# adrelino/mv-lm-icp

Measured on NVIDIA H100. Metric: ICP iterations/sec (corr+LM), higher is better.
Workload: dtype f64

## Files before the change

mv_lm_icp_b200/csrc/g2o.cuh:

```cuda
#pragma once
#include <cuda_runtime.h>
#include "../../include/mvicp.h"
#include "knn.cuh"
#include "lm_eval.cuh"
#include "lm_step.cuh"
#include "se3_math.cuh"
#include "types.cuh"

namespace mv {

enum { G2O_BUILD = 0, G2O_TRIAL = 1 };

struct G2oState {
  int32_t M, E, n, max_iter, max_calls, no_impr_limit, max_trials, ortho_after;
  int32_t phase, done, ended, last_call_end, call, iter, q, no_impr;
  int32_t n_iters, n_trials, n_accepted, n_evals, n_trace, trace_cap;
  double tau, lambda, nu, chi, last_chi, chi_initial, scale;
};

__host__ __device__ __forceinline__ void g2o_prec0(const double* n, double eps, double* Om) {
  double y[3] = {-n[1] * n[0], 1.0 - n[1] * n[1], -n[1] * n[2]};
  const double yy = y[0] * y[0] + y[1] * y[1] + y[2] * y[2];
  if (yy > 0.0) { const double s = sqrt(yy); y[0] /= s; y[1] /= s; y[2] /= s; }
  double x[3]; cross(n, y, x);
  const double* R[3] = {x, y, n};
  const double d[3] = {eps, eps, 1.0};
  int k = 0;
  for (int a = 0; a < 3; ++a)
    for (int b = a; b < 3; ++b) Om[k++] = (R[0][a] * d[0]) * R[0][b] + (R[1][a] * d[1]) * R[1][b] + (R[2][a] * d[2]) * R[2][b];
}

template <bool F32, bool NF32, int COST>
__global__ void __launch_bounds__(EVAL_THREADS)
g2o_eval_kernel(const FrameDev* __restrict__ frames, const EdgeDev* __restrict__ edges, const Tile* __restrict__ tiles, int tile_len,
                const int32_t* __restrict__ corr, const Rt* __restrict__ pose_eval, const G2oState* __restrict__ S, double eps,
                double* __restrict__ partial) {
  if (S->done) return;
  const bool build = S->phase == G2O_BUILD;
  const Tile t = tiles[blockIdx.x];
  const EdgeDev e = edges[t.edge];
  __shared__ double sF1[9], st1[3], sF0T[9], smt[3], sM01[9];
  __shared__ double sred[EVAL_THREADS / 32][2][GACC];
  if (threadIdx.x == 0) {
    const Rt a = pose_eval[e.src], k = pose_eval[e.dst];
    for (int i = 0; i < 9; ++i) sF1[i] = a.R[i];
    for (int i = 0; i < 3; ++i) for (int j = 0; j < 3; ++j) sF0T[3 * i + j] = k.R[3 * j + i];
    double ft[3]; matTvec(k.R, k.t, ft);
    for (int i = 0; i < 3; ++i) { st1[i] = a.t[i]; smt[i] = -ft[i]; }
    matTmul(k.R, a.R, sM01);
  }
  __syncthreads();
  const int role = threadIdx.x & 1;
  double C[9];
#pragma unroll
  for (int i = 0; i < 9; ++i) C[i] = role ? ((i % 4 == 0) ? 1.0 : 0.0) : sM01[i];
  const double tsg = role ? -1.0 : 1.0, rsg = role ? 2.0 : -2.0;
  const FrameDev fs = frames[e.src];
  const FrameDev fd = frames[e.dst];
  double acc[GACC];
#pragma unroll
  for (int i = 0; i < GACC; ++i) acc[i] = 0.0;
  const int end = min(t.start + tile_len, e.n_src);
  for (int k0 = t.start; k0 < end; k0 += EVAL_THREADS / 2) {
    const int k = k0 + (threadIdx.x >> 1);
    const int c = k < end ? __ldg(corr + e.off + k) : -1;
    const bool ok = c >= 0;
    if (!__any_sync(0xffffffffu, ok)) continue;
    double p[3] = {0, 0, 0}, q[3] = {0, 0, 0}, n[3] = {0, 0, 0}; int dummy;
    if (ok) {
      Rec<F32>::load(fs.pts_o, k, p[0], p[1], p[2], dummy);
      Rec<F32>::load(fd.pts_o, c, q[0], q[1], q[2], dummy);
      if (COST == COST_P2PLANE) Rec<NF32>::load(fd.nor_o, c, n[0], n[1], n[2], dummy);
    }
    const double live = ok ? 1.0 : 0.0;
    double y[3], u[3], r[3];
    matvec(sF1, p, y);
#pragma unroll
    for (int i = 0; i < 3; ++i) y[i] += st1[i];
    matvec(sF0T, y, u);
#pragma unroll
    for (int i = 0; i < 3; ++i) { u[i] += smt[i]; r[i] = u[i] - q[i]; }
    double Om[6] = {1, 0, 0, 1, 0, 1};
    if (COST == COST_P2PLANE) g2o_prec0(n, eps, Om);
    const double O3[9] = {Om[0], Om[1], Om[2], Om[1], Om[3], Om[4], Om[2], Om[4], Om[5]};
    double Or[3]; matvec(O3, r, Or);
    acc[45] += live * (r[0] * Or[0] + r[1] * Or[1] + r[2] * Or[2]);
    if (!build) continue;
    const double v[3] = {role ? u[0] : p[0], role ? u[1] : p[1], role ? u[2] : p[2]};
    const double vx[3][3] = {{0.0, v[2], -v[1]}, {-v[2], 0.0, v[0]}, {v[1], -v[0], 0.0}};
    double J[3][6], W[3][6];
#pragma unroll
    for (int i = 0; i < 3; ++i)
#pragma unroll
      for (int j = 0; j < 3; ++j) {
        J[i][j] = tsg * C[3 * i + j];
        J[i][3 + j] = rsg * (C[3 * i] * vx[j][0] + C[3 * i + 1] * vx[j][1] + C[3 * i + 2] * vx[j][2]);
      }
#pragma unroll
    for (int i = 0; i < 3; ++i)
#pragma unroll
      for (int j = 0; j < 6; ++j) W[i][j] = O3[3 * i] * J[0][j] + O3[3 * i + 1] * J[1][j] + O3[3 * i + 2] * J[2][j];
    int idx = 0;
#pragma unroll
    for (int a = 0; a < 6; ++a)
#pragma unroll
      for (int b = a; b < 6; ++b) acc[idx++] += live * (J[0][a] * W[0][b] + J[1][a] * W[1][b] + J[2][a] * W[2][b]);
#pragma unroll
    for (int a = 0; a < 3; ++a) {
      double X[3];
#pragma unroll
      for (int i = 0; i < 3; ++i) { const double o = __shfl_xor_sync(0xffffffffu, J[i][3 + a], 1); X[i] = role ? o : J[i][a]; }
#pragma unroll
      for (int b = 0; b < 6; ++b) {
        double Y[3];
#pragma unroll
        for (int i = 0; i < 3; ++i) { const double o = __shfl_xor_sync(0xffffffffu, W[i][b], 1); Y[i] = role ? W[i][b] : o; }
        acc[21 + 6 * a + b] += live * (X[0] * Y[0] + X[1] * Y[1] + X[2] * Y[2]);
      }
    }
#pragma unroll
    for (int a = 0; a < 6; ++a) acc[39 + a] += live * (J[0][a] * Or[0] + J[1][a] * Or[1] + J[2][a] * Or[2]);
  }
  const int lane = threadIdx.x & 31, wid = threadIdx.x >> 5;
#pragma unroll
  for (int i = 0; i < GACC; ++i) {
    if (!build && i != 45) continue;
    double v = acc[i];
#pragma unroll
    for (int o = 16; o > 1; o >>= 1) v += __shfl_xor_sync(0xffffffffu, v, o);
    if (lane < 2) sred[wid][lane][i] = v;
  }
  __syncthreads();
  if (threadIdx.x < 2 * GACC) {
    const int rl = threadIdx.x / GACC, i = threadIdx.x - GACC * rl;
    if (!build && i != 45) return;
    double v = 0.0;
    for (int w = 0; w < EVAL_THREADS / 32; ++w) v += sred[w][rl][i];
    int dst = -1;
    if (i < 21) {
      int a = 0, rem = i; while (rem >= 6 - a) { rem -= 6 - a; ++a; }
      dst = u12(6 * rl + a, 6 * rl + a + rem);
    } else if (i < 39) {
      const int a = (i - 21) / 6, b = (i - 21) - 6 * a;
      dst = u12(rl ? 3 + a : a, 6 + b);
    } else if (i < 45) dst = 78 + 6 * rl + (i - 39);
    else if (rl == 0) dst = 90;
    if (dst >= 0) partial[(size_t)blockIdx.x * GBLK + dst] = v;
  }
}

__global__ void __launch_bounds__(EDGE_THREADS)
g2o_edge_kernel(const int32_t* __restrict__ edge_tile_begin, const double* __restrict__ partial, const G2oState* __restrict__ S,
                double* __restrict__ out) {
  if (S->done) return;
  const bool build = S->phase == G2O_BUILD;
  const int e = blockIdx.x, tid = threadIdx.x;
  __shared__ double blk[GBLK];
  double* o = out + (size_t)EOUT_ * e;
  for (int j = tid; j < 91; j += EDGE_THREADS) {
    if (!build && j != 90) continue;
    double v = 0.0;
    for (int t = edge_tile_begin[e]; t < edge_tile_begin[e + 1]; ++t) v += partial[(size_t)t * GBLK + j];
    blk[j] = v;
  }
  __syncthreads();
  if (!build) { if (tid == 0) o[156] = blk[90]; return; }
  for (int r = tid; r < 157; r += EDGE_THREADS) {
    if (r < 144) { const int a = r / 12, b = r - 12 * a; o[r] = blk[u12(min(a, b), max(a, b))]; }
    else if (r < 156) o[r] = blk[78 + (r - 144)];
    else o[r] = blk[90];
  }
}

__global__ void g2o_count_kernel(const EdgeDev* __restrict__ edges, const Tile* __restrict__ tiles, int tile_len, const int32_t* __restrict__ corr,
                                 unsigned long long* __restrict__ count) {
  const Tile t = tiles[blockIdx.x];
  const EdgeDev e = edges[t.edge];
  const int end = min(t.start + tile_len, e.n_src);
  int m = 0;
  for (int k = t.start + threadIdx.x; k < end; k += blockDim.x) m += __ldg(corr + e.off + k) >= 0 ? 1 : 0;
  if (m) atomicAdd(count + t.edge, (unsigned long long)m);
}

struct G2oWork {
  G2oState* S;
  const double* eout;
  Rt* x;
  Rt* ev;
  int32_t* n_oplus;
  NormalLayout lay;
  double *H, *g;
  double* chi_calls;
  double* trace;
};

__global__ void g2o_init_kernel(G2oWork w, int M) {
  const int f = blockIdx.x * blockDim.x + threadIdx.x;
  if (f >= M) return;
  Rt a; pose16_to_Rt(w.lay.poses16 + 16 * f, &a);
  w.x[f] = a; w.ev[f] = a; w.n_oplus[f] = 0;
}

__device__ __forceinline__ void g2o_oplus(const Rt& x, const double* d, int* count, int ortho_after, Rt* out) {
  const double qq = d[3] * d[3] + d[4] * d[4] + d[5] * d[5];
  double R[9] = {1, 0, 0, 0, 1, 0, 0, 0, 1};
  if (!(1.0 - qq < 0.0)) {
    const double qw = sqrt(1.0 - qq), qx = d[3], qy = d[4], qz = d[5];
    const double tx = 2 * qx, ty = 2 * qy, tz = 2 * qz;
    const double twx = tx * qw, twy = ty * qw, twz = tz * qw, txx = tx * qx, txy = ty * qx, txz = tz * qx, tyy = ty * qy, tyz = tz * qy, tzz = tz * qz;
    R[0] = 1 - (tyy + tzz); R[1] = txy - twz; R[2] = txz + twy;
    R[3] = txy + twz; R[4] = 1 - (txx + tzz); R[5] = tyz - twx;
    R[6] = txz - twy; R[7] = tyz + twx; R[8] = 1 - (txx + tyy);
  }
  matmul(x.R, R, out->R);
  matvec(x.R, d, out->t);
  for (int i = 0; i < 3; ++i) out->t[i] += x.t[i];
  if (++*count > ortho_after) {
    *count = 0;
    double Em[9]; matTmul(out->R, out->R, Em);
    Em[0] -= 1; Em[4] -= 1; Em[8] -= 1;
    double FE[9]; matmul(out->R, Em, FE);
    for (int i = 0; i < 9; ++i) out->R[i] -= 0.5 * FE[i];
  }
}

__global__ void __launch_bounds__(STEP_THREADS) g2o_step_kernel(G2oWork w) {
  extern __shared__ double smem[];
  __shared__ double red[40];
  __shared__ G2oState s_state;
  __shared__ int s_solve, s_accept, s_tobuild;
  if (w.S->done) { if (threadIdx.x == 0) publish_step(w.lay, true); return; }
  const int tid = threadIdx.x, T = blockDim.x;
  copy_state(&s_state, w.S);
  G2oState* S = &s_state;
  const int n = S->n, M = S->M, E = S->E;
  const int phase = S->phase;
  const NormalLayout& lay = w.lay;
  double* colj = smem; double* dg = smem + 2 * (n + 1);
  double* L = lay.l_in_smem ? smem + 3 * (n + 1) : lay.Lg;

  const double chi_eval = edge_cost_sum(w.eout, E, red);

  auto end_iter = [&](double rho) {
    S->iter += 1; S->n_iters += 1;
    const bool term = S->q == S->max_trials || rho == 0.0;
    if (term || S->iter >= S->max_iter) {
      S->last_call_end = term ? MVICP_G2O_CALL_TERMINATE : MVICP_G2O_CALL_ITERATIONS;
      w.chi_calls[S->call + 1] = S->chi;
      const double impr = (S->last_chi - S->chi) / S->last_chi;
      S->last_chi = S->chi;
      if (!(impr > 0.0)) S->no_impr += 1;
      S->call += 1;
      if (S->no_impr > S->no_impr_limit) { S->done = 1; S->ended = MVICP_G2O_END_NO_IMPROVEMENT; return; }
      if (S->call >= S->max_calls) { S->done = 1; S->ended = MVICP_G2O_END_MAX_CALLS; return; }
      S->iter = 0;
    }
    S->phase = G2O_BUILD;
    s_tobuild = 1;
  };
  auto record = [&](double tchi, double rho, bool acc) {
    if (S->n_trace < S->trace_cap) {
      double* r = w.trace + 5 * (size_t)S->n_trace;
      r[0] = S->lambda; r[1] = S->chi; r[2] = tchi; r[3] = rho; r[4] = acc ? 1.0 : 0.0;
    }
    S->n_trace += 1;
  };

  if (tid == 0) { s_solve = 0; s_accept = 0; s_tobuild = 0; S->n_evals += 1; }
  if (phase == G2O_BUILD) {
    gather_blocks(lay, w.eout, n, w.H);
    gather_gradient(lay, w.eout, M, w.g);
    __syncthreads();
    double md = 0.0;
    for (int j = tid; j < n; j += T) md = fmax(md, fabs(w.H[(size_t)j * n + j]));
    md = block_max(md, red);
    if (tid == 0) {
      if (S->call == 0 && S->iter == 0) { S->chi_initial = S->last_chi = chi_eval; w.chi_calls[0] = chi_eval; }
      S->chi = chi_eval;
      if (S->iter == 0) { S->lambda = S->tau * md; S->nu = 2.0; }
      S->q = 0;
      s_solve = 1;
    }
  } else if (tid == 0) {
    const double tchi = chi_eval;
    const double rho = (S->chi - tchi) / S->scale;
    const bool acc = rho > 0.0 && isfinite(tchi);
    record(tchi, rho, acc);
    if (acc) {
      const double a = 1.0 - (2.0 * rho - 1.0) * (2.0 * rho - 1.0) * (2.0 * rho - 1.0);
      S->lambda *= fmax(1.0 / 3.0, fmin(2.0 / 3.0, a));
      S->nu = 2.0; S->chi = tchi; S->n_accepted += 1;
      s_accept = 1;
    } else { S->lambda *= S->nu; S->nu *= 2.0; }
    S->q += 1;
    if (rho < 0.0 && S->q < S->max_trials) s_solve = 1; else end_iter(rho);
  }
  __syncthreads();
  if (s_accept) for (int f = tid; f < M; f += T) w.x[f] = w.ev[f];
  __syncthreads();

  while (s_solve) {
    const double lambda = S->lambda;
    for (int i = tid >> 5; i < n; i += T >> 5) {
      const int rbi = lay.rowbase[i];
      for (int j = lay.rfirst[i] + (tid & 31); j <= i; j += 32) L[rbi + j] = w.H[(size_t)i * n + j] + (i == j ? lambda : 0.0);
    }
    { const int rbn = lay.rowbase[n]; for (int j = tid; j < n; j += T) L[rbn + j] = -w.g[j]; }
    __syncthreads();
    bool ok = chol_solve(L, lay.rowbase, n, colj, dg, lay.rhs, lay.rlast, lay.rfirst);
    double bad = 0.0;
    if (ok) for (int j = tid; j < n; j += T) if (!isfinite(lay.rhs[j])) bad = 1.0;
    bad = block_sum(bad, red);
    ok = ok && bad == 0.0;
    double sc = 0.0;
    if (ok) for (int j = tid; j < n; j += T) sc += lay.rhs[j] * (lambda * lay.rhs[j] - w.g[j]);
    sc = block_sum(sc, red);
    for (int f = tid; f < M; f += T) {
      const int cf = lay.col[f];
      if (cf < 0) continue;
      Rt nx;
      g2o_oplus(w.x[f], lay.rhs + cf, &w.n_oplus[f], S->ortho_after, &nx);
      if (ok) w.ev[f] = nx;
    }
    __syncthreads();
    if (tid == 0) {
      S->n_trials += 1;
      s_solve = 0;
      if (ok) { S->scale = sc + 1e-3; S->phase = G2O_TRIAL; }
      else {
        const double rho = -INFINITY;
        record(INFINITY, rho, false);
        S->lambda *= S->nu; S->nu *= 2.0; S->q += 1;
        if (S->q < S->max_trials) s_solve = 1; else end_iter(rho);
      }
    }
    __syncthreads();
  }
  if (s_tobuild && !S->done) for (int f = tid; f < M; f += T) w.ev[f] = w.x[f];
  if (S->done)
    for (int f = tid; f < M; f += T) if (lay.col[f] >= 0) Rt_to_pose16(&w.x[f], lay.poses16 + 16 * f);
  __syncthreads();
  copy_state(w.S, &s_state);
  if (tid == 0) publish_step(lay, S->done);
}

}
```

mv_lm_icp_b200/csrc/lm_step.cuh:

```cuda
#pragma once
#include <cuda_runtime.h>
#include "../../include/mvicp.h"
#include "se3_math.cuh"
#include "types.cuh"

namespace mv {

constexpr int STEP_THREADS = 512;
constexpr int EOUT = 160;

struct LmState {
  mvicp_lm_options opt;
  int32_t param, cost_kind, robust, M, E, F, n, G;
  int32_t phase, done, termination, iteration, n_success, n_invalid, n_evals, n_solves, reuse_diagonal, nonrigid;
  double radius, decrease_factor, x_cost, cand_cost, x_norm, initial_cost, model_cost_change, step_norm, gmax;
};

struct NormalLayout {
  const int32_t* col;
  const int32_t* hb_ptr; const int32_t* hb_row; const int32_t* hb_col; const int32_t* hc_edge; const int32_t* hc_sub; int32_t n_hblocks;
  const int32_t* gb_ptr; const int32_t* gc_edge; const int32_t* gc_side;
  const int32_t* rlast; const int32_t* rfirst;
  const int32_t* rowbase;
  double *Lg, *rhs;
  int32_t l_in_smem;
  double* poses16;
  volatile int32_t* host_flag;
  int32_t seq;
};

struct LmWork {
  LmState* S;
  const EdgeDev* edges;
  const double* eout;
  volatile int* peer_flags;
  int32_t world, xseq;
  double* x;
  double* cand;
  Rt* Rt_eval;
  double* K_eval;
  FrameGen* G_eval;
  NormalLayout lay;
  double *H, *g, *Hc, *gc, *scale, *diag, *step;
  long long* prof;
};

struct LmProblem {
  LmState* S;
  const int32_t* frame;
  const int32_t* edge;
  NormalLayout lay;
  double *H, *g, *Hc, *gc, *scale, *diag, *step;
};

__device__ __forceinline__ double block_sum(double v, double* red) {
  __syncthreads();
  const int lane = threadIdx.x & 31, wid = threadIdx.x >> 5;
#pragma unroll
  for (int o = 16; o > 0; o >>= 1) v += __shfl_down_sync(0xffffffffu, v, o);
  if (lane == 0) red[wid] = v;
  __syncthreads();
  if (threadIdx.x == 0) { double s = 0; for (int w = 0; w < STEP_THREADS / 32; ++w) s += red[w]; red[32] = s; }
  __syncthreads();
  return red[32];
}
__device__ __forceinline__ double block_max(double v, double* red) {
  __syncthreads();
  const int lane = threadIdx.x & 31, wid = threadIdx.x >> 5;
#pragma unroll
  for (int o = 16; o > 0; o >>= 1) v = fmax(v, __shfl_down_sync(0xffffffffu, v, o));
  if (lane == 0) red[wid] = v;
  __syncthreads();
  if (threadIdx.x == 0) { double s = 0; for (int w = 0; w < STEP_THREADS / 32; ++w) s = fmax(s, red[w]); red[32] = s; }
  __syncthreads();
  return red[32];
}

__device__ __forceinline__ void gather_blocks(const NormalLayout& l, const double* eout, int n, double* H) {
  for (int idx = threadIdx.x; idx < l.n_hblocks * 36; idx += blockDim.x) {
    const int b = idx / 36, r = idx - 36 * b, i = r / 6, j = r - 6 * i;
    double s = 0;
    for (int c = l.hb_ptr[b]; c < l.hb_ptr[b + 1]; ++c) {
      const int e = l.hc_edge[c], sub = l.hc_sub[c];
      s += eout[(size_t)EOUT * e + (6 * (sub >> 1) + i) * 12 + 6 * (sub & 1) + j];
    }
    H[(size_t)(l.hb_row[b] + i) * n + l.hb_col[b] + j] = s;
  }
}
__device__ __forceinline__ void gather_gradient(const NormalLayout& l, const double* eout, int M, double* g) {
  for (int idx = threadIdx.x; idx < M * 6; idx += blockDim.x) {
    const int f = idx / 6, i = idx - 6 * f;
    if (l.col[f] < 0) continue;
    double s = 0;
    for (int c = l.gb_ptr[f]; c < l.gb_ptr[f + 1]; ++c) s += eout[(size_t)EOUT * l.gc_edge[c] + 144 + 6 * l.gc_side[c] + i];
    g[l.col[f] + i] = s;
  }
}
__device__ __forceinline__ double edge_cost_sum(const double* eout, int E, double* red, const int32_t* edge = nullptr) {
  double s = 0.0;
  for (int e = threadIdx.x; e < E; e += blockDim.x) s += eout[(size_t)EOUT * (edge ? edge[e] : e) + 156];
  return block_sum(s, red);
}
template <typename State> __device__ __forceinline__ void copy_state(State* dst, const State* src) {
  for (int i = threadIdx.x; i < (int)(sizeof(State) / sizeof(int32_t)); i += blockDim.x)
    reinterpret_cast<int32_t*>(dst)[i] = reinterpret_cast<const int32_t*>(src)[i];
  __syncthreads();
}
__device__ __forceinline__ void publish_step(const NormalLayout& l, bool done) {
  __threadfence();
  l.host_flag[l.seq & 7] = (l.seq << 1) | (done ? 1 : 0);
  __threadfence_system();
}

__global__ void lm_init_kernel(LmWork w) {
  LmState* S = w.S;
  const int f = blockIdx.x * blockDim.x + threadIdx.x;
  if (f >= S->M) return;
  double x[7] = {0, 0, 0, 0, 0, 0, 0};
  param_of_pose(S->param, w.lay.poses16 + 16 * f, x);
  if (S->param != PARAM_AA) {
    const double n2 = x[0] * x[0] + x[1] * x[1] + x[2] * x[2] + x[3] * x[3];
    if (!(fabs(n2 - 1.0) <= 1e-9)) atomicExch(&S->nonrigid, 1);
  }
  Rt a; Rt_of_param(S->param, x, &a);
  double K[36]; tangent_map(S->param, x, &a, K);
  for (int i = 0; i < 7; ++i) { w.x[7 * f + i] = x[i]; w.cand[7 * f + i] = x[i]; }
  w.Rt_eval[f] = a;
  for (int i = 0; i < 36; ++i) w.K_eval[36 * f + i] = K[i];
  if (w.G_eval && S->param != PARAM_AA) frame_general(S->param, x, &w.G_eval[f]);
}

__device__ __forceinline__ void chol_factor_diag(double* L, const int32_t* rb, int j0, double* dinv, volatile int* s_ok, int lane) {
  double D[6][6], inv[6];
#pragma unroll
  for (int i = 0; i < 6; ++i)
#pragma unroll
    for (int k = 0; k <= i; ++k) D[i][k] = L[rb[j0 + i] + j0 + k];
  bool okb = true;
#pragma unroll
  for (int k = 0; k < 6; ++k) {
    double d = D[k][k];
#pragma unroll
    for (int m = 0; m < k; ++m) d -= D[k][m] * D[k][m];
    if (!(d > 0.0) || !isfinite(d)) okb = false;
    inv[k] = rsqrt(d); D[k][k] = d * inv[k];
#pragma unroll
    for (int i = k + 1; i < 6; ++i) {
      double v = D[i][k];
#pragma unroll
      for (int m = 0; m < k; ++m) v -= D[i][m] * D[k][m];
      D[i][k] = v * inv[k];
    }
  }
  __syncwarp();
  if (lane == 0) {
    if (!okb) *s_ok = 0;
#pragma unroll
    for (int i = 0; i < 6; ++i) {
#pragma unroll
      for (int k = 0; k <= i; ++k) L[rb[j0 + i] + j0 + k] = D[i][k];
      dinv[j0 + i] = inv[i];
    }
  }
}

__device__ bool chol_solve(double* L, const int32_t* __restrict__ rowbase, int n, double* scratch, double* dinv, double* y,
                           const int32_t* __restrict__ rlast, const int32_t* __restrict__ rfirst, long long* prof = nullptr) {
  const int T = blockDim.x, tid = threadIdx.x, lane = tid & 31, wid = tid >> 5, nw = T >> 5;
  int32_t* s_rfirst = reinterpret_cast<int32_t*>(scratch);
  int32_t* s_rlast = s_rfirst + n;
  int32_t* rb = s_rlast + n;
  volatile int* s_ok = reinterpret_cast<volatile int*>(rb + n + 1);
  for (int i = tid; i < n; i += T) { s_rfirst[i] = rfirst[i]; s_rlast[i] = rlast[i]; }
  for (int i = tid; i <= n; i += T) rb[i] = rowbase[i];
  if (tid == 0) *s_ok = 1;
  __syncthreads();
  const int NB = n / 6;
  if (wid == 0) chol_factor_diag(L, rb, 0, dinv, s_ok, lane);
  __syncthreads();
  long long t_panel = 0, t_ahead = 0, t_bar = 0;
  for (int J = 0; J < NB; ++J) {
    if (!*s_ok) return false;
    const long long c0 = prof ? clock64() : 0;
    const int j0 = 6 * J;
    const int rl = s_rlast[j0 + 5];
    const int nrows = rl - (j0 + 5) + 1;
    for (int q = tid; q < nrows; q += T) {
      const int r = (q == nrows - 1) ? n : j0 + 6 + q;
      if (r < n && s_rfirst[r] > j0 + 5) continue;
      double* row = L + rb[r] + j0;
      double v[6];
#pragma unroll
      for (int k = 0; k < 6; ++k) {
        double a = row[k];
#pragma unroll
        for (int m = 0; m < k; ++m) a -= v[m] * L[rb[j0 + k] + j0 + m];
        v[k] = a * dinv[j0 + k];
      }
#pragma unroll
      for (int k = 0; k < 6; ++k) row[k] = v[k];
    }
    const long long c1 = prof ? clock64() : 0;
    __syncthreads();
    const long long c2 = prof ? clock64() : 0;
    const bool next = J + 1 < NB;
    if (wid == 0 && next) {
      const int b0 = j0 + 6;
      if (lane < 21 && s_rfirst[b0] <= j0 + 5) {
        int i = 0, rem = lane; while (rem > i) { rem -= i + 1; ++i; }
        const int k = rem;
        double* row = L + rb[b0 + i]; const double* lc = L + rb[b0 + k] + j0;
        double a = row[b0 + k];
#pragma unroll
        for (int m = 0; m < 6; ++m) a -= row[j0 + m] * lc[m];
        row[b0 + k] = a;
      }
      __syncwarp();
      chol_factor_diag(L, rb, b0, dinv, s_ok, lane);
    } else {
      const int w0 = next ? 1 : 0, wn = next ? nw - 1 : nw;
      const int qfirst = next ? 6 : 0;
      for (int q = qfirst + (wid - w0); q < nrows; q += wn) {
        const int r = (q == nrows - 1) ? n : j0 + 6 + q;
        if (r < n && s_rfirst[r] > j0 + 5) continue;
        double* row = L + rb[r];
        double lr[6];
#pragma unroll
        for (int k = 0; k < 6; ++k) lr[k] = row[j0 + k];
        const int cend = min(r, rl);
        for (int c = j0 + 6 + lane; c <= cend; c += 32) {
          if (s_rfirst[c] > j0 + 5) continue;
          const double* lc = L + rb[c] + j0;
          double a = row[c];
#pragma unroll
          for (int k = 0; k < 6; ++k) a -= lr[k] * lc[k];
          row[c] = a;
        }
      }
    }
    const long long c3 = prof ? clock64() : 0;
    __syncthreads();
    if (prof) { const long long c4 = clock64(); t_panel += c1 - c0; t_ahead += c3 - c2; t_bar += (c2 - c1) + (c4 - c3); }
  }
  if (prof && tid == 0) { prof[8] = t_panel; prof[9] = t_ahead; prof[10] = t_bar; }
  if (!*s_ok) return false;
  for (int i = tid; i < n; i += T) y[i] = L[rb[n] + i];
  __syncthreads();
  if (wid == 0) {
    for (int J = NB - 1; J >= 0; --J) {
      const int j0 = 6 * J;
      double x[6];
#pragma unroll
      for (int k = 5; k >= 0; --k) {
        double a = y[j0 + k];
#pragma unroll
        for (int m = k + 1; m < 6; ++m) a -= L[rb[j0 + m] + j0 + k] * x[m];
        x[k] = a * dinv[j0 + k];
      }
      __syncwarp();
#pragma unroll
      for (int k = 0; k < 6; ++k) if (lane == k) y[j0 + k] = x[k];
      for (int i = s_rfirst[j0] + lane; i < j0; i += 32) {
        double a = y[i];
#pragma unroll
        for (int k = 0; k < 6; ++k) a -= L[rb[j0 + k] + i] * x[k];
        y[i] = a;
      }
      __syncwarp();
    }
  }
  __syncthreads();
  return true;
}

template <bool COMP>
__device__ __forceinline__ void lm_step_body(const LmWork& w, const LmProblem& p) {
  extern __shared__ double smem[];
  __shared__ double red[40];
  __shared__ int s_flag;
  if (p.S->done) { if (!COMP && threadIdx.x == 0) publish_step(w.lay, true); return; }
  const int tid = threadIdx.x, T = blockDim.x;
  __shared__ LmState s_state;
  copy_state(&s_state, p.S);
  LmState* S = &s_state;
  const int n = S->n, M = S->M, E = S->E, param = S->param;
  const NormalLayout& lay = p.lay;
  auto gf = [&](int f) { return COMP ? p.frame[f] : f; };
  long long* prof = w.prof ? w.prof + 16 * (w.lay.seq & 3) : nullptr;
#define MV_STAMP(i) do { if (prof && tid == 0) prof[i] = clock64(); } while (0)
  MV_STAMP(0);
  if (w.peer_flags) {
    if (tid < w.world) {
      const long long t0 = clock64();
      while (w.peer_flags[tid] - w.xseq < 0) {
        if (clock64() - t0 > 4000000000LL) { S->nonrigid = 2; break; }
      }
    }
    __syncthreads();
  }
  double* colj = smem; double* dg = smem + 2 * (S->n + 1);
  double* L = lay.l_in_smem ? smem + 3 * (S->n + 1) : lay.Lg;

  gather_blocks(lay, w.eout, n, p.Hc);
  gather_gradient(lay, w.eout, M, p.gc);
  __syncthreads();
  const double eval_cost = edge_cost_sum(w.eout, E, red, COMP ? p.edge : nullptr);

  MV_STAMP(1);
  bool take = false;
  if (tid == 0) {
    s_flag = 0;
    S->n_evals += 1;
    if (!isfinite(eval_cost)) {
      if (S->phase == 0) { S->done = 1; S->termination = MVICP_TERM_EVAL_FAILURE; }
      else {
        S->n_invalid += 1;
        if (S->n_invalid >= S->opt.max_num_consecutive_invalid_steps) { S->done = 1; S->termination = MVICP_TERM_INVALID_STEPS; }
        S->radius = S->radius / S->decrease_factor; S->decrease_factor *= 2.0; S->reuse_diagonal = 1;
      }
    } else if (S->phase == 0) {
      S->x_cost = eval_cost; S->initial_cost = eval_cost; s_flag = 1;
    } else {
      S->cand_cost = eval_cost;
      if (S->step_norm <= S->opt.parameter_tolerance * (S->x_norm + S->opt.parameter_tolerance)) {
        S->done = 1; S->termination = MVICP_TERM_PARAMETER_TOLERANCE;
      } else if (fabs(S->x_cost - eval_cost) <= S->opt.function_tolerance * S->x_cost) {
        S->done = 1; S->termination = MVICP_TERM_FUNCTION_TOLERANCE;
      } else {
        const double rho = (S->x_cost - eval_cost) / S->model_cost_change;
        if (rho > S->opt.min_relative_decrease) {
          s_flag = 1; S->n_success += 1; S->x_cost = eval_cost;
          const double q = 2.0 * rho - 1.0;
          S->radius = fmin(S->opt.max_trust_region_radius, S->radius / fmax(1.0 / 3.0, 1.0 - q * q * q));
          S->decrease_factor = 2.0; S->reuse_diagonal = 0;
        } else {
          S->radius = S->radius / S->decrease_factor; S->decrease_factor *= 2.0; S->reuse_diagonal = 1;
          if (S->radius < S->opt.min_trust_region_radius) { S->done = 1; S->termination = MVICP_TERM_MIN_RADIUS; }
        }
      }
    }
  }
  __syncthreads();
  take = s_flag != 0;
  if (take) {
    for (int idx = tid; idx < lay.n_hblocks * 36; idx += T) {
      const int b = idx / 36, r = idx - 36 * b, i = r / 6, j = r - 6 * i;
      const size_t at = (size_t)(lay.hb_row[b] + i) * n + lay.hb_col[b] + j;
      p.H[at] = p.Hc[at];
    }
    for (int idx = tid; idx < n; idx += T) p.g[idx] = p.gc[idx];
    for (int idx = tid; idx < M * 7; idx += T) { const int at = COMP ? 7 * gf(idx / 7) + idx % 7 : idx; w.x[at] = w.cand[at]; }
    __syncthreads();
    if (S->phase == 0)
      for (int j = tid; j < n; j += T) p.scale[j] = S->opt.jacobi_scaling ? 1.0 / (1.0 + sqrt(p.H[(size_t)j * n + j])) : 1.0;
    double xs = 0.0, gm = 0.0;
    for (int f = tid; f < M; f += T) {
      if (lay.col[f] < 0) continue;
      const int G = S->G;
      double xf[7], ng[6], xp[7];
      for (int i = 0; i < G; ++i) { xf[i] = w.x[7 * gf(f) + i]; xs += xf[i] * xf[i]; }
      for (int i = 0; i < 6; ++i) ng[i] = -p.g[lay.col[f] + i];
      param_plus(param, xf, ng, xp);
      for (int i = 0; i < G; ++i) gm = fmax(gm, fabs(xf[i] - xp[i]));
    }
    xs = block_sum(xs, red);
    gm = block_max(gm, red);
    if (tid == 0) {
      S->x_norm = sqrt(xs); S->gmax = gm;
      if (gm <= S->opt.gradient_tolerance) { S->done = 1; S->termination = MVICP_TERM_GRADIENT_TOLERANCE; }
      if (S->phase == 0) { S->phase = 1; S->iteration = 0; S->reuse_diagonal = 0; }
    }
    __syncthreads();
  }

  MV_STAMP(2);
  while (!S->done) {
    __syncthreads();
    if (S->iteration >= S->opt.max_num_iterations) {
      __syncthreads();
      if (tid == 0) { S->done = 1; S->termination = MVICP_TERM_MAX_ITERATIONS; }
      __syncthreads();
      break;
    }
    const int reuse = S->reuse_diagonal;
    const double radius = S->radius;
    __syncthreads();
    if (!reuse)
      for (int j = tid; j < n; j += T) {
        const double d = p.scale[j] * p.scale[j] * p.H[(size_t)j * n + j];
        p.diag[j] = fmin(fmax(d, S->opt.min_lm_diagonal), S->opt.max_lm_diagonal);
      }
    __syncthreads();
    for (int i = tid >> 5; i < n; i += T >> 5) {
      const double si = p.scale[i];
      const int rbi = lay.rowbase[i];
      for (int j = lay.rfirst[i] + (tid & 31); j <= i; j += 32) {
        double v = si * p.H[(size_t)i * n + j] * p.scale[j];
        if (i == j) { const double ldg = sqrt(p.diag[i] / radius); v += ldg * ldg; }
        L[rbi + j] = v;
      }
    }
    { const int rbn = lay.rowbase[n]; for (int j = tid; j < n; j += T) L[rbn + j] = p.scale[j] * p.g[j]; }
    __syncthreads();
    MV_STAMP(3);
    bool ok = chol_solve(L, lay.rowbase, n, colj, dg, lay.rhs, lay.rlast, lay.rfirst, prof);
    MV_STAMP(4);
    double bad = 0.0;
    if (ok) for (int j = tid; j < n; j += T) if (!isfinite(lay.rhs[j])) bad = 1.0;
    bad = block_sum(bad, red);
    ok = ok && (bad == 0.0);
    double mcc = 0.0;
    if (ok) {
      for (int j = tid; j < n; j += T) p.step[j] = -lay.rhs[j];
      __syncthreads();
      double acc = 0.0;
      for (int i = tid; i < n; i += T) {
        const double y = lay.rhs[i];
        acc += 0.5 * (y * p.scale[i] * p.g[i] + (p.diag[i] / radius) * y * y);
      }
      mcc = block_sum(acc, red);
    }
    const bool valid = ok && (mcc > 0.0);
    __syncthreads();
    if (tid == 0) {
      S->iteration += 1; S->n_solves += 1; S->reuse_diagonal = 1; S->model_cost_change = mcc;
      if (!valid) {
        S->n_invalid += 1;
        if (S->n_invalid >= S->opt.max_num_consecutive_invalid_steps) { S->done = 1; S->termination = MVICP_TERM_INVALID_STEPS; }
        S->radius = S->radius / S->decrease_factor; S->decrease_factor *= 2.0;
      } else S->n_invalid = 0;
    }
    __syncthreads();
    if (!valid) continue;
    double sn = 0.0;
    for (int f = tid; f < M; f += T) {
      const int G = S->G, g_f = gf(f);
      double xf[7], d[6], xp[7] = {0, 0, 0, 0, 0, 0, 0};
      for (int i = 0; i < 7; ++i) xf[i] = w.x[7 * g_f + i];
      if (lay.col[f] >= 0) {
        for (int i = 0; i < 6; ++i) d[i] = p.step[lay.col[f] + i] * p.scale[lay.col[f] + i];
        param_plus(param, xf, d, xp);
        for (int i = 0; i < G; ++i) sn += (xf[i] - xp[i]) * (xf[i] - xp[i]);
      } else for (int i = 0; i < 7; ++i) xp[i] = xf[i];
      for (int i = 0; i < 7; ++i) w.cand[7 * g_f + i] = xp[i];
      Rt a; Rt_of_param(param, xp, &a);
      w.Rt_eval[g_f] = a;
      double K[36]; tangent_map(param, xp, &a, K);
      for (int i = 0; i < 36; ++i) w.K_eval[36 * g_f + i] = K[i];
      if (w.G_eval && param != PARAM_AA) frame_general(param, xp, &w.G_eval[g_f]);
    }
    sn = block_sum(sn, red);
    MV_STAMP(5);
    if (tid == 0) S->step_norm = sqrt(sn);
    __syncthreads();
    break;
  }
  __syncthreads();
  if (S->done) {
    for (int f = tid; f < M; f += T) {
      double xf[7]; for (int i = 0; i < 7; ++i) xf[i] = w.x[7 * gf(f) + i];
      pose_of_param(param, xf, w.lay.poses16 + 16 * gf(f));
    }
  }
  __syncthreads();
  copy_state(p.S, &s_state);
  MV_STAMP(6);
  if (!COMP && tid == 0) publish_step(w.lay, S->done);
  MV_STAMP(7);
#undef MV_STAMP
}

__global__ void __launch_bounds__(STEP_THREADS) lm_step_kernel(LmWork w) {
  const LmProblem p{w.S, nullptr, nullptr, w.lay, w.H, w.g, w.Hc, w.gc, w.scale, w.diag, w.step};
  lm_step_body<false>(w, p);
}

__global__ void __launch_bounds__(STEP_THREADS) lm_step_components_kernel(LmWork w, const LmProblem* __restrict__ probs, unsigned int* ticket) {
  __shared__ LmProblem s_prob;
  copy_state(&s_prob, probs + blockIdx.x);
  lm_step_body<true>(w, s_prob);
  __shared__ int s_last;
  __syncthreads();
  if (threadIdx.x == 0) { __threadfence(); s_last = atomicAdd(ticket, 1u) == gridDim.x - 1; }
  __syncthreads();
  if (!s_last) return;
  __threadfence();
  int open = 0;
  for (int k = threadIdx.x; k < (int)gridDim.x; k += blockDim.x) open |= *(volatile const int*)&probs[k].S->done == 0;
  open = __syncthreads_count(open);
  if (threadIdx.x == 0) { *ticket = 0u; publish_step(w.lay, open == 0); }
}

}
```

mv_lm_icp_b200/csrc/mvicp.cu:

```cuda
#include <cuda_runtime.h>
#include <nccl.h>
#ifdef __linux__
#include <sched.h>
#endif
#include <algorithm>
#include <atomic>
#include <cmath>
#include <cstdarg>
#include <cstdio>
#include <cstdlib>
#include <cstring>
#include <limits>
#include <numeric>
#include <string>
#include <thread>
#include <vector>

#include "../../include/mvicp.h"
#include "closed.cuh"
#include "compact.cuh"
#include "device_io.cuh"
#include "far.cuh"
#include "g2o.cuh"
#include "knn.cuh"
#include "lm_eval.cuh"
#include "lm_step.cuh"
#include "normals.cuh"
#include "se3_math.cuh"
#include "select.cuh"
#include "types.cuh"

using namespace mv;

static thread_local std::string g_err;
static int fail(int code, const char* fmt, ...) {
  char buf[512];
  va_list ap; va_start(ap, fmt); vsnprintf(buf, sizeof buf, fmt, ap); va_end(ap);
  g_err = buf;
  return code;
}
#define CU(call)                                                                                              \
  do {                                                                                                        \
    cudaError_t e_ = (call);                                                                                  \
    if (e_ != cudaSuccess) return fail(MVICP_ERR_CUDA, "%s:%d %s: %s", __FILE__, __LINE__, #call, cudaGetErrorString(e_)); \
  } while (0)
#define NC(call)                                                                                              \
  do {                                                                                                        \
    ncclResult_t r_ = (call);                                                                                 \
    if (r_ != ncclSuccess) return fail(MVICP_ERR_NCCL, "%s:%d %s: %s", __FILE__, __LINE__, #call, ncclGetErrorString(r_)); \
  } while (0)
#define RET(call) do { int r__ = (call); if (r__ != MVICP_OK) return r__; } while (0)

struct DevBuf {
  void* p = nullptr; size_t cap = 0;
  DevBuf() = default;
  DevBuf(const DevBuf&) = delete;
  DevBuf& operator=(const DevBuf&) = delete;
  ~DevBuf() { release(); }
  int reserve(size_t bytes) {
    if (bytes <= cap) return MVICP_OK;
    if (p) cudaFree(p);
    p = nullptr; cap = 0;
    CU(cudaMalloc(&p, bytes ? bytes : 16));
    cap = bytes ? bytes : 16;
    return MVICP_OK;
  }
  void release() { if (p) cudaFree(p); p = nullptr; cap = 0; }
  template <typename T> T* as() const { return reinterpret_cast<T*>(p); }
};

struct mvicp_ctx {
  int device = 0, flags = 0;
  cudaStream_t stream = nullptr; bool own_stream = false;
  int rank = 0, world = 1; ncclComm_t comm = nullptr;
  void* xbuf = nullptr; void* peer_x[MAX_PEERS] = {}; bool p2p_ok = false; int32_t xseq = 0;
  static constexpr int X_ECAP = 4096;
  int M = 0; bool f32 = true; bool nor_f32 = true; bool have_normals = true;
  std::vector<void*> nor_dbl;
  float normals_ms = 0.f;
  std::vector<int64_t> n_pts;
  std::vector<FrameDev> h_frames;
  std::vector<void*> frame_allocs;
  DevBuf d_obb;
  int seeded_rounds = 0;
  DevBuf d_single;
  DevBuf d_prof;
  DevBuf d_tile_count, d_tile_off, d_edge_off, d_recs;
  bool obb_ready = false;
  int last_lm_iters = 1 << 20;
  DevBuf d_frames, d_poses;
  std::vector<uint8_t> fixed;
  std::vector<double> h_poses;
  int E = 0;
  std::vector<EdgeDev> h_edges;
  std::vector<int32_t> edge_owner;
  DevBuf d_edges, d_xf, d_corr, d_d2, d_count, d_sel, d_hist, d_weight, d_median, d_selcand, d_selcand_n;
  DevBuf d_sel_cnt;
  DevBuf d_sel_win;
  DevBuf d_certs, d_cert_cnt;
  DevBuf d_todo, d_todo_n;
  bool cert_valid = false;
  int64_t cert_rounds = 0;
  bool sel_valid = false;
  int64_t sel_guess_rounds = 0;
  DevBuf d_knn_tiles, d_eval_tiles, d_edge_tile_begin, d_partial;
  int n_knn_tiles = 0, n_eval_tiles = 0, eval_tile_len = EVAL_TILE;
  int64_t total_slots = 0;
  bool have_corr = false;
  bool nonrigid = false;
  std::vector<float> h_weight; std::vector<unsigned long long> h_count;
  DevBuf d_state, d_x, d_cand, d_Rt, d_K, d_col, d_H, d_g, d_Hc, d_gc, d_scale, d_diag, d_L, d_rhs, d_step,
      d_eout, d_hb_ptr, d_hb_row, d_hb_col, d_hc_edge, d_hc_sub, d_gb_ptr, d_gc_edge, d_gc_side, d_posegather, d_rlast, d_rfirst, d_rowbase, d_gen;
  int64_t l_size = 0;
  int n_free = 0;
  NormalLayout lay{};
  std::vector<int32_t> h_col;
  void* h_state = nullptr;
  volatile int32_t* h_flag = nullptr; volatile int32_t* d_flag = nullptr;
  std::vector<uint8_t> lm_key; uint32_t graph_gen = 0;
  DevBuf d_cmp_i32, d_cmp_f64, d_cmp_prob, d_cmp_state, d_cmp_ticket;
  std::vector<uint8_t> cmp_key;
  std::vector<int32_t> cmp_of_frame;
  std::vector<int32_t> cmp_prob;
  std::vector<int32_t> cmp_M, cmp_E, cmp_n;
  int n_cmp = 0, n_prob = 0; size_t cmp_dyn = 0, cmp_edge_map = 0;
  DevBuf d_g2o_state, d_g2o_x, d_g2o_ev, d_g2o_nop, d_g2o_chi, d_g2o_trace, d_g2o_tiles, d_g2o_tile_begin, d_g2o_cnt;
  int64_t g2o_trials = 0;
  mvicp_stats stats{};
  cudaEvent_t ev[8]{};
  std::vector<cudaEvent_t> eval_ev;
  int eval_ev_used = 0;
  bool ev_knn = false, ev_lm = false;
  float lm_eval_acc = 0.f;
  DevBuf d_cpq, d_cpr;
  DevBuf d_set_win, d_set_bad;
  DevBuf d_knn_nor;
};

static inline int owner_of(const mvicp_ctx* c, int frame) { return (int)(((int64_t)frame * c->world) / std::max(1, c->M)); }
static void assign_edge_owners(mvicp_ctx* c) {
  const int E = c->E;
  c->edge_owner.assign(E, -1);
  int64_t total = 0;
  for (int e = 0; e < E; ++e) if (!c->fixed[c->h_edges[e].src]) total += c->n_pts[c->h_edges[e].src];
  int64_t before = 0;
  for (int e = 0; e < E; ++e) {
    const int s = c->h_edges[e].src;
    if (c->fixed[s]) continue;
    const int64_t n = c->n_pts[s];
    c->edge_owner[e] = total > 0 ? (int)std::min<int64_t>(c->world - 1, ((2 * before + n) * c->world) / (2 * total)) : 0;
    before += n;
  }
}

#include "tree_build.h"
#include "tree_gpu.cuh"

extern "C" { static int refresh_after_fixed_change(mvicp_ctx* c); }

static bool poses_nonrigid(const double* poses16, int M) {
  for (int f = 0; f < M; ++f) {
    Rt a; pose16_to_Rt(poses16 + 16 * f, &a);
    double q[4]; quat_of_matrix(a.R, q);
    const double n2 = q[0] * q[0] + q[1] * q[1] + q[2] * q[2] + q[3] * q[3];
    if (!(std::fabs(n2 - 1.0) <= 1e-9)) return true;
  }
  return false;
}

static unsigned host_workers() {
  unsigned n = std::max(1u, std::thread::hardware_concurrency());
#ifdef __linux__
  cpu_set_t set; CPU_ZERO(&set);
  if (sched_getaffinity(0, sizeof set, &set) == 0) { const int k = CPU_COUNT(&set); if (k > 0) n = std::min<unsigned>(n, (unsigned)k); }
  if (FILE* f = std::fopen("/sys/fs/cgroup/cpu.max", "r")) {
    char q[32]; long long period = 0;
    if (std::fscanf(f, "%31s %lld", q, &period) == 2 && std::strcmp(q, "max") != 0 && period > 0) {
      const long long quota = std::atoll(q);
      if (quota > 0) n = std::min<unsigned>(n, (unsigned)std::max<long long>(1, quota / period));
    }
    std::fclose(f);
  }
#endif
  return std::max(1u, n);
}

static int finish_set_frames(mvicp_ctx* c, int M) {
  if (c->f32 && c->nor_f32)
    for (int f = 0; f < M; ++f) {
      FrameDev& fr = c->h_frames[f];
      if (!fr.nor_o) continue;
      void* d_pn = nullptr;
      CU(cudaMalloc(&d_pn, sizeof(float4) * 2 * (size_t)fr.n)); c->frame_allocs.push_back(d_pn);
      pack_pn_kernel<<<(fr.n + 255) / 256, 256, 0, c->stream>>>((const float4*)fr.pts_o, (const float4*)fr.nor_o, fr.n, (float4*)d_pn);
      c->stats.kernel_launches += 1;
      fr.pn_o = (const float4*)d_pn;
    }
  RET(c->d_frames.reserve(sizeof(FrameDev) * M));
  CU(cudaMemcpy(c->d_frames.p, c->h_frames.data(), sizeof(FrameDev) * M, cudaMemcpyHostToDevice));
  RET(c->d_poses.reserve(sizeof(double) * 16 * M));
  c->h_poses.assign((size_t)16 * M, 0.0);
  for (int f = 0; f < M; ++f) for (int i = 0; i < 4; ++i) c->h_poses[16 * f + 5 * i] = 1.0;
  CU(cudaMemcpy(c->d_poses.p, c->h_poses.data(), sizeof(double) * 16 * M, cudaMemcpyHostToDevice));
  c->fixed.assign(M, 0); c->fixed[0] = 1;
  c->E = 0; c->h_edges.clear(); c->have_corr = false;
  c->last_lm_iters = 1 << 20;
  return MVICP_OK;
}

#ifdef __CUDACC__
template <bool F32>
static int build_frames_on_device(mvicp_ctx* c, int M, const std::vector<double*>& d_xyz, const std::vector<double*>& d_nor,
                                  const int64_t* n_pts, const std::vector<float>& absmax) {
  const size_t rec = F32 ? sizeof(float4) : sizeof(double4a);
  const bool want_obb = !(c->flags & MVICP_FLAG_NO_OBB);
  KdScratch S;
  std::vector<ObbDev> ho(M);
  cudaError_t err = cudaSuccess;
  for (int f = 0; f < M && err == cudaSuccess; ++f) {
    const int n = (int)n_pts[f];
    const int64_t n_leaf = std::max<int64_t>(1, ((int64_t)n + LEAF - 1) / LEAF);
    int L = 1; while (L < n_leaf) L <<= 1;
    int depth = 0; while ((1 << depth) < L) ++depth;
    const int n_pad = (int)(n_leaf * LEAF);
    void *d_o = nullptr, *d_n = nullptr, *d_s = nullptr, *d_b = nullptr, *d_sf = nullptr, *d_pos = nullptr, *d_fc = nullptr, *d_ob = nullptr, *d_adj = nullptr;
    auto grab = [&](void** p, size_t bytes) { if (err == cudaSuccess) { err = cudaMalloc(p, bytes); if (err == cudaSuccess) c->frame_allocs.push_back(*p); } };
    grab(&d_o, rec * (size_t)n); grab(&d_s, rec * (size_t)n_pad); grab(&d_b, sizeof(Box) * 2 * (size_t)L); grab(&d_fc, sizeof(float) * 2 * (size_t)L);
    grab(&d_pos, sizeof(int32_t) * (size_t)n); grab(&d_adj, sizeof(int32_t) * ADJ_SLOTS * (size_t)L);
    if (F32) d_sf = d_s; else grab(&d_sf, sizeof(float4) * (size_t)n_pad);
    if (d_nor[f]) grab(&d_n, rec * (size_t)n);
    if (want_obb) grab(&d_ob, sizeof(ObbNode) * 2 * (size_t)L);
    if (err != cudaSuccess) break;
    const KdGeom g{n, L, depth};
    err = kd_build_device<F32>(c->stream, S, d_xyz[f], g, d_s, (float4*)d_sf, (int32_t*)d_pos, (Box*)d_b, (float*)d_fc, (int32_t*)d_adj, (ObbNode*)d_ob,
                               &c->stats.kernel_launches);
    kd_pack_orig_kernel<F32><<<(n + 255) / 256, 256, 0, c->stream>>>(d_xyz[f], n, d_o);
    if (d_nor[f]) kd_pack_orig_kernel<F32><<<(n + 255) / 256, 256, 0, c->stream>>>(d_nor[f], n, d_n);
    c->stats.kernel_launches += d_nor[f] ? 2 : 1;
    c->h_frames[f] = FrameDev{d_o, d_n, nullptr, d_s, (const float4*)d_sf, (const Box*)d_b, (const float*)d_fc, (const int32_t*)d_pos,
                              (c->flags & MVICP_FLAG_NO_ADJ) ? nullptr : (const int32_t*)d_adj, (int32_t)n, L, depth, absmax[f]};
    ho[f] = ObbDev{(const ObbNode*)d_ob};
  }
  if (err == cudaSuccess) err = cudaStreamSynchronize(c->stream);
  S.release();
  if (err != cudaSuccess) return fail(MVICP_ERR_CUDA, "device tree build: %s", cudaGetErrorString(err));
  if (want_obb) {
    RET(c->d_obb.reserve(sizeof(ObbDev) * M));
    CU(cudaMemcpy(c->d_obb.p, ho.data(), sizeof(ObbDev) * M, cudaMemcpyHostToDevice));
    c->obb_ready = true;
  }
  return MVICP_OK;
}

static int set_frames_device(mvicp_ctx* c, int M, const double* const* pts, const double* const* nor, const int64_t* n_pts,
                             cudaMemcpyKind kind) {
  std::vector<double*> d_xyz(M, nullptr), d_nor(M, nullptr);
  int* d_flags = nullptr;
  auto cleanup = [&]() { for (double* p : d_xyz) cudaFree(p); for (double* p : d_nor) cudaFree(p); cudaFree(d_flags); };
  std::vector<int> h_flags(4 * (size_t)M);
  for (int f = 0; f < M; ++f) { h_flags[4 * f] = 1; h_flags[4 * f + 1] = 0; h_flags[4 * f + 2] = 1; h_flags[4 * f + 3] = 0; }
  cudaError_t err = cudaMalloc(&d_flags, sizeof(int) * 4 * (size_t)M);
  if (err == cudaSuccess) err = cudaMemcpy(d_flags, h_flags.data(), sizeof(int) * 4 * (size_t)M, cudaMemcpyHostToDevice);
  for (int f = 0; f < M && err == cudaSuccess; ++f) {
    const size_t bytes = sizeof(double) * 3 * (size_t)n_pts[f];
    err = cudaMalloc(&d_xyz[f], bytes);
    if (err == cudaSuccess) err = cudaMemcpyAsync(d_xyz[f], pts[f], bytes, kind, c->stream);
    if (err == cudaSuccess) kd_scan_kernel<<<2 * NUM_SMS, 256, 0, c->stream>>>(d_xyz[f], 3ll * n_pts[f], d_flags + 4 * f);
    if (err == cudaSuccess && nor && nor[f]) {
      err = cudaMalloc(&d_nor[f], bytes);
      if (err == cudaSuccess) err = cudaMemcpyAsync(d_nor[f], nor[f], bytes, kind, c->stream);
      if (err == cudaSuccess) kd_scan_kernel<<<2 * NUM_SMS, 256, 0, c->stream>>>(d_nor[f], 3ll * n_pts[f], d_flags + 4 * f + 2);
    }
    c->stats.kernel_launches += (nor && nor[f]) ? 2 : 1;
  }
  if (err == cudaSuccess) err = cudaMemcpyAsync(h_flags.data(), d_flags, sizeof(int) * 4 * (size_t)M, cudaMemcpyDeviceToHost, c->stream);
  if (err == cudaSuccess) err = cudaStreamSynchronize(c->stream);
  if (err != cudaSuccess) { cleanup(); return fail(MVICP_ERR_CUDA, "mvicp_set_frames (upload): %s", cudaGetErrorString(err)); }
  bool f32 = true; std::vector<float> absmax(M);
  for (int f = 0; f < M; ++f) {
    f32 = f32 && h_flags[4 * f] != 0 && h_flags[4 * f + 2] != 0;
    std::memcpy(&absmax[f], &h_flags[4 * f + 1], 4);
    if (!std::isfinite(absmax[f])) { cleanup(); return fail(MVICP_ERR_INVALID, "frame %d has a non-finite coordinate", f); }
  }
  c->f32 = f32; c->nor_f32 = f32;
  c->h_frames.assign(M, FrameDev{});
  const int rc = f32 ? build_frames_on_device<true>(c, M, d_xyz, d_nor, n_pts, absmax) : build_frames_on_device<false>(c, M, d_xyz, d_nor, n_pts, absmax);
  cleanup();
  return rc;
}
#endif

static bool all_fp32(const double* v, int64_t n) {
  for (int64_t i = 0; i < n; ++i) if ((double)(float)v[i] != v[i]) return false;
  return true;
}

static void pack_records(bool f32, const double* xyz, const int32_t* order, const int32_t* wfield, int64_t n, void* out) {
  for (int64_t i = 0; i < n; ++i) {
    const int64_t j = order ? order[i] : i;
    const int32_t w = wfield ? wfield[i] : 0;
    if (f32) {
      float4 r; r.x = (float)xyz[3 * j]; r.y = (float)xyz[3 * j + 1]; r.z = (float)xyz[3 * j + 2];
      std::memcpy(&r.w, &w, 4);
      reinterpret_cast<float4*>(out)[i] = r;
    } else {
      double4a r; r.x = xyz[3 * j]; r.y = xyz[3 * j + 1]; r.z = xyz[3 * j + 2];
      const long long wl = w; std::memcpy(&r.w, &wl, 8);
      reinterpret_cast<double4a*>(out)[i] = r;
    }
  }
}

static void pad_records(bool f32, void* recs, int64_t n, int64_t n_pad) {
  const int32_t w = INT32_MAX;
  for (int64_t i = n; i < n_pad; ++i) {
    if (f32) { float4 r; r.x = r.y = r.z = INFINITY; std::memcpy(&r.w, &w, 4); reinterpret_cast<float4*>(recs)[i] = r; }
    else { double4a r; r.x = r.y = r.z = INFINITY; const long long wl = w; std::memcpy(&r.w, &wl, 8); reinterpret_cast<double4a*>(recs)[i] = r; }
  }
}

static int check_device_ptr(const mvicp_ctx* c, const void* p, const char* fn, const char* what) {
  if (!p) return fail(MVICP_ERR_INVALID, "%s: %s is null", fn, what);
  cudaPointerAttributes a; std::memset(&a, 0, sizeof a);
  if (cudaPointerGetAttributes(&a, p) != cudaSuccess) { cudaGetLastError(); return fail(MVICP_ERR_INVALID, "%s: %s is not device memory", fn, what); }
  if ((a.type != cudaMemoryTypeDevice && a.type != cudaMemoryTypeManaged) || a.device != c->device)
    return fail(MVICP_ERR_INVALID, "%s: %s is not device memory of device %d", fn, what, c->device);
  return MVICP_OK;
}

extern "C" {

int mvicp_abi_version(void) { return 1; }
const char* mvicp_last_error(void) { return g_err.c_str(); }

void mvicp_default_lm_options(mvicp_lm_options* o) {
  o->max_num_iterations = 50; o->max_num_consecutive_invalid_steps = 5; o->jacobi_scaling = 1; o->reserved = 0;
  o->initial_trust_region_radius = 1e4; o->max_trust_region_radius = 1e16; o->min_trust_region_radius = 1e-32;
  o->min_relative_decrease = 1e-3; o->min_lm_diagonal = 1e-6; o->max_lm_diagonal = 1e32;
  o->function_tolerance = 1e-6; o->gradient_tolerance = 1e-10; o->parameter_tolerance = 1e-8;
}

int mvicp_create(const mvicp_config* cfg, mvicp_ctx** out) {
  if (!out) return fail(MVICP_ERR_INVALID, "mvicp_create: out is null");
  int ndev = 0;
  cudaError_t e = cudaGetDeviceCount(&ndev);
  if (e != cudaSuccess || ndev == 0)
    return fail(MVICP_ERR_CUDA, "mvicp_create: no CUDA device (%s); this engine has no CPU path", cudaGetErrorString(e));
  mvicp_ctx* c = new mvicp_ctx();
  c->device = cfg ? cfg->device : 0;
  c->flags = cfg ? cfg->flags : 0;
  if (c->device < 0 || c->device >= ndev) { const int d = c->device; delete c; return fail(MVICP_ERR_INVALID, "device %d out of range", d); }
  auto init = [&]() -> int {
    CU(cudaSetDevice(c->device));
    if (cfg && cfg->stream) c->stream = (cudaStream_t)cfg->stream;
    else { CU(cudaStreamCreateWithFlags(&c->stream, cudaStreamNonBlocking)); c->own_stream = true; }
    for (auto& ev : c->ev) CU(cudaEventCreate(&ev));
    CU(cudaMallocHost(&c->h_state, sizeof(LmState)));
    CU(cudaHostAlloc((void**)&c->h_flag, sizeof(int32_t) * 8, cudaHostAllocMapped));
    CU(cudaHostGetDevicePointer((void**)&c->d_flag, (void*)c->h_flag, 0));
    RET(c->d_single.reserve(16));
    return MVICP_OK;
  };
  const int rc = init();
  if (rc != MVICP_OK) { const std::string keep = g_err; mvicp_destroy(c); g_err = keep; return rc; }
  *out = c;
  return MVICP_OK;
}

void mvicp_destroy(mvicp_ctx* c) {
  if (!c) return;
  cudaSetDevice(c->device);
  if (c->stream) cudaStreamSynchronize(c->stream);
  for (int p = 0; p < MAX_PEERS; ++p) if (c->peer_x[p] && c->peer_x[p] != c->xbuf) cudaIpcCloseMemHandle(c->peer_x[p]);
  if (c->xbuf) cudaFree(c->xbuf);
  if (c->comm) ncclCommDestroy(c->comm);
  for (void* p : c->frame_allocs) cudaFree(p);
  for (auto& ev : c->ev) if (ev) cudaEventDestroy(ev);
  for (auto& ev : c->eval_ev) cudaEventDestroy(ev);
  if (c->h_state) cudaFreeHost(c->h_state);
  if (c->h_flag) cudaFreeHost((void*)c->h_flag);

  if (c->own_stream && c->stream) cudaStreamDestroy(c->stream);
  delete c;
}

}
static int set_frames_impl(mvicp_ctx* c, int32_t M, const double* const* pts, const double* const* nor, const int64_t* n_pts, bool dev_src) {
  if (!c || M <= 0 || !pts || !n_pts) return fail(MVICP_ERR_INVALID, "mvicp_set_frames: bad arguments");
  CU(cudaSetDevice(c->device));
  CU(cudaStreamSynchronize(c->stream));
  for (void* p : c->frame_allocs) cudaFree(p);
  c->frame_allocs.clear();
  c->M = M; c->n_pts.assign(n_pts, n_pts + M);
  c->have_normals = true;
  bool f32 = true;
  for (int f = 0; f < M; ++f) {
    if (n_pts[f] <= 0) return fail(MVICP_ERR_EMPTY, "frame %d has no points (nanoflann would throw, nanoflann.hpp:904)", f);
    if (n_pts[f] > (int64_t)INT32_MAX / 2) return fail(MVICP_ERR_INVALID, "frame %d too large", f);
    if (!pts[f]) return fail(MVICP_ERR_INVALID, "frame %d: null points", f);
    if (!nor || !nor[f]) c->have_normals = false;
  }
  c->nor_dbl.clear();
  c->obb_ready = false;
#ifdef __CUDACC__
  if (!(c->flags & MVICP_FLAG_HOST_BUILD)) {
    RET(set_frames_device(c, M, pts, nor, n_pts, dev_src ? cudaMemcpyDeviceToDevice : cudaMemcpyHostToDevice));
    return finish_set_frames(c, M);
  }
#endif
  std::vector<std::vector<double>> staged;
  std::vector<const double*> hp, hn;
  if (dev_src) {
    staged.resize(2 * (size_t)M); hp.assign(M, nullptr); hn.assign(M, nullptr);
    for (int f = 0; f < M; ++f) {
      const size_t cnt = 3 * (size_t)n_pts[f];
      staged[2 * f].resize(cnt);
      CU(cudaMemcpyAsync(staged[2 * f].data(), pts[f], sizeof(double) * cnt, cudaMemcpyDeviceToHost, c->stream));
      hp[f] = staged[2 * f].data();
      if (nor && nor[f]) {
        staged[2 * f + 1].resize(cnt);
        CU(cudaMemcpyAsync(staged[2 * f + 1].data(), nor[f], sizeof(double) * cnt, cudaMemcpyDeviceToHost, c->stream));
        hn[f] = staged[2 * f + 1].data();
      }
    }
    CU(cudaStreamSynchronize(c->stream));
    pts = hp.data();
    if (nor) nor = hn.data();
  }
  for (int f = 0; f < M; ++f) f32 = f32 && all_fp32(pts[f], 3 * n_pts[f]) && (!nor || !nor[f] || all_fp32(nor[f], 3 * n_pts[f]));
  c->f32 = f32; c->nor_f32 = f32;
  const size_t rec = f32 ? sizeof(float4) : sizeof(double4a);
  std::vector<HostFrameBuild> builds(M);
  {
    const unsigned hw = host_workers();
    std::vector<std::thread> pool;
    std::atomic<int> next{0};
    for (unsigned t = 0; t < std::min<unsigned>(hw, (unsigned)M); ++t)
      pool.emplace_back([&]() { for (int f; (f = next.fetch_add(1)) < M;) build_frame(pts[f], n_pts[f], builds[f]); });
    for (auto& th : pool) th.join();
  }
  c->h_frames.assign(M, FrameDev{});
  std::vector<char> stage;
  for (int f = 0; f < M; ++f) {
    const int64_t n = n_pts[f];
    void *d_o = nullptr, *d_n = nullptr, *d_s = nullptr, *d_b = nullptr, *d_sf = nullptr, *d_pos = nullptr, *d_fc = nullptr, *d_adj = nullptr;
    CU(cudaMalloc(&d_o, rec * n)); c->frame_allocs.push_back(d_o);
    const int64_t n_pad = ((n + LEAF - 1) / LEAF) * LEAF;
    CU(cudaMalloc(&d_s, rec * n_pad)); c->frame_allocs.push_back(d_s);
    CU(cudaMalloc(&d_b, sizeof(Box) * builds[f].boxes.size())); c->frame_allocs.push_back(d_b);
    stage.resize(rec * n);
    pack_records(f32, pts[f], nullptr, nullptr, n, stage.data());
    CU(cudaMemcpy(d_o, stage.data(), rec * n, cudaMemcpyHostToDevice));
    stage.resize(rec * n_pad);
    pack_records(f32, pts[f], builds[f].order.data(), builds[f].order.data(), n, stage.data());
    pad_records(f32, stage.data(), n, n_pad);
    CU(cudaMemcpy(d_s, stage.data(), rec * n_pad, cudaMemcpyHostToDevice));
    if (nor && nor[f]) {
      CU(cudaMalloc(&d_n, rec * n)); c->frame_allocs.push_back(d_n);
      pack_records(f32, nor[f], nullptr, nullptr, n, stage.data());
      CU(cudaMemcpy(d_n, stage.data(), rec * n, cudaMemcpyHostToDevice));
    }
    CU(cudaMemcpy(d_b, builds[f].boxes.data(), sizeof(Box) * builds[f].boxes.size(), cudaMemcpyHostToDevice));
    if (f32) d_sf = d_s;
    else {
      CU(cudaMalloc(&d_sf, sizeof(float4) * n_pad)); c->frame_allocs.push_back(d_sf);
      stage.resize(sizeof(float4) * n_pad);
      pack_records(true, pts[f], builds[f].order.data(), builds[f].order.data(), n, stage.data());
      pad_records(true, stage.data(), n, n_pad);
      CU(cudaMemcpy(d_sf, stage.data(), sizeof(float4) * n_pad, cudaMemcpyHostToDevice));
    }
    CU(cudaMalloc(&d_fc, sizeof(float) * builds[f].faces.size())); c->frame_allocs.push_back(d_fc);
    CU(cudaMemcpy(d_fc, builds[f].faces.data(), sizeof(float) * builds[f].faces.size(), cudaMemcpyHostToDevice));
    CU(cudaMalloc(&d_pos, sizeof(int32_t) * n)); c->frame_allocs.push_back(d_pos);
    CU(cudaMemcpy(d_pos, builds[f].pos_of.data(), sizeof(int32_t) * n, cudaMemcpyHostToDevice));
    CU(cudaMalloc(&d_adj, sizeof(int32_t) * builds[f].adj.size())); c->frame_allocs.push_back(d_adj);
    CU(cudaMemcpy(d_adj, builds[f].adj.data(), sizeof(int32_t) * builds[f].adj.size(), cudaMemcpyHostToDevice));
    c->h_frames[f] = FrameDev{d_o, d_n, nullptr, d_s, (const float4*)d_sf, (const Box*)d_b, (const float*)d_fc, (const int32_t*)d_pos,
                              (c->flags & MVICP_FLAG_NO_ADJ) ? nullptr : (const int32_t*)d_adj, (int32_t)n, builds[f].n_leaf_pad, builds[f].depth, builds[f].absmax};
  }
  c->last_lm_iters = 1 << 20;
  if (!(c->flags & MVICP_FLAG_NO_OBB)) {
    std::vector<ObbDev> ho(M);
    std::vector<std::vector<ObbHost>> obbs(M);
    {
      const unsigned hw = host_workers();
      std::vector<std::thread> pool; std::atomic<int> next{0};
      for (unsigned t = 0; t < std::min<unsigned>(hw, (unsigned)M); ++t)
        pool.emplace_back([&]() { for (int f; (f = next.fetch_add(1)) < M;) build_obb(pts[f], n_pts[f], builds[f], obbs[f]); });
      for (auto& th : pool) th.join();
    }
    static_assert(sizeof(ObbHost) == sizeof(ObbNode) && sizeof(ObbNode) == 64, "oriented node = 64 bytes");
    for (int f = 0; f < M; ++f) {
      void* d = nullptr;
      CU(cudaMalloc(&d, sizeof(ObbNode) * obbs[f].size())); c->frame_allocs.push_back(d);
      CU(cudaMemcpy(d, obbs[f].data(), sizeof(ObbNode) * obbs[f].size(), cudaMemcpyHostToDevice));
      ho[f] = ObbDev{(const ObbNode*)d};
    }
    RET(c->d_obb.reserve(sizeof(ObbDev) * M));
    CU(cudaMemcpy(c->d_obb.p, ho.data(), sizeof(ObbDev) * M, cudaMemcpyHostToDevice));
    c->obb_ready = true;
  }
  return finish_set_frames(c, M);
}
extern "C" {

int mvicp_set_frames(mvicp_ctx* c, int32_t M, const double* const* pts, const double* const* nor, const int64_t* n_pts) {
  return set_frames_impl(c, M, pts, nor, n_pts, false);
}

int mvicp_set_frames_device(mvicp_ctx* c, int32_t M, const double* const* pts, const double* const* nor, const int64_t* n_pts) {
  if (!c || M <= 0 || !pts || !n_pts) return fail(MVICP_ERR_INVALID, "mvicp_set_frames_device: bad arguments");
  CU(cudaSetDevice(c->device));
  for (int f = 0; f < M; ++f) {
    if (n_pts[f] <= 0 || !pts[f]) continue;
    RET(check_device_ptr(c, pts[f], "mvicp_set_frames_device", "pts_xyz[f]"));
    if (nor && nor[f]) RET(check_device_ptr(c, nor[f], "mvicp_set_frames_device", "nor_xyz[f]"));
  }
  return set_frames_impl(c, M, pts, nor, n_pts, true);
}

int mvicp_set_poses(mvicp_ctx* c, const double* poses16, const uint8_t* fixed) {
  if (!c || !c->M || !poses16) return fail(MVICP_ERR_INVALID, "mvicp_set_poses: bad arguments / no frames");
  CU(cudaSetDevice(c->device));
  if (std::memcmp(c->h_poses.data(), poses16, sizeof(double) * 16 * c->M) != 0) c->last_lm_iters = 1 << 20;
  std::memcpy(c->h_poses.data(), poses16, sizeof(double) * 16 * c->M);
  CU(cudaMemcpyAsync(c->d_poses.p, c->h_poses.data(), sizeof(double) * 16 * c->M, cudaMemcpyHostToDevice, c->stream));
  CU(cudaStreamSynchronize(c->stream));
  if (fixed && !std::equal(fixed, fixed + c->M, c->fixed.begin())) { c->fixed.assign(fixed, fixed + c->M); RET(refresh_after_fixed_change(c)); }
  c->nonrigid = poses_nonrigid(poses16, c->M);
  return MVICP_OK;
}

int mvicp_get_poses(mvicp_ctx* c, double* poses16) {
  if (!c || !c->M || !poses16) return fail(MVICP_ERR_INVALID, "mvicp_get_poses: bad arguments / no frames");
  CU(cudaSetDevice(c->device));
  CU(cudaMemcpyAsync(c->h_poses.data(), c->d_poses.p, sizeof(double) * 16 * c->M, cudaMemcpyDeviceToHost, c->stream));
  CU(cudaStreamSynchronize(c->stream));
  std::memcpy(poses16, c->h_poses.data(), sizeof(double) * 16 * c->M);
  return MVICP_OK;
}

static int layout_work(mvicp_ctx* c) {
  const int E = c->E;
  if (!E) return MVICP_OK;
  int64_t off = 0, owned_slots = 0;
  assign_edge_owners(c);
  for (int e = 0; e < E; ++e) {
    EdgeDev& ed = c->h_edges[e];
    ed.off = off; ed.n_src = (int32_t)c->n_pts[ed.src];
    ed.owned = c->edge_owner[e] == c->rank ? 1 : 0;
    off += ed.n_src;
    if (ed.owned) owned_slots += ed.n_src;
  }
  c->total_slots = off;
  int64_t active_slots = 0;
  for (int e = 0; e < E; ++e) if (c->edge_owner[e] >= 0) active_slots += c->h_edges[e].n_src;
  int tl = 8192;
  while (tl > 1024 && active_slots / tl < 8 * NUM_SMS) tl >>= 1;
  c->eval_tile_len = tl;
  (void)owned_slots;
  std::vector<Tile> kt, et; std::vector<int32_t> etb(E + 1, 0);
  for (int e = 0; e < E; ++e) {
    const EdgeDev& ed = c->h_edges[e];
    etb[e] = (int32_t)et.size();
    if (!ed.owned) continue;
    for (int s = 0; s < ed.n_src; s += KNN_TILE) kt.push_back(Tile{e, s});
    for (int s = 0; s < ed.n_src; s += tl) et.push_back(Tile{e, s});
  }
  etb[E] = (int32_t)et.size();
  c->n_knn_tiles = (int)kt.size(); c->n_eval_tiles = (int)et.size();
  RET(c->d_edges.reserve(sizeof(EdgeDev) * E));
  RET(c->d_knn_tiles.reserve(sizeof(Tile) * std::max<size_t>(1, kt.size())));
  RET(c->d_eval_tiles.reserve(sizeof(Tile) * std::max<size_t>(1, et.size())));
  RET(c->d_edge_tile_begin.reserve(sizeof(int32_t) * (E + 1)));
  RET(c->d_partial.reserve(sizeof(double) * NBLK * std::max<size_t>(1, et.size())));
  CU(cudaMemcpy(c->d_edges.p, c->h_edges.data(), sizeof(EdgeDev) * E, cudaMemcpyHostToDevice));
  if (!kt.empty()) CU(cudaMemcpy(c->d_knn_tiles.p, kt.data(), sizeof(Tile) * kt.size(), cudaMemcpyHostToDevice));
  if (!et.empty()) CU(cudaMemcpy(c->d_eval_tiles.p, et.data(), sizeof(Tile) * et.size(), cudaMemcpyHostToDevice));
  CU(cudaMemcpy(c->d_edge_tile_begin.p, etb.data(), sizeof(int32_t) * (E + 1), cudaMemcpyHostToDevice));
  ++c->graph_gen;
  return MVICP_OK;
}

static int rebuild_work(mvicp_ctx* c) {
  const int E = c->E;
  if (!E) return MVICP_OK;
  RET(layout_work(c));
  const int64_t off = c->total_slots;
  RET(c->d_xf.reserve(sizeof(EdgeXf) * E));
  RET(c->d_corr.reserve(sizeof(int32_t) * off));
  RET(c->d_d2.reserve(sizeof(double) * off));
  RET(c->d_count.reserve(sizeof(unsigned long long) * E));
  RET(c->d_sel.reserve(sizeof(SelState) * E));
  RET(c->d_hist.reserve(sizeof(unsigned int) * SEL_BINS * (size_t)E));
  RET(c->d_weight.reserve(sizeof(float) * E));
  RET(c->d_median.reserve(sizeof(double) * E));
  RET(c->d_selcand.reserve(sizeof(unsigned long long) * SEL_CAP * (size_t)E));
  RET(c->d_selcand_n.reserve(sizeof(unsigned int) * E));
  RET(c->d_sel_cnt.reserve(sizeof(unsigned int) * (2 * (size_t)E + 1)));
  CU(cudaMemset(c->d_sel_cnt.p, 0, sizeof(unsigned int) * (2 * (size_t)E + 1)));
  RET(c->d_sel_win.reserve(sizeof(unsigned long long) * 3 * (size_t)E));
  RET(c->d_certs.reserve(sizeof(float4) * off));
  RET(c->d_todo.reserve(sizeof(int2) * off));
  RET(c->d_todo_n.reserve(sizeof(unsigned int)));
  CU(cudaMemset(c->d_todo_n.p, 0, sizeof(unsigned int)));
  RET(c->d_cert_cnt.reserve(sizeof(unsigned long long) * E));
  CU(cudaMemset(c->d_cert_cnt.p, 0, sizeof(unsigned long long) * E));
  c->cert_valid = false;
  c->sel_valid = false;
  CU(cudaMemset(c->d_hist.p, 0, sizeof(unsigned int) * SEL_BINS * (size_t)E));
  CU(cudaMemset(c->d_weight.p, 0, sizeof(float) * E));
  CU(cudaMemset(c->d_selcand_n.p, 0, sizeof(unsigned int) * E));
  CU(cudaMemset(c->d_count.p, 0, sizeof(unsigned long long) * E));
  CU(cudaMemset(c->d_corr.p, 0xff, sizeof(int32_t) * off));
  c->h_weight.assign(E, 0.f); c->h_count.assign(E, 0ull);
  c->have_corr = false;
  return MVICP_OK;
}

static int refresh_after_fixed_change(mvicp_ctx* c) {
  if (!c->E) return MVICP_OK;
  CU(cudaStreamSynchronize(c->stream));
  return c->world > 1 ? rebuild_work(c) : layout_work(c);
}

int mvicp_set_graph(mvicp_ctx* c, int32_t E, const int32_t* src, const int32_t* dst) {
  if (!c || !c->M || E < 0 || (E && (!src || !dst))) return fail(MVICP_ERR_INVALID, "mvicp_set_graph: bad arguments / no frames");
  CU(cudaSetDevice(c->device));
  CU(cudaStreamSynchronize(c->stream));
  for (int e = 0; e < E; ++e)
    if (src[e] < 0 || src[e] >= c->M || dst[e] < 0 || dst[e] >= c->M || src[e] == dst[e])
      return fail(MVICP_ERR_INVALID, "edge %d: (%d -> %d) invalid", e, src[e], dst[e]);
  c->E = E; c->h_edges.assign(E, EdgeDev{});
  for (int e = 0; e < E; ++e) { c->h_edges[e].src = src[e]; c->h_edges[e].dst = dst[e]; }
  return rebuild_work(c);
}

int mvicp_pose_graph_knn(mvicp_ctx* c, int32_t knn) {
  if (!c || !c->M || knn < 0) return fail(MVICP_ERR_INVALID, "mvicp_pose_graph_knn: bad arguments / no frames");
  std::vector<int32_t> src, dst;
  for (int i = 0; i < c->M; ++i) {
    std::vector<std::pair<float, int>> nb;
    for (int j = 0; j < c->M; ++j) {
      if (i == j) continue;
      const double* a = &c->h_poses[16 * i + 12]; const double* b = &c->h_poses[16 * j + 12];
      const double d0 = a[0] - b[0], d1 = a[1] - b[1], d2 = a[2] - b[2];
      nb.push_back({(float)std::sqrt(d0 * d0 + d1 * d1 + d2 * d2), j});
    }
    std::stable_sort(nb.begin(), nb.end(), [](const std::pair<float, int>& x, const std::pair<float, int>& y) { return x.first < y.first; });
    for (int q = 0; q < knn && q < (int)nb.size(); ++q) { src.push_back(i); dst.push_back(nb[q].second); }
  }
  return mvicp_set_graph(c, (int32_t)src.size(), src.data(), dst.data());
}

int mvicp_get_graph(mvicp_ctx* c, int32_t* E, int32_t* src, int32_t* dst) {
  if (!c || !E) return fail(MVICP_ERR_INVALID, "mvicp_get_graph: bad arguments");
  *E = c->E;
  for (int e = 0; e < c->E; ++e) { if (src) src[e] = c->h_edges[e].src; if (dst) dst[e] = c->h_edges[e].dst; }
  return MVICP_OK;
}

}
static double cutoff_d2max(float thresh) {
  const double t = (double)thresh;
  if (!(t > 0.0)) return -1.0;
  if (std::isinf(t)) return std::numeric_limits<double>::max();
  double x = t * t;
  while (x > 0.0 && !(std::sqrt(x) < t)) x = std::nextafter(x, 0.0);
  while (std::sqrt(std::nextafter(x, std::numeric_limits<double>::infinity())) < t) x = std::nextafter(x, std::numeric_limits<double>::infinity());
  return std::sqrt(x) < t ? x : -1.0;
}
template <bool F32> static int launch_correspond(mvicp_ctx* c, float thresh) {
  const int E = c->E;
  const double d2max = cutoff_d2max(thresh);
  const bool seed = c->have_corr && !(c->flags & MVICP_FLAG_NO_SEED);
  bool guess = false, far = false;
  int cert = 0;
  const bool ww = !(c->flags & MVICP_FLAG_STEP_LOOP);
  if (c->n_knn_tiles) {
    if (!seed || c->last_lm_iters == (1 << 20)) c->seeded_rounds = 0;
    far = c->obb_ready && (!seed || c->seeded_rounds < 1);
    if (seed) ++c->seeded_rounds;
    const bool steady = seed && !far && ww, converged = steady && c->last_lm_iters <= 1;
    guess = converged && c->sel_valid && !(c->flags & MVICP_FLAG_NO_SELECT_GUESS);
    if (steady && !(c->flags & MVICP_FLAG_NO_CERT)) cert = (guess && c->cert_valid) ? 2 : (c->last_lm_iters <= 3 ? 1 : 0);
  }
  edge_xf_kernel<<<(E + 127) / 128, 128, 0, c->stream>>>(c->d_poses.as<double>(), c->d_edges.as<EdgeDev>(), E, c->d_xf.as<EdgeXf>());
  CU(cudaEventRecord(c->ev[0], c->stream));
  if (c->n_knn_tiles) {
    unsigned int* cnt = c->d_sel_cnt.as<unsigned int>();
    const SelGuess sg = {c->d_sel_win.as<unsigned long long>(), cnt, cnt + E, c->d_selcand.as<unsigned long long>(), c->d_selcand_n.as<unsigned int>()};
#define MV_KNN_ARGS c->d_frames.as<FrameDev>(), c->d_edges.as<EdgeDev>(), c->d_xf.as<EdgeXf>(), c->d_knn_tiles.as<Tile>(), \
                    c->d_corr.as<int32_t>(), c->d_d2.as<double>(), seed ? c->d_corr.as<int32_t>() : nullptr, d2max
#define MV_KNN_TAIL sg, E, c->d_certs.as<float4>()
    if (far) knn_far_kernel<F32><<<c->n_knn_tiles, KNN_TILE, 0, c->stream>>>(MV_KNN_ARGS, c->d_obb.as<ObbDev>());
    else if (cert == 2) {
      const CertTodo todo = {c->d_todo.as<int2>(), c->d_todo_n.as<unsigned int>()};
      knn_cert_kernel<F32><<<c->n_knn_tiles, KNN_TILE, 0, c->stream>>>(MV_KNN_ARGS, MV_KNN_TAIL, c->d_cert_cnt.as<unsigned long long>(), todo);
      knn_todo_kernel<F32><<<NUM_SMS * 5, KNN_TILE, 0, c->stream>>>(c->d_frames.as<FrameDev>(), c->d_edges.as<EdgeDev>(), c->d_xf.as<EdgeXf>(),
          c->d_corr.as<int32_t>(), c->d_d2.as<double>(), c->d_corr.as<int32_t>(), d2max, MV_KNN_TAIL, todo);
      c->stats.kernel_launches += 1;
    }
    else if (guess && cert == 1) knn_kernel<F32, true, true, 1><<<c->n_knn_tiles, KNN_TILE, 0, c->stream>>>(MV_KNN_ARGS, MV_KNN_TAIL);
    else if (guess) knn_kernel<F32, true, true, 0><<<c->n_knn_tiles, KNN_TILE, 0, c->stream>>>(MV_KNN_ARGS, MV_KNN_TAIL);
    else if (cert == 1) knn_kernel<F32, true, false, 1><<<c->n_knn_tiles, KNN_TILE, 0, c->stream>>>(MV_KNN_ARGS, MV_KNN_TAIL);
    else if (ww) knn_kernel<F32, true, false, 0><<<c->n_knn_tiles, KNN_TILE, 0, c->stream>>>(MV_KNN_ARGS, MV_KNN_TAIL);
    else knn_kernel<F32, false, false, 0><<<c->n_knn_tiles, KNN_TILE, 0, c->stream>>>(MV_KNN_ARGS, MV_KNN_TAIL);
    c->cert_valid = cert != 0;
    if (cert == 2) ++c->cert_rounds;
#undef MV_KNN_TAIL
#undef MV_KNN_ARGS
  }
  CU(cudaEventRecord(c->ev[1], c->stream));
  c->stats.kernel_launches += 1 + (c->n_knn_tiles ? 1 : 0);
  if (guess) {
    unsigned int* cnt = c->d_sel_cnt.as<unsigned int>();
    select_guess_finish_kernel<<<E, SEL_THREADS, 0, c->stream>>>(c->d_edges.as<EdgeDev>(), c->d_corr.as<int32_t>(), c->d_d2.as<double>(),
        c->d_sel.as<SelState>(), cnt, cnt + E, c->d_selcand.as<unsigned long long>(), c->d_selcand_n.as<unsigned int>(),
        c->d_weight.as<float>(), c->d_median.as<double>(), c->d_count.as<unsigned long long>(), c->d_sel_win.as<unsigned long long>(), cnt + 2 * (size_t)E,
        c->d_todo_n.as<unsigned int>());
    c->stats.kernel_launches += 1;
    ++c->sel_guess_rounds;
  } else {
  select_init_kernel<<<(E + 127) / 128, 128, 0, c->stream>>>(c->d_sel.as<SelState>(), E);
  c->stats.kernel_launches += 1;
  const int shifts[2] = {53, 42};
  for (int p = 0; p < 2; ++p) {
    if (c->n_eval_tiles)
      select_hist_kernel<<<c->n_eval_tiles, SEL_THREADS, 0, c->stream>>>(
          c->d_edges.as<EdgeDev>(), c->d_eval_tiles.as<Tile>(), c->eval_tile_len, c->d_corr.as<int32_t>(), c->d_d2.as<double>(),
          c->d_sel.as<SelState>(), shifts[p], 11, c->d_hist.as<unsigned int>());
    select_pick_kernel<<<E, SEL_THREADS, 0, c->stream>>>(c->d_sel.as<SelState>(), c->d_hist.as<unsigned int>(), shifts[p], p == 0, 0,
                                                         c->d_weight.as<float>(), c->d_median.as<double>(),
                                                         c->d_count.as<unsigned long long>());
    c->stats.kernel_launches += 1 + (c->n_eval_tiles ? 1 : 0);
  }
  if (c->n_eval_tiles)
    select_collect_kernel<<<c->n_eval_tiles, SEL_THREADS, 0, c->stream>>>(
        c->d_edges.as<EdgeDev>(), c->d_eval_tiles.as<Tile>(), c->eval_tile_len, c->d_corr.as<int32_t>(), c->d_d2.as<double>(),
        c->d_sel.as<SelState>(), c->d_selcand.as<unsigned long long>(), c->d_selcand_n.as<unsigned int>());
  select_finish_kernel<<<E, SEL_THREADS, 0, c->stream>>>(c->d_edges.as<EdgeDev>(), c->d_corr.as<int32_t>(), c->d_d2.as<double>(),
                                                         c->d_sel.as<SelState>(), c->d_selcand.as<unsigned long long>(),
                                                         c->d_selcand_n.as<unsigned int>(), c->d_weight.as<float>(), c->d_median.as<double>(),
                                                         c->d_sel_win.as<unsigned long long>());
  c->stats.kernel_launches += 1 + (c->n_eval_tiles ? 1 : 0);
  }
  c->sel_valid = true;
  CU(cudaEventRecord(c->ev[2], c->stream));
  CU(cudaGetLastError());
  return MVICP_OK;
}

extern "C" {
int mvicp_correspond(mvicp_ctx* c, float thresh) {
  if (!c || !c->M || !c->E) return fail(MVICP_ERR_STATE, "mvicp_correspond: frames and graph must be set first");
  CU(cudaSetDevice(c->device));
  RET(c->f32 ? launch_correspond<true>(c, thresh) : launch_correspond<false>(c, thresh));
  c->have_corr = true; c->ev_knn = true;
  int64_t q = 0; for (const EdgeDev& e : c->h_edges) if (e.owned) q += e.n_src;
  c->stats.queries = q;
  return MVICP_OK;
}

static int fetch_edge_meta(mvicp_ctx* c) {
  CU(cudaMemcpyAsync(c->h_weight.data(), c->d_weight.p, sizeof(float) * c->E, cudaMemcpyDeviceToHost, c->stream));
  CU(cudaMemcpyAsync(c->h_count.data(), c->d_count.p, sizeof(unsigned long long) * c->E, cudaMemcpyDeviceToHost, c->stream));
  CU(cudaStreamSynchronize(c->stream));
  return MVICP_OK;
}

int mvicp_get_edge(mvicp_ctx* c, int32_t e, int32_t* first, int32_t* second, double* dist, int64_t* count, float* weight) {
  if (!c || e < 0 || e >= c->E) return fail(MVICP_ERR_INVALID, "mvicp_get_edge: bad edge");
  CU(cudaSetDevice(c->device));
  const EdgeDev& ed = c->h_edges[e];
  if (!ed.owned && !c->fixed[ed.src]) return fail(MVICP_ERR_NOT_OWNER, "edge %d is processed by rank %d", e, c->edge_owner[e]);
  RET(fetch_edge_meta(c));
  if (weight) *weight = c->h_weight[e];
  if (count) *count = (int64_t)c->h_count[e];
  if (first || second || dist) {
    std::vector<int32_t> corr(ed.n_src); std::vector<double> d2(ed.n_src);
    CU(cudaMemcpy(corr.data(), c->d_corr.as<int32_t>() + ed.off, sizeof(int32_t) * ed.n_src, cudaMemcpyDeviceToHost));
    CU(cudaMemcpy(d2.data(), c->d_d2.as<double>() + ed.off, sizeof(double) * ed.n_src, cudaMemcpyDeviceToHost));
    int64_t n = 0;
    for (int k = 0; k < ed.n_src; ++k)
      if (corr[k] >= 0) {
        if (first) first[n] = k;
        if (second) second[n] = corr[k];
        if (dist) dist[n] = std::sqrt(d2[k]);
        ++n;
      }
    if (count) *count = n;
  }
  return MVICP_OK;
}

static int compact_count_scan(mvicp_ctx* c) {
  const int E = c->E, nt = c->n_knn_tiles;
  RET(c->d_tile_count.reserve(sizeof(unsigned int) * std::max(1, nt)));
  RET(c->d_tile_off.reserve(sizeof(unsigned long long) * std::max(1, nt)));
  RET(c->d_edge_off.reserve(sizeof(unsigned long long) * (E + 1)));
  if (nt) compact_count_kernel<<<nt, KNN_TILE, 0, c->stream>>>(c->d_edges.as<EdgeDev>(), c->d_knn_tiles.as<Tile>(), c->d_corr.as<int32_t>(), c->d_tile_count.as<unsigned int>());
  compact_scan_kernel<<<1, 1024, 0, c->stream>>>(c->d_tile_count.as<unsigned int>(), nt, c->d_knn_tiles.as<Tile>(), E,
                                                 c->d_tile_off.as<unsigned long long>(), c->d_edge_off.as<unsigned long long>());
  c->stats.kernel_launches += nt ? 2 : 1;
  return MVICP_OK;
}

int mvicp_get_all_edges(mvicp_ctx* c, void* out_records, int64_t capacity, int64_t* offsets, float* weights) {
  if (!c || !c->E || !offsets) return fail(MVICP_ERR_INVALID, "mvicp_get_all_edges: bad arguments / no graph");
  if (!c->have_corr) return fail(MVICP_ERR_STATE, "mvicp_get_all_edges: call mvicp_correspond first");
  CU(cudaSetDevice(c->device));
  const int E = c->E, nt = c->n_knn_tiles;
  RET(compact_count_scan(c));
  std::vector<unsigned long long> eo(E + 1);
  CU(cudaMemcpyAsync(eo.data(), c->d_edge_off.p, sizeof(unsigned long long) * (E + 1), cudaMemcpyDeviceToHost, c->stream));
  if (weights) CU(cudaMemcpyAsync(weights, c->d_weight.p, sizeof(float) * E, cudaMemcpyDeviceToHost, c->stream));
  CU(cudaStreamSynchronize(c->stream));
  for (int e = 0; e <= E; ++e) offsets[e] = (int64_t)eo[e];
  if (out_records) {
    const int64_t total = (int64_t)eo[E];
    if (total > capacity) return fail(MVICP_ERR_INVALID, "mvicp_get_all_edges: %lld records, capacity %lld", (long long)total, (long long)capacity);
    if (total) {
      RET(c->d_recs.reserve(sizeof(CorrRec) * (size_t)total));
      compact_scatter_kernel<<<nt, KNN_TILE, 0, c->stream>>>(c->d_edges.as<EdgeDev>(), c->d_knn_tiles.as<Tile>(), c->d_corr.as<int32_t>(), c->d_d2.as<double>(),
                                                             c->d_tile_off.as<unsigned long long>(), c->d_recs.as<CorrRec>());
      c->stats.kernel_launches += 1;
      CU(cudaMemcpyAsync(out_records, c->d_recs.p, sizeof(CorrRec) * (size_t)total, cudaMemcpyDeviceToHost, c->stream));
      CU(cudaStreamSynchronize(c->stream));
    }
  }
  CU(cudaGetLastError());
  return MVICP_OK;
}

int mvicp_get_all_edges_device(mvicp_ctx* c, void* out_records, int64_t capacity, int64_t* offsets, float* weights) {
  if (!c || !c->E || !offsets) return fail(MVICP_ERR_INVALID, "mvicp_get_all_edges_device: bad arguments / no graph");
  if (!c->have_corr) return fail(MVICP_ERR_STATE, "mvicp_get_all_edges_device: call mvicp_correspond first");
  CU(cudaSetDevice(c->device));
  RET(check_device_ptr(c, offsets, "mvicp_get_all_edges_device", "offsets"));
  if (out_records) RET(check_device_ptr(c, out_records, "mvicp_get_all_edges_device", "out_records"));
  if (weights) RET(check_device_ptr(c, weights, "mvicp_get_all_edges_device", "weights"));
  const int E = c->E, nt = c->n_knn_tiles;
  if (out_records) {
    int64_t bound = 0;
    for (const EdgeDev& ed : c->h_edges) if (ed.owned) bound += ed.n_src;
    if (capacity < bound)
      return fail(MVICP_ERR_INVALID, "mvicp_get_all_edges_device: up to %lld records, capacity %lld", (long long)bound, (long long)capacity);
  }
  RET(compact_count_scan(c));
  static_assert(sizeof(unsigned long long) == sizeof(int64_t), "offsets are copied as they are");
  CU(cudaMemcpyAsync(offsets, c->d_edge_off.p, sizeof(int64_t) * (E + 1), cudaMemcpyDeviceToDevice, c->stream));
  if (weights) CU(cudaMemcpyAsync(weights, c->d_weight.p, sizeof(float) * E, cudaMemcpyDeviceToDevice, c->stream));
  if (out_records && nt) {
    compact_scatter_kernel<<<nt, KNN_TILE, 0, c->stream>>>(c->d_edges.as<EdgeDev>(), c->d_knn_tiles.as<Tile>(), c->d_corr.as<int32_t>(), c->d_d2.as<double>(),
                                                           c->d_tile_off.as<unsigned long long>(), reinterpret_cast<CorrRec*>(out_records));
    c->stats.kernel_launches += 1;
  }
  CU(cudaGetLastError());
  return MVICP_OK;
}

int mvicp_host_alloc(size_t bytes, void** out) {
  if (!out) return fail(MVICP_ERR_INVALID, "mvicp_host_alloc: bad arguments");
  *out = nullptr;
  if (!bytes) return MVICP_OK;
  CU(cudaHostAlloc(out, bytes, cudaHostAllocPortable));
  return MVICP_OK;
}
int mvicp_host_free(void* p) {
  if (p) CU(cudaFreeHost(p));
  return MVICP_OK;
}

int mvicp_get_nn(mvicp_ctx* c, int32_t e, int32_t* nn_idx, double* nn_d2) {
  if (!c || e < 0 || e >= c->E) return fail(MVICP_ERR_INVALID, "mvicp_get_nn: bad edge");
  CU(cudaSetDevice(c->device));
  const EdgeDev& ed = c->h_edges[e];
  if (!ed.owned) return fail(MVICP_ERR_NOT_OWNER, "edge %d is not processed by this rank", e);
  CU(cudaStreamSynchronize(c->stream));
  if (nn_idx) {
    CU(cudaMemcpy(nn_idx, c->d_corr.as<int32_t>() + ed.off, sizeof(int32_t) * ed.n_src, cudaMemcpyDeviceToHost));
    for (int k = 0; k < ed.n_src; ++k) if (nn_idx[k] < 0) nn_idx[k] = ~nn_idx[k];
  }
  if (nn_d2) CU(cudaMemcpy(nn_d2, c->d_d2.as<double>() + ed.off, sizeof(double) * ed.n_src, cudaMemcpyDeviceToHost));
  return MVICP_OK;
}

int mvicp_set_edge(mvicp_ctx* c, int32_t e, const int32_t* first, const int32_t* second, int64_t count, float weight) {
  if (!c || e < 0 || e >= c->E || count < 0 || (count && (!first || !second))) return fail(MVICP_ERR_INVALID, "mvicp_set_edge: bad arguments");
  CU(cudaSetDevice(c->device));
  const EdgeDev& ed = c->h_edges[e];
  std::vector<int32_t> corr(ed.n_src, ~0);
  const int n_dst = (int)c->n_pts[ed.dst];
  for (int64_t i = 0; i < count; ++i) {
    if (first[i] < 0 || first[i] >= ed.n_src || second[i] < 0 || second[i] >= n_dst) return fail(MVICP_ERR_INVALID, "mvicp_set_edge: index out of range at %lld", (long long)i);
    corr[first[i]] = second[i];
  }
  CU(cudaStreamSynchronize(c->stream));
  CU(cudaMemcpy(c->d_corr.as<int32_t>() + ed.off, corr.data(), sizeof(int32_t) * ed.n_src, cudaMemcpyHostToDevice));
  CU(cudaMemcpy(c->d_weight.as<float>() + e, &weight, sizeof(float), cudaMemcpyHostToDevice));
  const unsigned long long cnt = (unsigned long long)count;
  CU(cudaMemcpy(c->d_count.as<unsigned long long>() + e, &cnt, sizeof cnt, cudaMemcpyHostToDevice));
  c->cert_valid = false;
  return MVICP_OK;
}

int mvicp_set_edge_device(mvicp_ctx* c, int32_t e, const int32_t* first, const int32_t* second, int64_t count, float weight) {
  if (!c || e < 0 || e >= c->E || count < 0 || (count && (!first || !second))) return fail(MVICP_ERR_INVALID, "mvicp_set_edge_device: bad arguments");
  CU(cudaSetDevice(c->device));
  if (count) {
    RET(check_device_ptr(c, first, "mvicp_set_edge_device", "first"));
    RET(check_device_ptr(c, second, "mvicp_set_edge_device", "second"));
  }
  const EdgeDev& ed = c->h_edges[e];
  const int n_dst = (int)c->n_pts[ed.dst];
  RET(c->d_set_win.reserve(sizeof(unsigned long long) * (size_t)std::max(1, ed.n_src)));
  RET(c->d_set_bad.reserve(sizeof(unsigned long long)));
  unsigned long long* win = c->d_set_win.as<unsigned long long>();
  unsigned long long* bad = c->d_set_bad.as<unsigned long long>();
  CU(cudaMemsetAsync(win, 0, sizeof(unsigned long long) * (size_t)ed.n_src, c->stream));
  CU(cudaMemsetAsync(bad, 0xff, sizeof(unsigned long long), c->stream));
  if (count) {
    const int grid = (int)std::min<int64_t>((count + 255) / 256, 8 * NUM_SMS);
    set_edge_scan_kernel<<<grid, 256, 0, c->stream>>>(first, second, (long long)count, ed.n_src, n_dst, win, bad);
    c->stats.kernel_launches += 1;
  }
  const int grid = (int)std::max<int64_t>(1, std::min<int64_t>((ed.n_src + 255) / 256, 8 * NUM_SMS));
  set_edge_write_kernel<<<grid, 256, 0, c->stream>>>(second, win, ed.n_src, bad, c->d_corr.as<int32_t>() + ed.off, c->d_weight.as<float>() + e,
                                                     c->d_count.as<unsigned long long>() + e, weight, (unsigned long long)count);
  c->stats.kernel_launches += 1;
  unsigned long long h_bad = 0;
  CU(cudaMemcpyAsync(&h_bad, bad, sizeof h_bad, cudaMemcpyDeviceToHost, c->stream));
  CU(cudaStreamSynchronize(c->stream));
  CU(cudaGetLastError());
  if (h_bad != ~0ull) return fail(MVICP_ERR_INVALID, "mvicp_set_edge_device: index out of range at %lld", (long long)h_bad);
  c->cert_valid = false;
  return MVICP_OK;
}

int mvicp_closest_point(mvicp_ctx* c, int32_t frame, const double q[3], int64_t* idx, double* d2) {
  if (!c || frame < 0 || frame >= c->M || !q) return fail(MVICP_ERR_INVALID, "mvicp_closest_point: bad arguments");
  CU(cudaSetDevice(c->device));
  long long* d_i = c->d_single.as<long long>(); double* d_d = c->d_single.as<double>() + 1;
  if (c->f32) knn_single_kernel<true><<<1, 1, 0, c->stream>>>(c->d_frames.as<FrameDev>(), frame, q[0], q[1], q[2], d_i, d_d);
  else knn_single_kernel<false><<<1, 1, 0, c->stream>>>(c->d_frames.as<FrameDev>(), frame, q[0], q[1], q[2], d_i, d_d);
  c->stats.kernel_launches += 1;
  long long hi = 0; double hd = 0;
  CU(cudaMemcpyAsync(&hi, d_i, 8, cudaMemcpyDeviceToHost, c->stream));
  CU(cudaMemcpyAsync(&hd, d_d, 8, cudaMemcpyDeviceToHost, c->stream));
  CU(cudaStreamSynchronize(c->stream));
  if (idx) *idx = hi;
  if (d2) *d2 = hd;
  return MVICP_OK;
}

}
static int launch_closest_points(mvicp_ctx* c, int frame, const double* q, int64_t n, long long* idx, double* d2) {
  const int grid = (int)std::min<int64_t>((n + 127) / 128, 64 * NUM_SMS);
  if (c->f32) closest_points_kernel<true><<<grid, 128, 0, c->stream>>>(c->d_frames.as<FrameDev>(), frame, q, (long long)n, idx, d2);
  else closest_points_kernel<false><<<grid, 128, 0, c->stream>>>(c->d_frames.as<FrameDev>(), frame, q, (long long)n, idx, d2);
  c->stats.kernel_launches += 1;
  CU(cudaGetLastError());
  return MVICP_OK;
}
extern "C" {

int mvicp_closest_points(mvicp_ctx* c, int32_t frame, const double* q, int64_t n, int64_t* idx, double* d2) {
  if (!c || frame < 0 || frame >= c->M || n < 0 || (n && !q)) return fail(MVICP_ERR_INVALID, "mvicp_closest_points: bad arguments");
  if (!n) return MVICP_OK;
  CU(cudaSetDevice(c->device));
  RET(c->d_cpq.reserve(sizeof(double) * 3 * (size_t)n));
  RET(c->d_cpr.reserve(16 * (size_t)n));
  long long* d_i = c->d_cpr.as<long long>(); double* d_d = c->d_cpr.as<double>() + n;
  CU(cudaMemcpyAsync(c->d_cpq.p, q, sizeof(double) * 3 * (size_t)n, cudaMemcpyHostToDevice, c->stream));
  RET(launch_closest_points(c, frame, c->d_cpq.as<double>(), n, d_i, d_d));
  if (idx) CU(cudaMemcpyAsync(idx, d_i, sizeof(int64_t) * (size_t)n, cudaMemcpyDeviceToHost, c->stream));
  if (d2) CU(cudaMemcpyAsync(d2, d_d, sizeof(double) * (size_t)n, cudaMemcpyDeviceToHost, c->stream));
  CU(cudaStreamSynchronize(c->stream));
  return MVICP_OK;
}

int mvicp_closest_points_device(mvicp_ctx* c, int32_t frame, const double* q, int64_t n, int64_t* idx, double* d2) {
  if (!c || frame < 0 || frame >= c->M || n < 0 || (n && !q)) return fail(MVICP_ERR_INVALID, "mvicp_closest_points_device: bad arguments");
  if (!n) return MVICP_OK;
  CU(cudaSetDevice(c->device));
  RET(check_device_ptr(c, q, "mvicp_closest_points_device", "q_xyz"));
  if (idx) RET(check_device_ptr(c, idx, "mvicp_closest_points_device", "idx"));
  if (d2) RET(check_device_ptr(c, d2, "mvicp_closest_points_device", "d2"));
  return launch_closest_points(c, frame, q, n, reinterpret_cast<long long*>(idx), d2);
}

struct LayoutPlan {
  std::vector<int32_t> col, hb_ptr{0}, hb_row, hb_col, hc_edge, hc_sub, gb_ptr{0}, gc_edge, gc_side, rlast, rfirst, rowbase;
  int64_t l_size = 0;
};
static int plan_normal_layout(const mvicp_ctx* c, const std::vector<int32_t>& frames, const std::vector<int32_t>& edges, int n,
                              const std::vector<uint8_t>& active, LayoutPlan& p) {
  const int M = (int)frames.size();
  std::vector<int32_t> loc(c->M, -1);
  for (int i = 0; i < M; ++i) loc[frames[i]] = i;
  std::vector<std::vector<std::pair<int, int>>> blk((size_t)M * M), gl(M);
  for (const int e : edges) {
    if (!active[e]) continue;
    const int s = loc[c->h_edges[e].src], k = loc[c->h_edges[e].dst];
    const bool fs = c->h_col[frames[s]] >= 0, fk = c->h_col[frames[k]] >= 0;
    if (fs) { blk[(size_t)s * M + s].push_back({e, 0}); gl[s].push_back({e, 0}); }
    if (fs && fk) { blk[(size_t)s * M + k].push_back({e, 1}); blk[(size_t)k * M + s].push_back({e, 2}); }
    if (fk) { blk[(size_t)k * M + k].push_back({e, 3}); gl[k].push_back({e, 1}); }
  }
  p.col.resize(M);
  for (int i = 0; i < M; ++i) p.col[i] = c->h_col[frames[i]];
  for (int r = 0; r < M; ++r)
    for (int q = 0; q < M; ++q) {
      const auto& l = blk[(size_t)r * M + q];
      if (l.empty()) continue;
      p.hb_row.push_back(p.col[r]); p.hb_col.push_back(p.col[q]);
      for (auto& pr : l) { p.hc_edge.push_back(pr.first); p.hc_sub.push_back(pr.second); }
      p.hb_ptr.push_back((int32_t)p.hc_edge.size());
    }
  for (int f = 0; f < M; ++f) { for (auto& pr : gl[f]) { p.gc_edge.push_back(pr.first); p.gc_side.push_back(pr.second); } p.gb_ptr.push_back((int32_t)p.gc_edge.size()); }
  const int n_hblocks = (int)p.hb_row.size();
  std::vector<int32_t>& rfirst = p.rfirst; std::vector<int32_t>& rlast = p.rlast;
  rfirst.resize(n); rlast.resize(n);
  for (int r = 0; r < n; ++r) rfirst[r] = (r / 6) * 6;
  for (int b = 0; b < n_hblocks; ++b)
    if (p.hb_col[b] < p.hb_row[b]) for (int i = 0; i < 6; ++i) rfirst[p.hb_row[b] + i] = std::min(rfirst[p.hb_row[b] + i], p.hb_col[b]);
  for (int j = 0; j < n; ++j) { rlast[j] = j; }
  for (int r = 0; r < n; ++r) for (int j = rfirst[r]; j <= r; ++j) rlast[j] = std::max(rlast[j], r);
  for (int j = 1; j < n; ++j) rlast[j] = std::max(rlast[j], rlast[j - 1]);
  p.rowbase.resize(n + 1); int64_t at = 0;
  for (int r = 0; r < n; ++r) { p.rowbase[r] = (int32_t)(at - rfirst[r]); at += r - rfirst[r] + 1; }
  p.rowbase[n] = (int32_t)at; at += n;
  if (at > INT32_MAX) return fail(MVICP_ERR_INVALID, "normal matrix too large");
  p.l_size = at;
  return MVICP_OK;
}

static int build_normal_layout(mvicp_ctx* c, int n, const std::vector<uint8_t>& active) {
  const int E = c->E;
  std::vector<int32_t> frames(c->M), edges(E);
  std::iota(frames.begin(), frames.end(), 0); std::iota(edges.begin(), edges.end(), 0);
  LayoutPlan pl;
  RET(plan_normal_layout(c, frames, edges, n, active, pl));
  const int n_hblocks = (int)pl.hb_row.size();
  auto up = [&](DevBuf& b, const std::vector<int32_t>& v) -> int {
    RET(b.reserve(sizeof(int32_t) * std::max<size_t>(1, v.size())));
    if (!v.empty()) CU(cudaMemcpyAsync(b.p, v.data(), sizeof(int32_t) * v.size(), cudaMemcpyHostToDevice, c->stream));
    return MVICP_OK;
  };
  RET(up(c->d_hb_ptr, pl.hb_ptr)); RET(up(c->d_hb_row, pl.hb_row)); RET(up(c->d_hb_col, pl.hb_col)); RET(up(c->d_hc_edge, pl.hc_edge));
  RET(up(c->d_hc_sub, pl.hc_sub)); RET(up(c->d_gb_ptr, pl.gb_ptr)); RET(up(c->d_gc_edge, pl.gc_edge)); RET(up(c->d_gc_side, pl.gc_side));
  RET(up(c->d_col, pl.col));
  RET(up(c->d_rlast, pl.rlast)); RET(up(c->d_rfirst, pl.rfirst));
  const int64_t at = pl.l_size;
  c->l_size = at;
  RET(c->d_L.reserve(sizeof(double) * (size_t)at));
  RET(up(c->d_rowbase, pl.rowbase));
  RET(c->d_H.reserve(sizeof(double) * n * n)); RET(c->d_g.reserve(sizeof(double) * n)); RET(c->d_rhs.reserve(sizeof(double) * n));
  RET(c->d_eout.reserve(sizeof(double) * EOUT * E));
  CU(cudaMemsetAsync(c->d_H.p, 0, sizeof(double) * (size_t)n * n, c->stream));
  CU(cudaStreamSynchronize(c->stream));
  NormalLayout& l = c->lay;
  l.col = c->d_col.as<int32_t>();
  l.hb_ptr = c->d_hb_ptr.as<int32_t>(); l.hb_row = c->d_hb_row.as<int32_t>(); l.hb_col = c->d_hb_col.as<int32_t>();
  l.hc_edge = c->d_hc_edge.as<int32_t>(); l.hc_sub = c->d_hc_sub.as<int32_t>(); l.n_hblocks = n_hblocks;
  l.gb_ptr = c->d_gb_ptr.as<int32_t>(); l.gc_edge = c->d_gc_edge.as<int32_t>(); l.gc_side = c->d_gc_side.as<int32_t>();
  l.rlast = c->d_rlast.as<int32_t>(); l.rfirst = c->d_rfirst.as<int32_t>(); l.rowbase = c->d_rowbase.as<int32_t>();
  l.Lg = c->d_L.as<double>(); l.rhs = c->d_rhs.as<double>(); l.host_flag = c->d_flag;
  return MVICP_OK;
}
}
template <bool F32> static void launch_eval(mvicp_ctx* c, int cost, int robust, DoneGate gate) {
  const int nt = c->n_eval_tiles;
  if (!nt) return;
#define MV_EVAL(NF, COSTK)                                                                                       \
  lm_eval_kernel<F32, NF, COSTK><<<nt, EVAL_THREADS, 0, c->stream>>>(                                            \
      c->d_frames.as<FrameDev>(), c->d_edges.as<EdgeDev>(), c->d_eval_tiles.as<Tile>(), c->eval_tile_len,       \
      c->d_corr.as<int32_t>(), c->d_Rt.as<Rt>(), c->d_weight.as<float>(), robust, c->d_partial.as<double>(), gate)
#define MV_EVALC(NF) { if (cost == COST_P2P) MV_EVAL(NF, COST_P2P); else if (cost == COST_P2PLANE) MV_EVAL(NF, COST_P2PLANE); else MV_EVAL(NF, COST_MIXED); }
  if (F32 && c->nor_f32) MV_EVALC(F32) else MV_EVALC(false)
#undef MV_EVALC
#undef MV_EVAL
}

template <bool F32> static void launch_eval_general(mvicp_ctx* c, int param, int cost, int robust, DoneGate gate) {
  const int rot0 = param == PARAM_QUAT ? 0 : 3;
  const int nt = c->n_eval_tiles;
  if (!nt) return;
#define MV_EVALG(COSTK)                                                                                          \
  if (F32 && c->nor_f32) lm_eval_general_kernel<F32, F32, COSTK><<<nt, EVAL_THREADS, 0, c->stream>>>(        \
      c->d_frames.as<FrameDev>(), c->d_edges.as<EdgeDev>(), c->d_eval_tiles.as<Tile>(), c->eval_tile_len,       \
      c->d_corr.as<int32_t>(), c->d_gen.as<FrameGen>(), c->d_weight.as<float>(), robust, rot0, c->d_partial.as<double>(), gate); \
  else lm_eval_general_kernel<F32, false, COSTK><<<nt, EVAL_THREADS, 0, c->stream>>>(                        \
      c->d_frames.as<FrameDev>(), c->d_edges.as<EdgeDev>(), c->d_eval_tiles.as<Tile>(), c->eval_tile_len,       \
      c->d_corr.as<int32_t>(), c->d_gen.as<FrameGen>(), c->d_weight.as<float>(), robust, rot0, c->d_partial.as<double>(), gate)
  if (cost == COST_P2P) { MV_EVALG(COST_P2P); } else if (cost == COST_P2PLANE) { MV_EVALG(COST_P2PLANE); } else { MV_EVALG(COST_MIXED); }
#undef MV_EVALG
}

template <typename Kernel, typename Eval, typename Step>
static int run_steps(mvicp_ctx* c, Kernel kernel, int n, int64_t max_evals, const char* what, NormalLayout& lay, Eval&& eval, Step&& step) {
  const size_t l_bytes = sizeof(double) * (size_t)c->l_size;
  const size_t vec_bytes = sizeof(double) * 3 * (size_t)(n + 1);
  lay.l_in_smem = (l_bytes + vec_bytes) <= 220 * 1024 ? 1 : 0;
  const size_t dyn = vec_bytes + (lay.l_in_smem ? l_bytes : 0);
  CU(cudaFuncSetAttribute(kernel, cudaFuncAttributeMaxDynamicSharedMemorySize, 220 * 1024));
  for (int i = 0; i < 8; ++i) c->h_flag[i] = 0;
  c->eval_ev_used = 0;
  int64_t issued = 0, seen = 0;
  auto issue = [&]() -> int {
    if ((int)c->eval_ev.size() < c->eval_ev_used + 2) { cudaEvent_t a, b; CU(cudaEventCreate(&a)); CU(cudaEventCreate(&b)); c->eval_ev.push_back(a); c->eval_ev.push_back(b); }
    CU(cudaEventRecord(c->eval_ev[c->eval_ev_used], c->stream));
    eval();
    CU(cudaEventRecord(c->eval_ev[c->eval_ev_used + 1], c->stream));
    c->eval_ev_used += 2;
    lay.seq = (int32_t)(issued + 1);
    RET(step(dyn));
    ++issued;
    return MVICP_OK;
  };
  RET(issue());
  while (true) {
    if (issued - seen < 2 && issued <= max_evals) RET(issue());
    const int32_t want = (int32_t)(seen + 1);
    int32_t v;
    long spins = 0;
    while (((v = c->h_flag[want & 7]) >> 1) != want) {
      if ((++spins & 0xfffff) == 0 && cudaStreamQuery(c->stream) != cudaErrorNotReady) {
        v = c->h_flag[want & 7];
        if ((v >> 1) != want) { CU(cudaGetLastError()); return fail(MVICP_ERR_CUDA, "%s step %d never reported", what, want); }
        break;
      }
    }
    ++seen;
    if ((v & 1) != 0 || seen > max_evals) break;
  }
  return MVICP_OK;
}

static int read_back_solve(mvicp_ctx* c, void* state, const void* d_state, size_t bytes) {
  CU(cudaEventRecord(c->ev[4], c->stream));
  CU(cudaMemcpyAsync(state, d_state, bytes, cudaMemcpyDeviceToHost, c->stream));
  CU(cudaMemcpyAsync(c->h_poses.data(), c->d_poses.p, sizeof(double) * 16 * c->M, cudaMemcpyDeviceToHost, c->stream));
  CU(cudaStreamSynchronize(c->stream));
  CU(cudaGetLastError());
  c->ev_lm = true;
  return MVICP_OK;
}

static int refresh_if_fixed_changed(mvicp_ctx* c) {
  bool stale = false;
  for (int e = 0; e < c->E; ++e) if ((c->edge_owner[e] < 0) != (c->fixed[c->h_edges[e].src] != 0)) stale = true;
  if (!stale) return MVICP_OK;
  if (c->world > 1) return fail(MVICP_ERR_STATE, "sharded run: frame 0 was free when the edges were distributed; fix it (mvicp_set_poses) before mvicp_correspond");
  return refresh_after_fixed_change(c);
}

template <typename Solve>
static int run_pairwise(const mvicp_config* cfg, const double* src, const double* dst, const double* nor, int64_t n, double* pose16_out,
                        Solve&& solve) {
  mvicp_ctx* c = nullptr;
  RET(mvicp_create(cfg, &c));
  const double* pts[2] = {dst, src}; const double* nrs[2] = {nor, nor};
  const int64_t np[2] = {n, n};
  int rc = mvicp_set_frames(c, 2, pts, nor ? nrs : nullptr, np);
  const int32_t es = 1, ed = 0;
  if (rc == MVICP_OK) rc = mvicp_set_graph(c, 1, &es, &ed);
  if (rc == MVICP_OK) {
    std::vector<int32_t> id(n); std::iota(id.begin(), id.end(), 0);
    rc = mvicp_set_edge(c, 0, id.data(), id.data(), n, 1.0f);
  }
  if (rc == MVICP_OK) rc = solve(c);
  std::vector<double> poses(32);
  if (rc == MVICP_OK) rc = mvicp_get_poses(c, poses.data());
  if (rc == MVICP_OK) std::memcpy(pose16_out, poses.data() + 16, sizeof(double) * 16);
  const std::string keep = g_err;
  mvicp_destroy(c);
  g_err = keep;
  return rc;
}

static void summary_of_state(const LmState& st, mvicp_lm_summary* s) {
  s->termination = st.termination; s->num_iterations = st.iteration; s->num_successful_steps = st.n_success;
  s->num_evaluations = st.n_evals; s->num_linear_solves = st.n_solves; s->reserved = 0;
  s->initial_cost = st.initial_cost; s->final_cost = st.x_cost;
}
static void summary_no_unknowns(mvicp_lm_summary* s) { std::memset(s, 0, sizeof *s); s->termination = MVICP_TERM_GRADIENT_TOLERANCE; }

extern "C" {
int mvicp_optimize(mvicp_ctx* c, int32_t param, int32_t cost, int32_t robust, const mvicp_lm_options* opt_in, mvicp_lm_summary* summary) {
  if (!c || !c->M || !c->E) return fail(MVICP_ERR_STATE, "mvicp_optimize: frames and graph must be set first");
  if (param < 0 || param > 2 || cost < 0 || cost > 2) return fail(MVICP_ERR_INVALID, "mvicp_optimize: bad param/cost");
  if (cost != COST_P2P && !c->have_normals) return fail(MVICP_ERR_INVALID, "point-to-plane needs normals for every frame");
  CU(cudaSetDevice(c->device));
  const int M = c->M, E = c->E;
  c->fixed[0] = 1;
  c->h_col.assign(M, -1); int n = 0;
  for (int f = 0; f < M; ++f) if (!c->fixed[f]) { c->h_col[f] = n; n += 6; }
  c->n_free = n / 6;
  mvicp_lm_options opt; if (opt_in) opt = *opt_in; else mvicp_default_lm_options(&opt);
  if (n == 0) {
    if (summary) summary_no_unknowns(summary);
    return MVICP_OK;
  }
  RET(refresh_if_fixed_changed(c));
  std::vector<uint8_t> key(c->fixed); key.push_back((uint8_t)(c->graph_gen & 0xff)); key.push_back((uint8_t)((c->graph_gen >> 8) & 0xff));
  if (key != c->lm_key) {
    RET(c->d_state.reserve(sizeof(LmState)));
    RET(c->d_x.reserve(sizeof(double) * 7 * M)); RET(c->d_cand.reserve(sizeof(double) * 7 * M));
    RET(c->d_Rt.reserve(sizeof(Rt) * M)); RET(c->d_K.reserve(sizeof(double) * 36 * M));
    RET(c->d_Hc.reserve(sizeof(double) * n * n)); RET(c->d_gc.reserve(sizeof(double) * n)); RET(c->d_scale.reserve(sizeof(double) * n));
    RET(c->d_diag.reserve(sizeof(double) * n)); RET(c->d_step.reserve(sizeof(double) * n));
    CU(cudaMemsetAsync(c->d_Hc.p, 0, sizeof(double) * (size_t)n * n, c->stream));
    std::vector<uint8_t> active(E);
    for (int e = 0; e < E; ++e) active[e] = !c->fixed[c->h_edges[e].src];
    RET(build_normal_layout(c, n, active));
    c->lm_key = key;
  }
  LmState st; std::memset(&st, 0, sizeof st);
  st.opt = opt; st.param = param; st.cost_kind = cost; st.robust = robust ? 1 : 0; st.M = M; st.E = E; st.F = n / 6; st.n = n;
  st.G = ambient_size(param); st.radius = opt.initial_trust_region_radius; st.decrease_factor = 2.0;
  std::memcpy(c->h_state, &st, sizeof st);
  CU(cudaMemcpyAsync(c->d_state.p, c->h_state, sizeof st, cudaMemcpyHostToDevice, c->stream));

  LmWork w{};
  w.S = c->d_state.as<LmState>(); w.edges = c->d_edges.as<EdgeDev>(); w.eout = c->d_eout.as<double>();
  if (std::getenv("MVICP_STEP_PROFILE")) { RET(c->d_prof.reserve(sizeof(long long) * 64)); w.prof = c->d_prof.as<long long>(); }
  c->nonrigid = poses_nonrigid(c->h_poses.data(), M);
  const bool general = c->nonrigid && param != PARAM_AA;
  if (general) { RET(c->d_gen.reserve(sizeof(FrameGen) * M)); RET(c->d_partial.reserve(sizeof(double) * GBLK * std::max<size_t>(1, c->n_eval_tiles))); }
  w.G_eval = general ? c->d_gen.as<FrameGen>() : nullptr;
  w.x = c->d_x.as<double>(); w.cand = c->d_cand.as<double>(); w.Rt_eval = c->d_Rt.as<Rt>(); w.K_eval = c->d_K.as<double>();
  w.lay = c->lay; w.lay.poses16 = c->d_poses.as<double>();
  w.H = c->d_H.as<double>(); w.g = c->d_g.as<double>(); w.Hc = c->d_Hc.as<double>(); w.gc = c->d_gc.as<double>();
  w.scale = c->d_scale.as<double>(); w.diag = c->d_diag.as<double>(); w.step = c->d_step.as<double>();

  CU(cudaEventRecord(c->ev[3], c->stream));
  lm_init_kernel<<<(M + 63) / 64, 64, 0, c->stream>>>(w);
  c->stats.kernel_launches += 1;
  const int max_evals = opt.max_num_iterations + 2;
  const bool use_p2p = c->comm && c->world > 1 && c->p2p_ok && E <= mvicp_ctx::X_ECAP;
  const DoneGate done_flag{&w.S->done, nullptr, 0};
  auto eval = [&]() {
    if (general) { if (c->f32) launch_eval_general<true>(c, param, cost, st.robust, done_flag); else launch_eval_general<false>(c, param, cost, st.robust, done_flag); }
    else if (c->f32) launch_eval<true>(c, cost, st.robust, done_flag); else launch_eval<false>(c, cost, st.robust, done_flag);
  };
  auto step = [&](size_t dyn) -> int {
    PeerTable pt; std::memset(&pt, 0, sizeof pt); pt.world = 1; pt.rank = 0;
    double* eout_local = c->d_eout.as<double>();
    unsigned int* xcounter = nullptr;
    int xs = 0;
    if (use_p2p) {
      xs = ++c->xseq;
      const size_t half = (size_t)mvicp_ctx::X_ECAP * EOUT;
      pt.world = c->world; pt.rank = c->rank;
      for (int p = 0; p < c->world; ++p) {
        pt.eout[p] = (double*)c->peer_x[p] + (size_t)(xs & 1) * half;
        pt.flags[p] = (volatile int*)((double*)c->peer_x[p] + 2 * half);
      }
      eout_local = pt.eout[c->rank];
      xcounter = (unsigned int*)((double*)c->xbuf + 2 * half) + 32;
    }
    if (general)
      lm_edge_general_kernel<<<E, EDGE_THREADS, 0, c->stream>>>(c->d_edges.as<EdgeDev>(), c->d_edge_tile_begin.as<int32_t>(),
                                                                c->d_partial.as<double>(), eout_local, done_flag, pt, xs, xcounter);
    else
      lm_edge_kernel<<<E, EDGE_THREADS, 0, c->stream>>>(c->d_edges.as<EdgeDev>(), c->d_edge_tile_begin.as<int32_t>(), c->d_partial.as<double>(),
                                                        cost == COST_P2PLANE ? NBLK_PLANE : NBLK, c->d_Rt.as<Rt>(), c->d_K.as<double>(),
                                                        eout_local, done_flag, pt, xs, xcounter);
    if (c->comm && c->world > 1 && !use_p2p)
      NC(ncclAllReduce(c->d_eout.p, c->d_eout.p, (size_t)EOUT * E, ncclDouble, ncclSum, c->comm, c->stream));
    w.eout = eout_local; w.peer_flags = use_p2p ? pt.flags[c->rank] : nullptr; w.world = c->world; w.xseq = xs;
    lm_step_kernel<<<1, STEP_THREADS, dyn, c->stream>>>(w);
    c->stats.kernel_launches += (c->n_eval_tiles ? 1 : 0) + 2;
    return MVICP_OK;
  };
  RET(run_steps(c, lm_step_kernel, n, max_evals, "LM", w.lay, eval, step));
  if (c->comm && c->world > 1 && !use_p2p) {
    const int chunk = (M + c->world - 1) / c->world;
    RET(c->d_posegather.reserve(sizeof(double) * 16 * (size_t)chunk * c->world * 2));
    double* sendb = c->d_posegather.as<double>();
    double* recvb = sendb + (size_t)16 * chunk * c->world;
    CU(cudaMemsetAsync(sendb, 0, sizeof(double) * 16 * chunk, c->stream));
    int f0 = -1, f1 = -1;
    for (int f = 0; f < M; ++f) if (owner_of(c, f) == c->rank) { if (f0 < 0) f0 = f; f1 = f; }
    if (f0 >= 0) CU(cudaMemcpyAsync(sendb, c->d_poses.as<double>() + 16 * f0, sizeof(double) * 16 * (f1 - f0 + 1), cudaMemcpyDeviceToDevice, c->stream));
    NC(ncclAllGather(sendb, recvb, (size_t)16 * chunk, ncclDouble, c->comm, c->stream));
    for (int r = 0; r < c->world; ++r) {
      int a = -1, b = -1;
      for (int f = 0; f < M; ++f) if (owner_of(c, f) == r) { if (a < 0) a = f; b = f; }
      if (a >= 0) CU(cudaMemcpyAsync(c->d_poses.as<double>() + 16 * a, recvb + (size_t)16 * chunk * r, sizeof(double) * 16 * (b - a + 1), cudaMemcpyDeviceToDevice, c->stream));
    }
  }
  RET(read_back_solve(c, c->h_state, c->d_state.p, sizeof st));
  std::memcpy(&st, c->h_state, sizeof st);
  c->last_lm_iters = st.iteration;
  if (summary) summary_of_state(st, summary);
  if (st.nonrigid == 2) return fail(MVICP_ERR_NCCL, "a peer rank never delivered its pair matrices (peer-memory exchange timed out)");
  if (st.nonrigid && !general)
    return fail(MVICP_ERR_NONRIGID, "a pose's quaternion is not unit (non-rigid Isometry) but the unit-quaternion LM path was run");
  if (!st.done) return fail(MVICP_ERR_STATE, "LM loop did not terminate within %d evaluations", max_evals);
  return MVICP_OK;
}

}
static int graph_components(const mvicp_ctx* c, std::vector<int32_t>& comp) {
  std::vector<int32_t> up(c->M);
  std::iota(up.begin(), up.end(), 0);
  auto root = [&](int f) { while (up[f] != f) f = up[f] = up[up[f]]; return f; };
  for (const EdgeDev& e : c->h_edges) {
    const int a = root(e.src), b = root(e.dst);
    if (a != b) up[std::max(a, b)] = std::min(a, b);
  }
  comp.assign(c->M, -1);
  int n = 0;
  for (int f = 0; f < c->M; ++f) { const int r = root(f); comp[f] = r == f ? n++ : comp[r]; }
  return n;
}

static int build_component_layouts(mvicp_ctx* c, const std::vector<uint8_t>& key) {
  const int M = c->M, E = c->E;
  const int K = c->n_cmp = graph_components(c, c->cmp_of_frame);
  std::vector<std::vector<int32_t>> fr(K), ed(K);
  for (int f = 0; f < M; ++f) fr[c->cmp_of_frame[f]].push_back(f);
  for (int e = 0; e < E; ++e) ed[c->cmp_of_frame[c->h_edges[e].src]].push_back(e);
  std::vector<uint8_t> active(E);
  for (int e = 0; e < E; ++e) active[e] = !c->fixed[c->h_edges[e].src];
  c->h_col.assign(M, -1);
  c->cmp_prob.assign(K, -1); c->cmp_M.clear(); c->cmp_E.clear(); c->cmp_n.clear();
  std::vector<LayoutPlan> plans; std::vector<int32_t> pc;
  for (int k = 0; k < K; ++k) {
    int n = 0;
    for (int f : fr[k]) if (!c->fixed[f]) { c->h_col[f] = n; n += 6; }
    if (!n) continue;
    c->cmp_prob[k] = (int32_t)plans.size();
    plans.emplace_back();
    RET(plan_normal_layout(c, fr[k], ed[k], n, active, plans.back()));
    pc.push_back(k); c->cmp_n.push_back(n);
    c->cmp_M.push_back((int32_t)fr[k].size()); c->cmp_E.push_back((int32_t)ed[k].size());
  }
  const int P = c->n_prob = (int)plans.size();
  if (!P) { c->cmp_key = key; return MVICP_OK; }
  std::vector<int32_t> blob;
  auto put = [&](const std::vector<int32_t>& v) { const size_t o = blob.size(); blob.insert(blob.end(), v.begin(), v.end()); return o; };
  struct Off { size_t frame, edge, col, hb_ptr, hb_row, hb_col, hc_edge, hc_sub, gb_ptr, gc_edge, gc_side, rlast, rfirst, rowbase; };
  std::vector<Off> io(P);
  for (int q = 0; q < P; ++q) {
    const LayoutPlan& pl = plans[q];
    io[q] = Off{put(fr[pc[q]]), put(ed[pc[q]]), put(pl.col), put(pl.hb_ptr), put(pl.hb_row), put(pl.hb_col), put(pl.hc_edge), put(pl.hc_sub),
                put(pl.gb_ptr), put(pl.gc_edge), put(pl.gc_side), put(pl.rlast), put(pl.rfirst), put(pl.rowbase)};
  }
  std::vector<int32_t> prob_of_edge(E);
  for (int e = 0; e < E; ++e) prob_of_edge[e] = c->cmp_prob[c->cmp_of_frame[c->h_edges[e].src]];
  c->cmp_edge_map = put(prob_of_edge);
  std::vector<size_t> fo(P + 1, 0);
  for (int q = 0; q < P; ++q) { const size_t n = c->cmp_n[q]; fo[q + 1] = fo[q] + 2 * n * n + 6 * n + (size_t)plans[q].l_size; }
  RET(c->d_cmp_i32.reserve(sizeof(int32_t) * blob.size()));
  RET(c->d_cmp_f64.reserve(sizeof(double) * fo[P]));
  RET(c->d_cmp_prob.reserve(sizeof(LmProblem) * P));
  RET(c->d_cmp_state.reserve(sizeof(LmState) * (P + 1)));
  RET(c->d_cmp_ticket.reserve(sizeof(unsigned int)));
  const int32_t* ib = c->d_cmp_i32.as<int32_t>();
  std::vector<LmProblem> probs(P);
  size_t dyn = 0;
  for (int q = 0; q < P; ++q) {
    const int n = c->cmp_n[q]; const Off& o = io[q];
    LmProblem& p = probs[q];
    std::memset(&p, 0, sizeof p);
    p.S = c->d_cmp_state.as<LmState>() + q;
    p.frame = ib + o.frame; p.edge = ib + o.edge;
    NormalLayout& l = p.lay;
    l.col = ib + o.col;
    l.hb_ptr = ib + o.hb_ptr; l.hb_row = ib + o.hb_row; l.hb_col = ib + o.hb_col; l.hc_edge = ib + o.hc_edge; l.hc_sub = ib + o.hc_sub;
    l.n_hblocks = (int32_t)plans[q].hb_row.size();
    l.gb_ptr = ib + o.gb_ptr; l.gc_edge = ib + o.gc_edge; l.gc_side = ib + o.gc_side;
    l.rlast = ib + o.rlast; l.rfirst = ib + o.rfirst; l.rowbase = ib + o.rowbase;
    double* d = c->d_cmp_f64.as<double>() + fo[q];
    p.H = d; d += (size_t)n * n; p.Hc = d; d += (size_t)n * n;
    p.g = d; d += n; p.gc = d; d += n; p.scale = d; d += n; p.diag = d; d += n; p.step = d; d += n; l.rhs = d; d += n;
    l.Lg = d;
    const size_t vec = sizeof(double) * 3 * (size_t)(n + 1), lb = sizeof(double) * (size_t)plans[q].l_size;
    l.l_in_smem = lb + vec <= 220 * 1024 ? 1 : 0;
    dyn = std::max(dyn, vec + (l.l_in_smem ? lb : 0));
  }
  c->cmp_dyn = dyn;
  CU(cudaMemcpyAsync(c->d_cmp_i32.p, blob.data(), sizeof(int32_t) * blob.size(), cudaMemcpyHostToDevice, c->stream));
  CU(cudaMemcpyAsync(c->d_cmp_prob.p, probs.data(), sizeof(LmProblem) * P, cudaMemcpyHostToDevice, c->stream));
  CU(cudaMemsetAsync(c->d_cmp_f64.p, 0, sizeof(double) * fo[P], c->stream));
  CU(cudaMemsetAsync(c->d_cmp_ticket.p, 0, sizeof(unsigned int), c->stream));
  CU(cudaStreamSynchronize(c->stream));
  c->cmp_key = key;
  return MVICP_OK;
}

extern "C" {
int mvicp_get_components(mvicp_ctx* c, int32_t* n_components, int32_t* component_of_frame) {
  if (!c || !n_components) return fail(MVICP_ERR_INVALID, "mvicp_get_components: bad arguments");
  if (!c->M) return fail(MVICP_ERR_STATE, "mvicp_get_components: frames must be set first");
  std::vector<int32_t> comp;
  *n_components = graph_components(c, comp);
  if (component_of_frame) std::memcpy(component_of_frame, comp.data(), sizeof(int32_t) * c->M);
  return MVICP_OK;
}

int mvicp_optimize_components(mvicp_ctx* c, int32_t param, int32_t cost, int32_t robust, const mvicp_lm_options* opt_in,
                              mvicp_lm_summary* summaries) {
  if (!c || !c->M || !c->E) return fail(MVICP_ERR_STATE, "mvicp_optimize_components: frames and graph must be set first");
  if (param < 0 || param > 2 || cost < 0 || cost > 2) return fail(MVICP_ERR_INVALID, "mvicp_optimize_components: bad param/cost");
  if (cost != COST_P2P && !c->have_normals) return fail(MVICP_ERR_INVALID, "point-to-plane needs normals for every frame");
  if (c->world > 1) return fail(MVICP_ERR_STATE, "mvicp_optimize_components: the component solve runs on one GPU; this context is sharded");
  CU(cudaSetDevice(c->device));
  const int M = c->M, E = c->E;
  {
    std::vector<int32_t> comp;
    std::vector<uint8_t> seen(graph_components(c, comp), 0);
    for (int f = 0; f < M; ++f) if (!seen[comp[f]]) { seen[comp[f]] = 1; c->fixed[f] = 1; }
  }
  mvicp_lm_options opt; if (opt_in) opt = *opt_in; else mvicp_default_lm_options(&opt);
  if (std::all_of(c->fixed.begin(), c->fixed.end(), [](uint8_t v) { return v != 0; })) {
    if (summaries) { int32_t K = 0; RET(mvicp_get_components(c, &K, nullptr)); for (int k = 0; k < K; ++k) summary_no_unknowns(summaries + k); }
    return MVICP_OK;
  }
  RET(refresh_if_fixed_changed(c));
  std::vector<uint8_t> key(c->fixed); key.push_back((uint8_t)(c->graph_gen & 0xff)); key.push_back((uint8_t)((c->graph_gen >> 8) & 0xff));
  if (key != c->cmp_key) RET(build_component_layouts(c, key));
  const int P = c->n_prob;
  std::vector<LmState> st(P + 1);
  std::memset(st.data(), 0, sizeof(LmState) * (P + 1));
  for (int q = 0; q <= P; ++q) {
    LmState& s = st[q];
    s.opt = opt; s.param = param; s.cost_kind = cost; s.robust = robust ? 1 : 0; s.G = ambient_size(param);
    if (q == P) { s.M = M; s.E = E; continue; }
    s.M = c->cmp_M[q]; s.E = c->cmp_E[q]; s.n = c->cmp_n[q]; s.F = s.n / 6;
    s.radius = opt.initial_trust_region_radius; s.decrease_factor = 2.0;
  }
  LmState* dS = c->d_cmp_state.as<LmState>();
  CU(cudaMemcpyAsync(dS, st.data(), sizeof(LmState) * (P + 1), cudaMemcpyHostToDevice, c->stream));
  RET(c->d_x.reserve(sizeof(double) * 7 * M)); RET(c->d_cand.reserve(sizeof(double) * 7 * M));
  RET(c->d_Rt.reserve(sizeof(Rt) * M)); RET(c->d_K.reserve(sizeof(double) * 36 * M));
  RET(c->d_eout.reserve(sizeof(double) * EOUT * E));
  c->nonrigid = poses_nonrigid(c->h_poses.data(), M);
  const bool general = c->nonrigid && param != PARAM_AA;
  if (general) { RET(c->d_gen.reserve(sizeof(FrameGen) * M)); RET(c->d_partial.reserve(sizeof(double) * GBLK * std::max<size_t>(1, c->n_eval_tiles))); }
  LmWork w{};
  w.S = dS + P; w.edges = c->d_edges.as<EdgeDev>(); w.eout = c->d_eout.as<double>(); w.world = 1;
  w.x = c->d_x.as<double>(); w.cand = c->d_cand.as<double>(); w.Rt_eval = c->d_Rt.as<Rt>(); w.K_eval = c->d_K.as<double>();
  w.G_eval = general ? c->d_gen.as<FrameGen>() : nullptr;
  w.lay.poses16 = c->d_poses.as<double>(); w.lay.host_flag = c->d_flag;
  const LmProblem* probs = c->d_cmp_prob.as<LmProblem>();
  unsigned int* ticket = c->d_cmp_ticket.as<unsigned int>();

  CU(cudaEventRecord(c->ev[3], c->stream));
  lm_init_kernel<<<(M + 63) / 64, 64, 0, c->stream>>>(w);
  c->stats.kernel_launches += 1;
  const int max_evals = opt.max_num_iterations + 2;
  const DoneGate gate{&dS[0].done, c->d_cmp_i32.as<int32_t>() + c->cmp_edge_map, (int32_t)(sizeof(LmState) / sizeof(int))};
  auto eval = [&]() {
    if (general) { if (c->f32) launch_eval_general<true>(c, param, cost, st[0].robust, gate); else launch_eval_general<false>(c, param, cost, st[0].robust, gate); }
    else if (c->f32) launch_eval<true>(c, cost, st[0].robust, gate); else launch_eval<false>(c, cost, st[0].robust, gate);
  };
  auto step = [&](size_t) -> int {
    PeerTable pt; std::memset(&pt, 0, sizeof pt); pt.world = 1; pt.rank = 0;
    if (general)
      lm_edge_general_kernel<<<E, EDGE_THREADS, 0, c->stream>>>(c->d_edges.as<EdgeDev>(), c->d_edge_tile_begin.as<int32_t>(),
                                                                c->d_partial.as<double>(), c->d_eout.as<double>(), gate, pt, 0, nullptr);
    else
      lm_edge_kernel<<<E, EDGE_THREADS, 0, c->stream>>>(c->d_edges.as<EdgeDev>(), c->d_edge_tile_begin.as<int32_t>(), c->d_partial.as<double>(),
                                                        cost == COST_P2PLANE ? NBLK_PLANE : NBLK, c->d_Rt.as<Rt>(), c->d_K.as<double>(),
                                                        c->d_eout.as<double>(), gate, pt, 0, nullptr);
    lm_step_components_kernel<<<P, STEP_THREADS, c->cmp_dyn, c->stream>>>(w, probs, ticket);
    c->stats.kernel_launches += (c->n_eval_tiles ? 1 : 0) + 2;
    return MVICP_OK;
  };
  RET(run_steps(c, lm_step_components_kernel, 0, max_evals, "LM (components)", w.lay, eval, step));
  RET(read_back_solve(c, st.data(), dS, sizeof(LmState) * (P + 1)));
  int max_iters = 0; bool all_done = true;
  for (int q = 0; q < P; ++q) { max_iters = std::max(max_iters, (int)st[q].iteration); all_done = all_done && st[q].done; }
  c->last_lm_iters = max_iters;
  if (summaries)
    for (int k = 0; k < c->n_cmp; ++k) {
      if (c->cmp_prob[k] < 0) summary_no_unknowns(summaries + k);
      else summary_of_state(st[c->cmp_prob[k]], summaries + k);
    }
  if (st[P].nonrigid && !general)
    return fail(MVICP_ERR_NONRIGID, "a pose's quaternion is not unit (non-rigid Isometry) but the unit-quaternion LM path was run");
  if (!all_done) return fail(MVICP_ERR_STATE, "LM loop did not terminate within %d evaluations", max_evals);
  return MVICP_OK;
}

int mvicp_icp_round(mvicp_ctx* c, float thresh, int32_t param, int32_t cost, int32_t robust, const mvicp_lm_options* opt, mvicp_lm_summary* summary) {
  RET(mvicp_correspond(c, thresh));
  return mvicp_optimize(c, param, cost, robust, opt, summary);
}

int mvicp_pairwise(const mvicp_config* cfg, int32_t param, int32_t cost, const double* src, const double* dst, const double* nor,
                   int64_t n, const mvicp_lm_options* opt, double* pose16_out, mvicp_lm_summary* summary) {
  if (!src || !dst || n <= 0 || !pose16_out) return fail(MVICP_ERR_INVALID, "mvicp_pairwise: bad arguments");
  if (cost != MVICP_COST_P2P && !nor) return fail(MVICP_ERR_INVALID, "mvicp_pairwise: point-to-plane needs dst normals");
  return run_pairwise(cfg, src, dst, nor, n, pose16_out, [&](mvicp_ctx* c) { return mvicp_optimize(c, param, cost, 0, opt, summary); });
}

}
template <bool F32> static void launch_g2o_eval(mvicp_ctx* c, int cost, int nt, const G2oState* S, double eps) {
#define MV_G2O(NF, COSTK)                                                                                          \
  g2o_eval_kernel<F32, NF, COSTK><<<nt, EVAL_THREADS, 0, c->stream>>>(c->d_frames.as<FrameDev>(), c->d_edges.as<EdgeDev>(), \
      c->d_g2o_tiles.as<Tile>(), c->eval_tile_len, c->d_corr.as<int32_t>(), c->d_g2o_ev.as<Rt>(), S, eps, c->d_partial.as<double>())
  if (cost == COST_P2P) MV_G2O(F32, COST_P2P);
  else if (F32 && c->nor_f32) MV_G2O(F32, COST_P2PLANE);
  else MV_G2O(false, COST_P2PLANE);
#undef MV_G2O
}
static constexpr int G2O_TRACE_CAP = 65536;

extern "C" {
void mvicp_default_g2o_options(mvicp_g2o_options* o) {
  o->iterations_per_call = 100; o->max_calls = 100; o->no_improvement_limit = 5; o->max_trials = 10; o->orthonormalize_after = 1000;
  o->reserved = 0; o->tau = 1e-5; o->information_eps = 0.01;
}

int mvicp_optimize_g2o(mvicp_ctx* c, int32_t cost, const mvicp_g2o_options* opt_in, mvicp_g2o_summary* summary, double* chi2_per_call) {
  if (!c || !c->M || !c->E) return fail(MVICP_ERR_STATE, "mvicp_optimize_g2o: frames and graph must be set first");
  if (cost != COST_P2P && cost != COST_P2PLANE) return fail(MVICP_ERR_INVALID, "mvicp_optimize_g2o: cost must be point-to-point or point-to-plane");
  if (cost == COST_P2PLANE && !c->have_normals) return fail(MVICP_ERR_INVALID, "point-to-plane needs normals for every frame");
  if (c->world > 1) return fail(MVICP_ERR_STATE, "mvicp_optimize_g2o: the g2o solve runs on one GPU; this context is sharded");
  mvicp_g2o_options opt; if (opt_in) opt = *opt_in; else mvicp_default_g2o_options(&opt);
  if (opt.iterations_per_call < 1 || opt.max_calls < 1 || opt.max_trials < 1 || opt.no_improvement_limit < 0 || opt.orthonormalize_after < 0)
    return fail(MVICP_ERR_INVALID, "mvicp_optimize_g2o: bad options");
  CU(cudaSetDevice(c->device));
  const int M = c->M, E = c->E;
  c->fixed[0] = 1;
  RET(refresh_if_fixed_changed(c));
  const int tl = c->eval_tile_len;
  std::vector<Tile> tiles; std::vector<int32_t> tb(E + 1, 0);
  for (int e = 0; e < E; ++e) {
    tb[e] = (int32_t)tiles.size();
    const EdgeDev& ed = c->h_edges[e];
    if (c->fixed[ed.src] && c->fixed[ed.dst]) continue;
    for (int s = 0; s < ed.n_src; s += tl) tiles.push_back(Tile{e, s});
  }
  tb[E] = (int32_t)tiles.size();
  const int nt = (int)tiles.size();
  RET(c->d_g2o_tiles.reserve(sizeof(Tile) * std::max(1, nt)));
  RET(c->d_g2o_tile_begin.reserve(sizeof(int32_t) * (E + 1)));
  RET(c->d_g2o_cnt.reserve(sizeof(unsigned long long) * E));
  RET(c->d_partial.reserve(sizeof(double) * GBLK * std::max(1, nt)));
  if (nt) CU(cudaMemcpyAsync(c->d_g2o_tiles.p, tiles.data(), sizeof(Tile) * nt, cudaMemcpyHostToDevice, c->stream));
  CU(cudaMemcpyAsync(c->d_g2o_tile_begin.p, tb.data(), sizeof(int32_t) * (E + 1), cudaMemcpyHostToDevice, c->stream));
  CU(cudaMemsetAsync(c->d_g2o_cnt.p, 0, sizeof(unsigned long long) * E, c->stream));
  if (nt) {
    g2o_count_kernel<<<nt, 256, 0, c->stream>>>(c->d_edges.as<EdgeDev>(), c->d_g2o_tiles.as<Tile>(), tl, c->d_corr.as<int32_t>(),
                                                c->d_g2o_cnt.as<unsigned long long>());
    c->stats.kernel_launches += 1;
  }
  std::vector<unsigned long long> cnt(E);
  CU(cudaMemcpyAsync(cnt.data(), c->d_g2o_cnt.p, sizeof(unsigned long long) * E, cudaMemcpyDeviceToHost, c->stream));
  CU(cudaStreamSynchronize(c->stream));
  std::vector<uint8_t> touched(M, 0);
  for (int e = 0; e < E; ++e) if (cnt[e]) { touched[c->h_edges[e].src] = 1; touched[c->h_edges[e].dst] = 1; }
  c->h_col.assign(M, -1); int n = 0;
  for (int f = 0; f < M; ++f) if (touched[f] && !c->fixed[f]) { c->h_col[f] = n; n += 6; }
  if (summary) std::memset(summary, 0, sizeof *summary);
  c->g2o_trials = 0;
  if (n == 0) {
    if (summary) summary->ended = MVICP_G2O_END_NO_VERTICES;
    if (chi2_per_call) chi2_per_call[0] = 0.0;
    return MVICP_OK;
  }
  std::vector<uint8_t> active(E);
  for (int e = 0; e < E; ++e) active[e] = cnt[e] != 0;
  RET(build_normal_layout(c, n, active));
  c->lm_key.clear();
  RET(c->d_g2o_state.reserve(sizeof(G2oState)));
  RET(c->d_g2o_x.reserve(sizeof(Rt) * M)); RET(c->d_g2o_ev.reserve(sizeof(Rt) * M)); RET(c->d_g2o_nop.reserve(sizeof(int32_t) * M));
  RET(c->d_g2o_chi.reserve(sizeof(double) * (opt.max_calls + 1)));
  RET(c->d_g2o_trace.reserve(sizeof(double) * 5 * G2O_TRACE_CAP));
  G2oState st; std::memset(&st, 0, sizeof st);
  st.M = M; st.E = E; st.n = n; st.max_iter = opt.iterations_per_call; st.max_calls = opt.max_calls;
  st.no_impr_limit = opt.no_improvement_limit; st.max_trials = opt.max_trials; st.ortho_after = opt.orthonormalize_after;
  st.phase = G2O_BUILD; st.trace_cap = G2O_TRACE_CAP; st.tau = opt.tau;
  CU(cudaMemcpyAsync(c->d_g2o_state.p, &st, sizeof st, cudaMemcpyHostToDevice, c->stream));
  G2oState* dS = c->d_g2o_state.as<G2oState>();

  G2oWork w{};
  w.S = dS; w.eout = c->d_eout.as<double>();
  w.x = c->d_g2o_x.as<Rt>(); w.ev = c->d_g2o_ev.as<Rt>(); w.n_oplus = c->d_g2o_nop.as<int32_t>();
  w.lay = c->lay; w.lay.poses16 = c->d_poses.as<double>();
  w.H = c->d_H.as<double>(); w.g = c->d_g.as<double>();
  w.chi_calls = c->d_g2o_chi.as<double>(); w.trace = c->d_g2o_trace.as<double>();

  CU(cudaEventRecord(c->ev[3], c->stream));
  g2o_init_kernel<<<(M + 63) / 64, 64, 0, c->stream>>>(w, M);
  c->stats.kernel_launches += 1;
  const int64_t max_evals = (int64_t)opt.max_calls * opt.iterations_per_call * (opt.max_trials + 1) + 2;
  const double eps = opt.information_eps;
  auto eval = [&]() { if (c->f32) launch_g2o_eval<true>(c, cost, nt, dS, eps); else launch_g2o_eval<false>(c, cost, nt, dS, eps); };
  auto step = [&](size_t dyn) -> int {
    g2o_edge_kernel<<<E, EDGE_THREADS, 0, c->stream>>>(c->d_g2o_tile_begin.as<int32_t>(), c->d_partial.as<double>(), dS, c->d_eout.as<double>());
    g2o_step_kernel<<<1, STEP_THREADS, dyn, c->stream>>>(w);
    c->stats.kernel_launches += 3;
    return MVICP_OK;
  };
  RET(run_steps(c, g2o_step_kernel, n, max_evals, "g2o", w.lay, eval, step));
  RET(read_back_solve(c, &st, dS, sizeof st));
  if (chi2_per_call) CU(cudaMemcpy(chi2_per_call, c->d_g2o_chi.p, sizeof(double) * (st.call + 1), cudaMemcpyDeviceToHost));
  c->last_lm_iters = 1 << 20;
  c->g2o_trials = st.n_trace;
  if (summary) {
    summary->calls = st.call; summary->iterations = st.n_iters; summary->trials = st.n_trials; summary->accepted = st.n_accepted;
    summary->evaluations = st.n_evals; summary->ended = st.ended; summary->last_call_end = st.last_call_end;
    summary->chi2_initial = st.chi_initial; summary->chi2_final = st.last_chi;
  }
  if (!st.done) return fail(MVICP_ERR_STATE, "g2o solve did not terminate within %lld evaluations", (long long)max_evals);
  return MVICP_OK;
}

int mvicp_pairwise_g2o(const mvicp_config* cfg, int32_t cost, const double* src, const double* dst, const double* nor, int64_t n,
                       const mvicp_g2o_options* opt_in, double* pose16_out, mvicp_g2o_summary* summary) {
  if (!src || !dst || n <= 0 || !pose16_out) return fail(MVICP_ERR_INVALID, "mvicp_pairwise_g2o: bad arguments");
  if (cost != MVICP_COST_P2P && !nor) return fail(MVICP_ERR_INVALID, "mvicp_pairwise_g2o: point-to-plane needs dst normals");
  mvicp_g2o_options opt;
  if (opt_in) opt = *opt_in; else { mvicp_default_g2o_options(&opt); opt.iterations_per_call = 300; }
  opt.max_calls = 1;
  return run_pairwise(cfg, src, dst, nor, n, pose16_out, [&](mvicp_ctx* c) { return mvicp_optimize_g2o(c, cost, &opt, summary, nullptr); });
}

int mvicp_g2o_trace(mvicp_ctx* c, double* out5, int64_t capacity, int64_t* n_trials) {
  if (!c || capacity < 0 || (capacity && !out5)) return fail(MVICP_ERR_INVALID, "mvicp_g2o_trace: bad arguments");
  if (n_trials) *n_trials = c->g2o_trials;
  const int64_t k = std::min<int64_t>(capacity, std::min<int64_t>(c->g2o_trials, G2O_TRACE_CAP));
  if (k <= 0) return MVICP_OK;
  CU(cudaSetDevice(c->device));
  CU(cudaStreamSynchronize(c->stream));
  CU(cudaMemcpy(out5, c->d_g2o_trace.p, sizeof(double) * 5 * (size_t)k, cudaMemcpyDeviceToHost));
  return MVICP_OK;
}

static void host_eig_sym3(double A[3][3], double w[3], double V[3][3]) {
  for (int i = 0; i < 3; ++i) for (int j = 0; j < 3; ++j) V[i][j] = (i == j);
  for (int sweep = 0; sweep < 60; ++sweep) {
    if (A[0][1] * A[0][1] + A[0][2] * A[0][2] + A[1][2] * A[1][2] < 1e-300) break;
    for (int p = 0; p < 2; ++p) for (int q = p + 1; q < 3; ++q) {
      if (A[p][q] == 0.0) continue;
      const double th = (A[q][q] - A[p][p]) / (2.0 * A[p][q]);
      const double t = (th >= 0 ? 1.0 : -1.0) / (std::fabs(th) + std::sqrt(th * th + 1.0)), cs = 1.0 / std::sqrt(t * t + 1.0), sn = t * cs;
      for (int k = 0; k < 3; ++k) { const double a = A[k][p], b = A[k][q]; A[k][p] = cs * a - sn * b; A[k][q] = sn * a + cs * b; }
      for (int k = 0; k < 3; ++k) { const double a = A[p][k], b = A[q][k]; A[p][k] = cs * a - sn * b; A[q][k] = sn * a + cs * b; }
      for (int k = 0; k < 3; ++k) { const double a = V[k][p], b = V[k][q]; V[k][p] = cs * a - sn * b; V[k][q] = sn * a + cs * b; }
    }
  }
  for (int i = 0; i < 3; ++i) w[i] = A[i][i];
}

int mvicp_pairwise_closed(const mvicp_config* cfg, int32_t cost, const double* src, const double* dst, const double* nor, int64_t n,
                          double* pose16_out) {
  if (!src || !dst || n <= 0 || !pose16_out) return fail(MVICP_ERR_INVALID, "mvicp_pairwise_closed: bad arguments");
  if (cost != MVICP_COST_P2P && cost != MVICP_COST_P2PLANE) return fail(MVICP_ERR_INVALID, "mvicp_pairwise_closed: cost must be P2P or P2PLANE");
  if (cost == MVICP_COST_P2PLANE && !nor) return fail(MVICP_ERR_INVALID, "mvicp_pairwise_closed: point-to-plane needs dst normals");
  int ndev = 0;
  if (cudaGetDeviceCount(&ndev) != cudaSuccess || ndev <= 0) return fail(MVICP_ERR_CUDA, "no CUDA device; this engine has no CPU path");
  const int dev = cfg ? cfg->device : 0;
  if (dev < 0 || dev >= ndev) return fail(MVICP_ERR_INVALID, "mvicp_pairwise_closed: bad device %d", dev);
  CU(cudaSetDevice(dev));
  cudaStream_t st = cfg && cfg->stream ? (cudaStream_t)cfg->stream : nullptr;
  const size_t bytes = sizeof(double) * 3 * (size_t)n;
  const int grid = (int)std::min<int64_t>(2 * NUM_SMS, (n + CLOSED_THREADS - 1) / CLOSED_THREADS);
  double *d_src = nullptr, *d_dst = nullptr, *d_nor = nullptr, *d_part = nullptr, *d_aux = nullptr;
  std::vector<double> part((size_t)grid * CLOSED_MAXV);
  auto cleanup = [&]() { cudaFree(d_src); cudaFree(d_dst); cudaFree(d_nor); cudaFree(d_part); cudaFree(d_aux); };
#define CUX(x) do { cudaError_t e_ = (x); if (e_ != cudaSuccess) { cleanup(); return fail(MVICP_ERR_CUDA, "%s: %s", #x, cudaGetErrorString(e_)); } } while (0)
  CUX(cudaMalloc(&d_src, bytes)); CUX(cudaMalloc(&d_dst, bytes)); CUX(cudaMalloc(&d_part, sizeof(double) * part.size())); CUX(cudaMalloc(&d_aux, sizeof(double) * 6));
  CUX(cudaMemcpyAsync(d_src, src, bytes, cudaMemcpyHostToDevice, st)); CUX(cudaMemcpyAsync(d_dst, dst, bytes, cudaMemcpyHostToDevice, st));
  if (cost == MVICP_COST_P2PLANE) { CUX(cudaMalloc(&d_nor, bytes)); CUX(cudaMemcpyAsync(d_nor, nor, bytes, cudaMemcpyHostToDevice, st)); }
  auto fetch = [&](int nv, double* out) -> int {
    if (cudaMemcpyAsync(part.data(), d_part, sizeof(double) * part.size(), cudaMemcpyDeviceToHost, st) != cudaSuccess || cudaStreamSynchronize(st) != cudaSuccess) return 1;
    for (int i = 0; i < nv; ++i) { double s = 0; for (int b = 0; b < grid; ++b) s += part[(size_t)b * CLOSED_MAXV + i]; out[i] = s; }
    return 0;
  };
  for (int i = 0; i < 16; ++i) pose16_out[i] = 0.0;
  pose16_out[15] = 1.0;
  if (cost == MVICP_COST_P2P) {
    double sums[6], K9[9];
    closed_reduce_kernel<0><<<grid, CLOSED_THREADS, 0, st>>>(d_src, d_dst, nullptr, (long long)n, nullptr, d_part);
    if (fetch(6, sums)) { cleanup(); return fail(MVICP_ERR_CUDA, "mvicp_pairwise_closed: reduction failed: %s", cudaGetErrorString(cudaGetLastError())); }
    for (int i = 0; i < 6; ++i) sums[i] /= (double)n;
    CUX(cudaMemcpyAsync(d_aux, sums, sizeof sums, cudaMemcpyHostToDevice, st));
    closed_reduce_kernel<1><<<grid, CLOSED_THREADS, 0, st>>>(d_src, d_dst, nullptr, (long long)n, d_aux, d_part);
    if (fetch(9, K9)) { cleanup(); return fail(MVICP_ERR_CUDA, "mvicp_pairwise_closed: reduction failed: %s", cudaGetErrorString(cudaGetLastError())); }
    double S[3][3], w[3], V[3][3], R[3][3] = {{0, 0, 0}, {0, 0, 0}, {0, 0, 0}};
    for (int a = 0; a < 3; ++a) for (int b = 0; b < 3; ++b) { S[a][b] = 0; for (int k = 0; k < 3; ++k) S[a][b] += K9[3 * k + a] * K9[3 * k + b]; }
    host_eig_sym3(S, w, V);
    int ord[3] = {0, 1, 2};
    std::sort(ord, ord + 3, [&](int x, int y) { return w[x] > w[y]; });
    double U[3][3], Vs[3][3];
    for (int j = 0; j < 3; ++j) for (int a = 0; a < 3; ++a) Vs[a][j] = V[a][ord[j]];
    auto Kv = [&](int j, double out[3]) { for (int a = 0; a < 3; ++a) { out[a] = 0; for (int k = 0; k < 3; ++k) out[a] += K9[3 * a + k] * Vs[k][j]; } };
    auto nrm = [](const double v[3]) { return std::sqrt(v[0] * v[0] + v[1] * v[1] + v[2] * v[2]); };
    double u0[3], u1[3], u2[3];
    Kv(0, u0); const double s0 = nrm(u0);
    if (s0 > 0) { for (int a = 0; a < 3; ++a) u0[a] /= s0; } else { u0[0] = 1; u0[1] = u0[2] = 0; }
    Kv(1, u1);
    { const double d = u1[0] * u0[0] + u1[1] * u0[1] + u1[2] * u0[2]; for (int a = 0; a < 3; ++a) u1[a] -= d * u0[a]; }
    double s1 = nrm(u1);
    if (s1 > 1e-13 * s0 && s1 > 0) { for (int a = 0; a < 3; ++a) u1[a] /= s1; }
    else {
      const int m = std::fabs(u0[0]) <= std::fabs(u0[1]) ? (std::fabs(u0[0]) <= std::fabs(u0[2]) ? 0 : 2) : (std::fabs(u0[1]) <= std::fabs(u0[2]) ? 1 : 2);
      double e[3] = {0, 0, 0}; e[m] = 1;
      const double d = u0[m]; for (int a = 0; a < 3; ++a) u1[a] = e[a] - d * u0[a];
      s1 = nrm(u1); for (int a = 0; a < 3; ++a) u1[a] /= s1;
    }
    u2[0] = u0[1] * u1[2] - u0[2] * u1[1]; u2[1] = u0[2] * u1[0] - u0[0] * u1[2]; u2[2] = u0[0] * u1[1] - u0[1] * u1[0];
    {
      double k2[3]; Kv(2, k2);
      const double s2 = k2[0] * u2[0] + k2[1] * u2[1] + k2[2] * u2[2];
      const double detV = Vs[0][0] * (Vs[1][1] * Vs[2][2] - Vs[1][2] * Vs[2][1]) - Vs[0][1] * (Vs[1][0] * Vs[2][2] - Vs[1][2] * Vs[2][0]) +
                          Vs[0][2] * (Vs[1][0] * Vs[2][1] - Vs[1][1] * Vs[2][0]);
      const bool neg = std::fabs(s2) > 1e-13 * s0 ? s2 < 0 : detV < 0;
      if (neg) for (int a = 0; a < 3; ++a) u2[a] = -u2[a];
    }
    for (int a = 0; a < 3; ++a) { U[a][0] = u0[a]; U[a][1] = u1[a]; U[a][2] = u2[a]; }
    for (int a = 0; a < 3; ++a) for (int b = 0; b < 3; ++b) for (int j = 0; j < 3; ++j) R[a][b] += U[a][j] * Vs[b][j];
    const double det = R[0][0] * (R[1][1] * R[2][2] - R[1][2] * R[2][1]) - R[0][1] * (R[1][0] * R[2][2] - R[1][2] * R[2][0]) + R[0][2] * (R[1][0] * R[2][1] - R[1][1] * R[2][0]);
    if (det < 0) for (int a = 0; a < 3; ++a) R[a][2] = -R[a][2];
    for (int a = 0; a < 3; ++a) {
      for (int b = 0; b < 3; ++b) pose16_out[4 * b + a] = R[a][b];
      pose16_out[12 + a] = sums[3 + a] - (R[a][0] * sums[0] + R[a][1] * sums[1] + R[a][2] * sums[2]);
    }
    for (int i = 0; i < 16; ++i) if (!std::isfinite(pose16_out[i])) { cleanup(); return fail(MVICP_ERR_INVALID, "mvicp_pairwise_closed: non-finite result (non-finite input?)"); }
  } else {
    double v[27];
    closed_reduce_kernel<2><<<grid, CLOSED_THREADS, 0, st>>>(d_src, d_dst, d_nor, (long long)n, nullptr, d_part);
    if (fetch(27, v)) { cleanup(); return fail(MVICP_ERR_CUDA, "mvicp_pairwise_closed: reduction failed: %s", cudaGetErrorString(cudaGetLastError())); }
    double Cm[6][6], L[6][6] = {{0}}, D[6], y[6], x[6];
    { int k = 0; for (int r = 0; r < 6; ++r) for (int c2 = r; c2 < 6; ++c2) { Cm[r][c2] = v[k]; Cm[c2][r] = v[k]; ++k; } }
    for (int j = 0; j < 6; ++j) {
      double dj = Cm[j][j]; for (int k = 0; k < j; ++k) dj -= L[j][k] * L[j][k] * D[k];
      D[j] = dj; L[j][j] = 1;
      for (int i = j + 1; i < 6; ++i) { double u = Cm[i][j]; for (int k = 0; k < j; ++k) u -= L[i][k] * L[j][k] * D[k]; L[i][j] = u / dj; }
    }
    for (int i = 0; i < 6; ++i) { y[i] = v[21 + i]; for (int k = 0; k < i; ++k) y[i] -= L[i][k] * y[k]; }
    for (int i = 5; i >= 0; --i) { x[i] = y[i] / D[i]; for (int k = i + 1; k < 6; ++k) x[i] -= L[k][i] * x[k]; }
    const double ca = std::cos(x[0]), sa = std::sin(x[0]), cb = std::cos(x[1]), sb = std::sin(x[1]), cg = std::cos(x[2]), sg = std::sin(x[2]);
    const double R[3][3] = {{cb * cg, -cb * sg, sb}, {sa * sb * cg + ca * sg, -sa * sb * sg + ca * cg, -sa * cb}, {-ca * sb * cg + sa * sg, ca * sb * sg + sa * cg, ca * cb}};
    for (int a = 0; a < 3; ++a) { for (int b = 0; b < 3; ++b) pose16_out[4 * b + a] = R[a][b]; pose16_out[12 + a] = x[3 + a]; }
    for (int i = 0; i < 16; ++i) if (!std::isfinite(pose16_out[i])) { cleanup(); return fail(MVICP_ERR_INVALID, "mvicp_pairwise_closed: singular point-to-plane system (degenerate surface)"); }
  }
#undef CUX
  cleanup();
  return MVICP_OK;
}

int mvicp_recompute_normals(mvicp_ctx* c, int32_t k) {
  if (!c || !c->M) return fail(MVICP_ERR_STATE, "mvicp_recompute_normals: frames must be set first");
  if (k < 3 || k > KNN_MAXK) return fail(MVICP_ERR_INVALID, "mvicp_recompute_normals: k must be in [3, %d] (pointSetPCA asserts >= 3)", KNN_MAXK);
  CU(cudaSetDevice(c->device));
  CU(cudaStreamSynchronize(c->stream));
  c->nor_dbl.resize(c->M, nullptr);
  cudaEvent_t e0 = c->ev[5], e1 = c->ev[6];
  CU(cudaEventRecord(e0, c->stream));
  for (int f = 0; f < c->M; ++f) {
    const int n = (int)c->n_pts[f];
    if (!c->nor_dbl[f]) { CU(cudaMalloc(&c->nor_dbl[f], sizeof(double) * 3 * (size_t)n)); c->frame_allocs.push_back(c->nor_dbl[f]); }
    if (c->f32) normals_kernel<true><<<(n + 127) / 128, 128, 0, c->stream>>>(c->d_frames.as<FrameDev>(), f, k, (double*)c->nor_dbl[f], nullptr);
    else normals_kernel<false><<<(n + 127) / 128, 128, 0, c->stream>>>(c->d_frames.as<FrameDev>(), f, k, (double*)c->nor_dbl[f], nullptr);
    void* rec = nullptr;
    if (c->nor_f32 || !c->h_frames[f].nor_o) { CU(cudaMalloc(&rec, sizeof(double4a) * (size_t)n)); c->frame_allocs.push_back(rec); }
    else rec = const_cast<void*>(c->h_frames[f].nor_o);
    pack_normals_kernel<<<(n + 255) / 256, 256, 0, c->stream>>>((const double*)c->nor_dbl[f], n, (double4a*)rec);
    c->h_frames[f].nor_o = rec;
    c->stats.kernel_launches += 2;
  }
  CU(cudaEventRecord(e1, c->stream));
  CU(cudaMemcpyAsync(c->d_frames.p, c->h_frames.data(), sizeof(FrameDev) * c->M, cudaMemcpyHostToDevice, c->stream));
  CU(cudaStreamSynchronize(c->stream));
  CU(cudaGetLastError());
  cudaEventElapsedTime(&c->normals_ms, e0, e1);
  c->nor_f32 = false; c->have_normals = true;
  return MVICP_OK;
}

int mvicp_get_normals(mvicp_ctx* c, int32_t frame, double* nor_xyz, float* elapsed_ms) {
  if (!c || frame < 0 || frame >= c->M || !nor_xyz) return fail(MVICP_ERR_INVALID, "mvicp_get_normals: bad arguments");
  if ((int)c->nor_dbl.size() <= frame || !c->nor_dbl[frame]) return fail(MVICP_ERR_STATE, "mvicp_get_normals: call mvicp_recompute_normals first");
  CU(cudaSetDevice(c->device));
  CU(cudaMemcpy(nor_xyz, c->nor_dbl[frame], sizeof(double) * 3 * (size_t)c->n_pts[frame], cudaMemcpyDeviceToHost));
  if (elapsed_ms) *elapsed_ms = c->normals_ms;
  return MVICP_OK;
}

int mvicp_knn_self(mvicp_ctx* c, int32_t frame, int32_t k, int32_t* nn_idx) {
  if (!c || frame < 0 || frame >= c->M || !nn_idx || k < 1 || k > KNN_MAXK) return fail(MVICP_ERR_INVALID, "mvicp_knn_self: bad arguments");
  CU(cudaSetDevice(c->device));
  const int n = (int)c->n_pts[frame];
  double* d_nor = nullptr; int32_t* d_nn = nullptr;
  CU(cudaMalloc(&d_nor, sizeof(double) * 3 * (size_t)n)); CU(cudaMalloc(&d_nn, sizeof(int32_t) * (size_t)k * n));
  if (c->f32) normals_kernel<true><<<(n + 127) / 128, 128, 0, c->stream>>>(c->d_frames.as<FrameDev>(), frame, k, d_nor, d_nn);
  else normals_kernel<false><<<(n + 127) / 128, 128, 0, c->stream>>>(c->d_frames.as<FrameDev>(), frame, k, d_nor, d_nn);
  c->stats.kernel_launches += 1;
  CU(cudaMemcpyAsync(nn_idx, d_nn, sizeof(int32_t) * (size_t)k * n, cudaMemcpyDeviceToHost, c->stream));
  CU(cudaStreamSynchronize(c->stream));
  cudaFree(d_nor); cudaFree(d_nn);
  CU(cudaGetLastError());
  return MVICP_OK;
}

int mvicp_get_normals_device(mvicp_ctx* c, int32_t frame, double* nor_xyz) {
  if (!c || frame < 0 || frame >= c->M || !nor_xyz) return fail(MVICP_ERR_INVALID, "mvicp_get_normals_device: bad arguments");
  if ((int)c->nor_dbl.size() <= frame || !c->nor_dbl[frame]) return fail(MVICP_ERR_STATE, "mvicp_get_normals_device: call mvicp_recompute_normals first");
  CU(cudaSetDevice(c->device));
  RET(check_device_ptr(c, nor_xyz, "mvicp_get_normals_device", "nor_xyz"));
  CU(cudaMemcpyAsync(nor_xyz, c->nor_dbl[frame], sizeof(double) * 3 * (size_t)c->n_pts[frame], cudaMemcpyDeviceToDevice, c->stream));
  return MVICP_OK;
}

int mvicp_knn_self_device(mvicp_ctx* c, int32_t frame, int32_t k, int32_t* nn_idx) {
  if (!c || frame < 0 || frame >= c->M || !nn_idx || k < 1 || k > KNN_MAXK) return fail(MVICP_ERR_INVALID, "mvicp_knn_self_device: bad arguments");
  CU(cudaSetDevice(c->device));
  RET(check_device_ptr(c, nn_idx, "mvicp_knn_self_device", "nn_idx"));
  const int n = (int)c->n_pts[frame];
  RET(c->d_knn_nor.reserve(sizeof(double) * 3 * (size_t)n));
  if (c->f32) normals_kernel<true><<<(n + 127) / 128, 128, 0, c->stream>>>(c->d_frames.as<FrameDev>(), frame, k, c->d_knn_nor.as<double>(), nn_idx);
  else normals_kernel<false><<<(n + 127) / 128, 128, 0, c->stream>>>(c->d_frames.as<FrameDev>(), frame, k, c->d_knn_nor.as<double>(), nn_idx);
  c->stats.kernel_launches += 1;
  CU(cudaGetLastError());
  return MVICP_OK;
}

int mvicp_nccl_unique_id(void* out128) {
  if (!out128) return fail(MVICP_ERR_INVALID, "mvicp_nccl_unique_id: null");
  static_assert(sizeof(ncclUniqueId) == 128, "ncclUniqueId is 128 bytes");
  ncclUniqueId id; NC(ncclGetUniqueId(&id));
  std::memcpy(out128, &id, 128);
  return MVICP_OK;
}

int mvicp_comm_init(mvicp_ctx* c, const void* id128, int32_t rank, int32_t world) {
  if (!c || !id128 || world < 1 || rank < 0 || rank >= world) return fail(MVICP_ERR_INVALID, "mvicp_comm_init: bad arguments");
  CU(cudaSetDevice(c->device));
  if (c->comm) { ncclCommDestroy(c->comm); c->comm = nullptr; }
  ncclUniqueId id; std::memcpy(&id, id128, 128);
  if (world > 1) NC(ncclCommInitRank(&c->comm, world, id, rank));
  c->rank = rank; c->world = world;
  c->p2p_ok = false;
  if (world > 1 && world <= MAX_PEERS && !(c->flags & MVICP_FLAG_NCCL_ONLY)) {
    const size_t xbytes = sizeof(double) * 2 * (size_t)mvicp_ctx::X_ECAP * EOUT + 256;
    bool ok = true;
    if (!c->xbuf) ok = cudaMalloc(&c->xbuf, xbytes) == cudaSuccess;
    if (ok) ok = cudaMemset(c->xbuf, 0, xbytes) == cudaSuccess;
    cudaIpcMemHandle_t mine; std::memset(&mine, 0, sizeof mine);
    if (ok) ok = cudaIpcGetMemHandle(&mine, c->xbuf) == cudaSuccess;
    void* d_h = nullptr;
    std::vector<cudaIpcMemHandle_t> all(world);
    int32_t okflag = ok ? 1 : 0;
    if (cudaMalloc(&d_h, sizeof(cudaIpcMemHandle_t) * (world + 1) + 64) != cudaSuccess) return fail(MVICP_ERR_CUDA, "comm_init: cudaMalloc");
    char* dh = (char*)d_h;
    struct Guard { void* p; ~Guard() { cudaFree(p); } } guard{d_h};
    CU(cudaMemcpy(dh, &mine, sizeof mine, cudaMemcpyHostToDevice));
    NC(ncclAllGather(dh, dh + sizeof(cudaIpcMemHandle_t), sizeof(cudaIpcMemHandle_t), ncclUint8, c->comm, c->stream));
    CU(cudaStreamSynchronize(c->stream));
    CU(cudaMemcpy(all.data(), dh + sizeof(cudaIpcMemHandle_t), sizeof(cudaIpcMemHandle_t) * world, cudaMemcpyDeviceToHost));
    for (int p = 0; p < world && ok; ++p) {
      if (p == rank) { c->peer_x[p] = c->xbuf; continue; }
      if (!c->peer_x[p]) ok = cudaIpcOpenMemHandle(&c->peer_x[p], all[p], cudaIpcMemLazyEnablePeerAccess) == cudaSuccess;
    }
    cudaGetLastError();
    okflag = ok ? 1 : 0;
    int32_t* d_ok = (int32_t*)(dh + sizeof(cudaIpcMemHandle_t) * (world + 1));
    CU(cudaMemcpy(d_ok, &okflag, sizeof okflag, cudaMemcpyHostToDevice));
    NC(ncclAllReduce(d_ok, d_ok, 1, ncclInt32, ncclMin, c->comm, c->stream));
    CU(cudaStreamSynchronize(c->stream));
    CU(cudaMemcpy(&okflag, d_ok, sizeof okflag, cudaMemcpyDeviceToHost));
    c->p2p_ok = okflag == 1;
    c->xseq = 0;
  }
  return rebuild_work(c);
}

int mvicp_get_stats(mvicp_ctx* c, mvicp_stats* out) {
  if (!c || !out) return fail(MVICP_ERR_INVALID, "mvicp_get_stats: bad arguments");
  CU(cudaSetDevice(c->device));
  CU(cudaStreamSynchronize(c->stream));
  if (c->ev_knn) {
    cudaEventElapsedTime(&c->stats.knn_ms, c->ev[0], c->ev[1]);
    cudaEventElapsedTime(&c->stats.select_ms, c->ev[1], c->ev[2]);
    c->stats.correspond_ms = c->stats.knn_ms + c->stats.select_ms;
  }
  if (c->ev_lm) {
    cudaEventElapsedTime(&c->stats.optimize_ms, c->ev[3], c->ev[4]);
    float acc = 0.f;
    for (int i = 0; i + 1 < c->eval_ev_used; i += 2) { float ms = 0.f; cudaEventElapsedTime(&ms, c->eval_ev[i], c->eval_ev[i + 1]); acc += ms; }
    c->stats.lm_eval_ms = acc; c->stats.lm_other_ms = c->stats.optimize_ms - acc;
  }
  if (c->E && fetch_edge_meta(c) == MVICP_OK) {
    int64_t s = 0; for (int e = 0; e < c->E; ++e) if (c->h_edges[e].owned) s += (int64_t)c->h_count[e];
    c->stats.correspondences = s;
  }
  c->stats.select_guess_rounds = c->sel_guess_rounds;
  c->stats.cert_rounds = c->cert_rounds;
  if (c->d_cert_cnt.p && c->E) {
    std::vector<unsigned long long> h(c->E);
    CU(cudaMemcpy(h.data(), c->d_cert_cnt.p, sizeof(unsigned long long) * c->E, cudaMemcpyDeviceToHost));
    int64_t s = 0; for (unsigned long long v : h) s += (int64_t)v;
    c->stats.cert_reused = s;
  }
  if (c->d_sel_cnt.p && c->E) {
    unsigned int miss = 0;
    CU(cudaMemcpy(&miss, c->d_sel_cnt.as<unsigned int>() + 2 * (size_t)c->E, sizeof miss, cudaMemcpyDeviceToHost));
    c->stats.select_guess_misses = miss;
  }
  *out = c->stats;
  return MVICP_OK;
}
int mvicp_debug_step_profile(mvicp_ctx* c, long long* out64) {
  if (!c || !out64 || !c->d_prof.p) return fail(MVICP_ERR_STATE, "mvicp_debug_step_profile: run with MVICP_STEP_PROFILE=1");
  CU(cudaSetDevice(c->device));
  CU(cudaMemcpy(out64, c->d_prof.p, sizeof(long long) * 64, cudaMemcpyDeviceToHost));
  return MVICP_OK;
}
int mvicp_get_stream(mvicp_ctx* c, void** stream) { if (!c || !stream) return fail(MVICP_ERR_INVALID, "bad arguments"); *stream = (void*)c->stream; return MVICP_OK; }
int mvicp_sync(mvicp_ctx* c) { if (!c) return fail(MVICP_ERR_INVALID, "null ctx"); CU(cudaSetDevice(c->device)); CU(cudaStreamSynchronize(c->stream)); return MVICP_OK; }

}
```

Measured before the change: 553.8.

## Replace skyline Cholesky with level-scheduled block-sparse Cholesky using nested dissection

Replaces the envelope/skyline Cholesky in the LM and g2o step kernels with a 6x6 block-sparse supernodal factorization. A host-side planner orders the frame graph by nested dissection, computes symbolic fill, and groups columns into elimination-tree levels so that independent block columns are factored in parallel with one barrier per level rather than per column. The plan can be held in shared memory, and the factor storage becomes compact 36-double blocks. This adds host planning cost and indirection, and performance depends on the pose graph's sparsity and tree depth.

```diff
diff --git a/mv_lm_icp_b200/csrc/block_plan.h b/mv_lm_icp_b200/csrc/block_plan.h
--- /dev/null
+++ b/mv_lm_icp_b200/csrc/block_plan.h
@@ -0,0 +1,130 @@
+#pragma once
+#include <algorithm>
+#include <cstdint>
+#include <utility>
+#include <vector>
+
+namespace mv {
+
+enum { BP_NB = 0, BP_NLEV, BP_NBLK, BP_NUPD, BP_PERM, BP_LEV, BP_COLP, BP_BROW, BP_BCOL, BP_UPDP, BP_UPD, BP_HEADER };
+
+struct BlockPlan {
+  std::vector<int32_t> words;
+  int64_t l_size = 0;
+};
+
+namespace bp_detail {
+inline void nd_order(const std::vector<std::vector<int>>& adj, const std::vector<int>& nodes, std::vector<int>& out) {
+  const int nb = (int)adj.size();
+  if (nodes.size() <= 2) { out.insert(out.end(), nodes.begin(), nodes.end()); return; }
+  std::vector<char> in(nb, 0);
+  for (const int v : nodes) in[v] = 1;
+  std::vector<int> d(nb, -1);
+  auto bfs = [&](int s) {
+    std::fill(d.begin(), d.end(), -1);
+    std::vector<int> q{s};
+    d[s] = 0;
+    for (size_t h = 0; h < q.size(); ++h)
+      for (const int u : adj[q[h]]) if (in[u] && d[u] < 0) { d[u] = d[q[h]] + 1; q.push_back(u); }
+    return q;
+  };
+  std::vector<int> reach = bfs(nodes[0]);
+  if (reach.size() < nodes.size()) {
+    std::vector<char> done(nb, 0);
+    for (const int s : nodes) {
+      if (done[s]) continue;
+      std::vector<int> comp = bfs(s);
+      for (const int v : comp) done[v] = 1;
+      std::sort(comp.begin(), comp.end());
+      nd_order(adj, comp, out);
+    }
+    return;
+  }
+  reach = bfs(reach.back());
+  const int depth = d[reach.back()];
+  if (depth < 2) { out.insert(out.end(), nodes.begin(), nodes.end()); return; }
+  std::vector<int> count(depth + 1, 0);
+  for (const int v : nodes) count[d[v]] += 1;
+  int m = 0, below = 0;
+  while (m < depth - 1 && 2 * (below + count[m]) < (int)nodes.size()) below += count[m++];
+  m = std::max(m, 1);
+  std::vector<int> a, b, sep;
+  for (const int v : nodes) {
+    if (d[v] > m) { b.push_back(v); continue; }
+    bool cut = false;
+    if (d[v] == m) for (const int u : adj[v]) cut = cut || (in[u] && d[u] == m + 1);
+    (cut ? sep : a).push_back(v);
+  }
+  nd_order(adj, a, out);
+  nd_order(adj, b, out);
+  out.insert(out.end(), sep.begin(), sep.end());
+}
+
+inline void symbolic(const std::vector<std::vector<int>>& adj, const std::vector<int>& order, std::vector<std::vector<int>>& rows,
+                     std::vector<int>& level) {
+  const int nb = (int)adj.size();
+  std::vector<int> pos(nb);
+  for (int k = 0; k < nb; ++k) pos[order[k]] = k;
+  std::vector<std::vector<int>> kids(nb);
+  rows.assign(nb, {}); level.assign(nb, 0);
+  for (int k = 0; k < nb; ++k) {
+    std::vector<int>& r = rows[k];
+    for (const int u : adj[order[k]]) if (pos[u] > k) r.push_back(pos[u]);
+    for (const int c : kids[k]) {
+      for (const int i : rows[c]) if (i > k) r.push_back(i);
+      level[k] = std::max(level[k], level[c] + 1);
+    }
+    std::sort(r.begin(), r.end());
+    r.erase(std::unique(r.begin(), r.end()), r.end());
+    if (!r.empty()) kids[r[0]].push_back(k);
+  }
+}
+}
+
+inline BlockPlan plan_block_cholesky(int nb, const std::vector<std::pair<int, int>>& links) {
+  using namespace bp_detail;
+  std::vector<std::vector<int>> adj(nb);
+  for (const auto& e : links) if (e.first != e.second) { adj[e.first].push_back(e.second); adj[e.second].push_back(e.first); }
+  for (auto& a : adj) { std::sort(a.begin(), a.end()); a.erase(std::unique(a.begin(), a.end()), a.end()); }
+  std::vector<int> all(nb), nd, order;
+  for (int i = 0; i < nb; ++i) all[i] = i;
+  nd_order(adj, all, nd);
+  std::vector<std::vector<int>> rows;
+  std::vector<int> level;
+  symbolic(adj, nd, rows, level);
+  std::vector<int> idx(nb);
+  for (int k = 0; k < nb; ++k) idx[k] = k;
+  std::stable_sort(idx.begin(), idx.end(), [&](int x, int y) { return level[x] < level[y]; });
+  for (int k = 0; k < nb; ++k) order.push_back(nd[idx[k]]);
+  symbolic(adj, order, rows, level);
+  const int nlev = nb ? level[nb - 1] + 1 : 0;
+  std::vector<int32_t> lev(nlev + 1, nb), colp{0}, brow, bcol, updp{0}, upd;
+  for (int k = nb - 1; k >= 0; --k) lev[level[k]] = k;
+  for (int k = 0; k < nb; ++k) {
+    brow.push_back(k); bcol.push_back(k);
+    for (const int i : rows[k]) { brow.push_back(i); bcol.push_back(k); }
+    colp.push_back((int32_t)brow.size());
+  }
+  auto block = [&](int i, int k) {
+    return (int32_t)(std::lower_bound(brow.begin() + colp[k] + 1, brow.begin() + colp[k + 1], i) - brow.begin()) - (i == k ? 1 : 0);
+  };
+  std::vector<std::vector<int>> rowof(nb);
+  for (int j = 0; j < nb; ++j) for (const int i : rows[j]) rowof[i].push_back(j);
+  for (int b = 0; b < (int)brow.size(); ++b) {
+    const int i = brow[b], k = bcol[b];
+    for (const int j : rowof[k])
+      if (i == k || std::binary_search(rows[j].begin(), rows[j].end(), i)) { upd.push_back(block(i, j)); upd.push_back(block(k, j)); }
+    updp.push_back((int32_t)(upd.size() / 2));
+  }
+  BlockPlan p;
+  std::vector<int32_t>& w = p.words;
+  w.assign(BP_HEADER, 0);
+  w[BP_NB] = nb; w[BP_NLEV] = nlev; w[BP_NBLK] = (int32_t)brow.size(); w[BP_NUPD] = (int32_t)(upd.size() / 2);
+  auto put = [&](int slot, const std::vector<int32_t>& v) { w[slot] = (int32_t)w.size(); w.insert(w.end(), v.begin(), v.end()); };
+  put(BP_PERM, std::vector<int32_t>(order.begin(), order.end()));
+  put(BP_LEV, lev); put(BP_COLP, colp); put(BP_BROW, brow); put(BP_BCOL, bcol); put(BP_UPDP, updp); put(BP_UPD, upd);
+  p.l_size = 36 * (int64_t)brow.size() + 6 * (int64_t)nb;
+  return p;
+}
+
+}
diff --git a/mv_lm_icp_b200/csrc/g2o.cuh b/mv_lm_icp_b200/csrc/g2o.cuh
--- a/mv_lm_icp_b200/csrc/g2o.cuh
+++ b/mv_lm_icp_b200/csrc/g2o.cuh
@@ -236,8 +236,8 @@
   const int n = S->n, M = S->M, E = S->E;
   const int phase = S->phase;
   const NormalLayout& lay = w.lay;
-  double* colj = smem; double* dg = smem + 2 * (n + 1);
-  double* L = lay.l_in_smem ? smem + 3 * (n + 1) : lay.Lg;
+  const StepSmem sm = step_smem(lay, n, smem);
+  double* L = sm.L;
 
   const double chi_eval = edge_cost_sum(w.eout, E, red);
 
@@ -301,13 +301,10 @@
 
   while (s_solve) {
     const double lambda = S->lambda;
-    for (int i = tid >> 5; i < n; i += T >> 5) {
-      const int rbi = lay.rowbase[i];
-      for (int j = lay.rfirst[i] + (tid & 31); j <= i; j += 32) L[rbi + j] = w.H[(size_t)i * n + j] + (i == j ? lambda : 0.0);
-    }
-    { const int rbn = lay.rowbase[n]; for (int j = tid; j < n; j += T) L[rbn + j] = -w.g[j]; }
+    load_system(sm.plan, L, [&](int i, int j) { return w.H[(size_t)i * n + j] + (i == j ? lambda : 0.0); },
+                [&](int j) { return -w.g[j]; });
     __syncthreads();
-    bool ok = chol_solve(L, lay.rowbase, n, colj, dg, lay.rhs, lay.rlast, lay.rfirst);
+    bool ok = chol_solve(sm.plan, L, sm.dinv, lay.rhs);
     double bad = 0.0;
     if (ok) for (int j = tid; j < n; j += T) if (!isfinite(lay.rhs[j])) bad = 1.0;
     bad = block_sum(bad, red);
diff --git a/mv_lm_icp_b200/csrc/lm_step.cuh b/mv_lm_icp_b200/csrc/lm_step.cuh
--- a/mv_lm_icp_b200/csrc/lm_step.cuh
+++ b/mv_lm_icp_b200/csrc/lm_step.cuh
@@ -1,6 +1,7 @@
 #pragma once
 #include <cuda_runtime.h>
 #include "../../include/mvicp.h"
+#include "block_plan.h"
 #include "se3_math.cuh"
 #include "types.cuh"
 
@@ -20,10 +21,10 @@
   const int32_t* col;
   const int32_t* hb_ptr; const int32_t* hb_row; const int32_t* hb_col; const int32_t* hc_edge; const int32_t* hc_sub; int32_t n_hblocks;
   const int32_t* gb_ptr; const int32_t* gc_edge; const int32_t* gc_side;
-  const int32_t* rlast; const int32_t* rfirst;
-  const int32_t* rowbase;
+  const int32_t* plan;
+  int32_t plan_words;
   double *Lg, *rhs;
-  int32_t l_in_smem;
+  int32_t plan_in_smem, l_in_smem;
   double* poses16;
   volatile int32_t* host_flag;
   int32_t seq;
@@ -130,147 +131,167 @@
   if (w.G_eval && S->param != PARAM_AA) frame_general(S->param, x, &w.G_eval[f]);
 }
 
-__device__ __forceinline__ void chol_factor_diag(double* L, const int32_t* rb, int j0, double* dinv, volatile int* s_ok, int lane) {
-  double D[6][6], inv[6];
-#pragma unroll
-  for (int i = 0; i < 6; ++i)
-#pragma unroll
-    for (int k = 0; k <= i; ++k) D[i][k] = L[rb[j0 + i] + j0 + k];
-  bool okb = true;
-#pragma unroll
-  for (int k = 0; k < 6; ++k) {
-    double d = D[k][k];
-#pragma unroll
-    for (int m = 0; m < k; ++m) d -= D[k][m] * D[k][m];
-    if (!(d > 0.0) || !isfinite(d)) okb = false;
-    inv[k] = rsqrt(d); D[k][k] = d * inv[k];
-#pragma unroll
-    for (int i = k + 1; i < 6; ++i) {
-      double v = D[i][k];
-#pragma unroll
-      for (int m = 0; m < k; ++m) v -= D[i][m] * D[k][m];
-      D[i][k] = v * inv[k];
-    }
-  }
-  __syncwarp();
-  if (lane == 0) {
-    if (!okb) *s_ok = 0;
-#pragma unroll
-    for (int i = 0; i < 6; ++i) {
-#pragma unroll
-      for (int k = 0; k <= i; ++k) L[rb[j0 + i] + j0 + k] = D[i][k];
-      dinv[j0 + i] = inv[i];
-    }
-  }
-}
-
-__device__ bool chol_solve(double* L, const int32_t* __restrict__ rowbase, int n, double* scratch, double* dinv, double* y,
-                           const int32_t* __restrict__ rlast, const int32_t* __restrict__ rfirst, long long* prof = nullptr) {
-  const int T = blockDim.x, tid = threadIdx.x, lane = tid & 31, wid = tid >> 5, nw = T >> 5;
-  int32_t* s_rfirst = reinterpret_cast<int32_t*>(scratch);
-  int32_t* s_rlast = s_rfirst + n;
-  int32_t* rb = s_rlast + n;
-  volatile int* s_ok = reinterpret_cast<volatile int*>(rb + n + 1);
-  for (int i = tid; i < n; i += T) { s_rfirst[i] = rfirst[i]; s_rlast[i] = rlast[i]; }
-  for (int i = tid; i <= n; i += T) rb[i] = rowbase[i];
-  if (tid == 0) *s_ok = 1;
-  __syncthreads();
-  const int NB = n / 6;
-  if (wid == 0) chol_factor_diag(L, rb, 0, dinv, s_ok, lane);
-  __syncthreads();
-  long long t_panel = 0, t_ahead = 0, t_bar = 0;
-  for (int J = 0; J < NB; ++J) {
-    if (!*s_ok) return false;
+struct StepSmem { double* dinv; const int32_t* plan; double* L; };
+__device__ __forceinline__ StepSmem step_smem(const NormalLayout& lay, int n, double* smem) {
+  int32_t* ps = reinterpret_cast<int32_t*>(smem + n + 1);
+  if (lay.plan_in_smem) for (int i = threadIdx.x; i < lay.plan_words; i += blockDim.x) ps[i] = lay.plan[i];
+  const int pd = lay.plan_in_smem ? (lay.plan_words + 1) / 2 : 0;
+  return {smem, lay.plan_in_smem ? ps : lay.plan, lay.l_in_smem ? smem + n + 1 + pd : lay.Lg};
+}
+
+template <typename A, typename B>
+__device__ __forceinline__ void load_system(const int32_t* __restrict__ pw, double* L, A a_of, B b_of) {
+  const int nb = pw[BP_NB], nblk = pw[BP_NBLK];
+  const int32_t *perm = pw + pw[BP_PERM], *brow = pw + pw[BP_BROW], *bcol = pw + pw[BP_BCOL];
+  for (int idx = threadIdx.x; idx < 36 * nblk; idx += blockDim.x) {
+    const int b = idx / 36, e = idx - 36 * b, i = e / 6, j = e - 6 * i;
+    if (brow[b] == bcol[b] && j > i) continue;
+    const int r = 6 * perm[brow[b]] + i, c = 6 * perm[bcol[b]] + j;
+    L[idx] = r >= c ? a_of(r, c) : a_of(c, r);
+  }
+  double* z = L + 36 * nblk;
+  for (int idx = threadIdx.x; idx < 6 * nb; idx += blockDim.x) z[idx] = b_of(6 * perm[idx / 6] + idx % 6);
+}
+
+__device__ bool chol_solve(const int32_t* __restrict__ pw, double* L, double* dinv, double* y, long long* prof = nullptr) {
+  __shared__ int s_ok;
+  const int tid = threadIdx.x, T = blockDim.x, lane = tid & 31, wid = tid >> 5, nw = T >> 5;
+  const int nb = pw[BP_NB], nlev = pw[BP_NLEV], nblk = pw[BP_NBLK];
+  const int32_t *perm = pw + pw[BP_PERM], *lev = pw + pw[BP_LEV], *colp = pw + pw[BP_COLP], *brow = pw + pw[BP_BROW],
+                *bcol = pw + pw[BP_BCOL], *updp = pw + pw[BP_UPDP], *upd = pw + pw[BP_UPD];
+  double* z = L + 36 * (size_t)nblk;
+  if (tid == 0) s_ok = 1;
+  __syncthreads();
+  long long t_upd = 0, t_fac = 0;
+  for (int l = 0; l < nlev; ++l) {
+    const int k0 = lev[l], k1 = lev[l + 1];
     const long long c0 = prof ? clock64() : 0;
-    const int j0 = 6 * J;
-    const int rl = s_rlast[j0 + 5];
-    const int nrows = rl - (j0 + 5) + 1;
-    for (int q = tid; q < nrows; q += T) {
-      const int r = (q == nrows - 1) ? n : j0 + 6 + q;
-      if (r < n && s_rfirst[r] > j0 + 5) continue;
-      double* row = L + rb[r] + j0;
-      double v[6];
-#pragma unroll
-      for (int k = 0; k < 6; ++k) {
-        double a = row[k];
-#pragma unroll
-        for (int m = 0; m < k; ++m) a -= v[m] * L[rb[j0 + k] + j0 + m];
-        v[k] = a * dinv[j0 + k];
-      }
-#pragma unroll
-      for (int k = 0; k < 6; ++k) row[k] = v[k];
+    if (l > 0) {
+      const int b0 = colp[k0], nt = 36 * (colp[k1] - b0);
+      for (int q = tid; q < nt + 6 * (k1 - k0); q += T) {
+        if (q < nt) {
+          const int b = b0 + q / 36, e = q % 36, a = e / 6, c = e - 6 * a;
+          if (brow[b] == bcol[b] && c > a) continue;
+          double v = L[36 * b + e];
+          for (int u = updp[b]; u < updp[b + 1]; ++u) {
+            const double* li = L + 36 * upd[2 * u] + 6 * a;
+            const double* lk = L + 36 * upd[2 * u + 1] + 6 * c;
+#pragma unroll
+            for (int m = 0; m < 6; ++m) v -= li[m] * lk[m];
+          }
+          L[36 * b + e] = v;
+        } else {
+          const int r = q - nt, k = k0 + r / 6, a = r % 6, bd = colp[k];
+          double v = z[6 * k + a];
+          for (int u = updp[bd]; u < updp[bd + 1]; ++u) {
+            const int bkj = upd[2 * u];
+            const double* li = L + 36 * bkj + 6 * a;
+            const double* zj = z + 6 * bcol[bkj];
+#pragma unroll
+            for (int m = 0; m < 6; ++m) v -= li[m] * zj[m];
+          }
+          z[6 * k + a] = v;
+        }
+      }
+      __syncthreads();
     }
     const long long c1 = prof ? clock64() : 0;
-    __syncthreads();
-    const long long c2 = prof ? clock64() : 0;
-    const bool next = J + 1 < NB;
-    if (wid == 0 && next) {
-      const int b0 = j0 + 6;
-      if (lane < 21 && s_rfirst[b0] <= j0 + 5) {
-        int i = 0, rem = lane; while (rem > i) { rem -= i + 1; ++i; }
-        const int k = rem;
-        double* row = L + rb[b0 + i]; const double* lc = L + rb[b0 + k] + j0;
-        double a = row[b0 + k];
-#pragma unroll
-        for (int m = 0; m < 6; ++m) a -= row[j0 + m] * lc[m];
-        row[b0 + k] = a;
+    for (int k = k0 + wid; k < k1; k += nw) {
+      const int bd = colp[k], nrow = 6 * (colp[k + 1] - bd - 1);
+      double* Bd = L + 36 * bd;
+      double D[6][6], inv[6];
+#pragma unroll
+      for (int i = 0; i < 6; ++i)
+#pragma unroll
+        for (int m = 0; m <= i; ++m) D[i][m] = Bd[6 * i + m];
+      bool okb = true;
+#pragma unroll
+      for (int kk = 0; kk < 6; ++kk) {
+        double d = D[kk][kk];
+#pragma unroll
+        for (int m = 0; m < kk; ++m) d -= D[kk][m] * D[kk][m];
+        if (!(d > 0.0) || !isfinite(d)) okb = false;
+        inv[kk] = rsqrt(d); D[kk][kk] = d * inv[kk];
+#pragma unroll
+        for (int i = kk + 1; i < 6; ++i) {
+          double v = D[i][kk];
+#pragma unroll
+          for (int m = 0; m < kk; ++m) v -= D[i][m] * D[kk][m];
+          D[i][kk] = v * inv[kk];
+        }
       }
       __syncwarp();
-      chol_factor_diag(L, rb, b0, dinv, s_ok, lane);
-    } else {
-      const int w0 = next ? 1 : 0, wn = next ? nw - 1 : nw;
-      const int qfirst = next ? 6 : 0;
-      for (int q = qfirst + (wid - w0); q < nrows; q += wn) {
-        const int r = (q == nrows - 1) ? n : j0 + 6 + q;
-        if (r < n && s_rfirst[r] > j0 + 5) continue;
-        double* row = L + rb[r];
-        double lr[6];
-#pragma unroll
-        for (int k = 0; k < 6; ++k) lr[k] = row[j0 + k];
-        const int cend = min(r, rl);
-        for (int c = j0 + 6 + lane; c <= cend; c += 32) {
-          if (s_rfirst[c] > j0 + 5) continue;
-          const double* lc = L + rb[c] + j0;
-          double a = row[c];
-#pragma unroll
-          for (int k = 0; k < 6; ++k) a -= lr[k] * lc[k];
-          row[c] = a;
+      for (int q = lane; q <= nrow; q += 32) {
+        double* row = q < nrow ? Bd + 36 + 6 * q : z + 6 * k;
+        double v[6];
+#pragma unroll
+        for (int kk = 0; kk < 6; ++kk) {
+          double a = row[kk];
+#pragma unroll
+          for (int m = 0; m < kk; ++m) a -= v[m] * D[kk][m];
+          v[kk] = a * inv[kk];
         }
-      }
-    }
-    const long long c3 = prof ? clock64() : 0;
-    __syncthreads();
-    if (prof) { const long long c4 = clock64(); t_panel += c1 - c0; t_ahead += c3 - c2; t_bar += (c2 - c1) + (c4 - c3); }
-  }
-  if (prof && tid == 0) { prof[8] = t_panel; prof[9] = t_ahead; prof[10] = t_bar; }
-  if (!*s_ok) return false;
-  for (int i = tid; i < n; i += T) y[i] = L[rb[n] + i];
-  __syncthreads();
-  if (wid == 0) {
-    for (int J = NB - 1; J >= 0; --J) {
-      const int j0 = 6 * J;
+#pragma unroll
+        for (int kk = 0; kk < 6; ++kk) row[kk] = v[kk];
+      }
+      if (lane == 0) {
+        if (!okb) s_ok = 0;
+#pragma unroll
+        for (int i = 0; i < 6; ++i) {
+#pragma unroll
+          for (int m = 0; m <= i; ++m) Bd[6 * i + m] = D[i][m];
+          dinv[6 * k + i] = inv[i];
+        }
+      }
+    }
+    __syncthreads();
+    if (prof) { const long long c2 = clock64(); t_upd += c1 - c0; t_fac += c2 - c1; }
+    if (!s_ok) return false;
+  }
+  const long long c3 = prof ? clock64() : 0;
+  for (int l = nlev - 1; l >= 0; --l) {
+    for (int k = lev[l] + wid; k < lev[l + 1]; k += nw) {
+      const int bd = colp[k];
+      double* zk = z + 6 * k;
+      if (lane < 6) {
+        double a = zk[lane];
+        for (int b = bd + 1; b < colp[k + 1]; ++b) {
+          const double* lb = L + 36 * b + lane;
+          const double* xi = z + 6 * brow[b];
+#pragma unroll
+          for (int m = 0; m < 6; ++m) a -= lb[6 * m] * xi[m];
+        }
+        zk[lane] = a;
+      }
+      __syncwarp();
+      const double* Bd = L + 36 * bd;
       double x[6];
 #pragma unroll
-      for (int k = 5; k >= 0; --k) {
-        double a = y[j0 + k];
-#pragma unroll
-        for (int m = k + 1; m < 6; ++m) a -= L[rb[j0 + m] + j0 + k] * x[m];
-        x[k] = a * dinv[j0 + k];
+      for (int kk = 5; kk >= 0; --kk) {
+        double a = zk[kk];
+#pragma unroll
+        for (int m = kk + 1; m < 6; ++m) a -= Bd[6 * m + kk] * x[m];
+        x[kk] = a * dinv[6 * k + kk];
       }
       __syncwarp();
 #pragma unroll
-      for (int k = 0; k < 6; ++k) if (lane == k) y[j0 + k] = x[k];
-      for (int i = s_rfirst[j0] + lane; i < j0; i += 32) {
-        double a = y[i];
-#pragma unroll
-        for (int k = 0; k < 6; ++k) a -= L[rb[j0 + k] + i] * x[k];
-        y[i] = a;
-      }
-      __syncwarp();
-    }
-  }
+      for (int kk = 0; kk < 6; ++kk) if (lane == kk) zk[kk] = x[kk];
+    }
+    __syncthreads();
+  }
+  for (int idx = tid; idx < 6 * nb; idx += T) y[6 * perm[idx / 6] + idx % 6] = z[idx];
+  if (prof && tid == 0) { prof[8] = t_upd; prof[9] = t_fac; prof[10] = clock64() - c3; }
   __syncthreads();
   return true;
+}
+
+__global__ void __launch_bounds__(STEP_THREADS) block_solve_kernel(NormalLayout lay, const double* A, const double* b, int n, int* ok) {
+  extern __shared__ double smem[];
+  const StepSmem sm = step_smem(lay, n, smem);
+  load_system(lay.plan, sm.L, [&](int i, int j) { return A[(size_t)i * n + j]; }, [&](int j) { return b[j]; });
+  __syncthreads();
+  const bool r = chol_solve(sm.plan, sm.L, sm.dinv, lay.rhs);
+  if (threadIdx.x == 0) *ok = r ? 1 : 0;
 }
 
 template <bool COMP>
@@ -298,8 +319,8 @@
     }
     __syncthreads();
   }
-  double* colj = smem; double* dg = smem + 2 * (S->n + 1);
-  double* L = lay.l_in_smem ? smem + 3 * (S->n + 1) : lay.Lg;
+  const StepSmem sm = step_smem(lay, n, smem);
+  double* L = sm.L;
 
   gather_blocks(lay, w.eout, n, p.Hc);
   gather_gradient(lay, w.eout, M, p.gc);
@@ -391,19 +412,16 @@
         p.diag[j] = fmin(fmax(d, S->opt.min_lm_diagonal), S->opt.max_lm_diagonal);
       }
     __syncthreads();
-    for (int i = tid >> 5; i < n; i += T >> 5) {
-      const double si = p.scale[i];
-      const int rbi = lay.rowbase[i];
-      for (int j = lay.rfirst[i] + (tid & 31); j <= i; j += 32) {
-        double v = si * p.H[(size_t)i * n + j] * p.scale[j];
-        if (i == j) { const double ldg = sqrt(p.diag[i] / radius); v += ldg * ldg; }
-        L[rbi + j] = v;
-      }
-    }
-    { const int rbn = lay.rowbase[n]; for (int j = tid; j < n; j += T) L[rbn + j] = p.scale[j] * p.g[j]; }
+    load_system(sm.plan, L,
+                [&](int i, int j) {
+                  double v = p.scale[i] * p.H[(size_t)i * n + j] * p.scale[j];
+                  if (i == j) { const double ldg = sqrt(p.diag[i] / radius); v += ldg * ldg; }
+                  return v;
+                },
+                [&](int j) { return p.scale[j] * p.g[j]; });
     __syncthreads();
     MV_STAMP(3);
-    bool ok = chol_solve(L, lay.rowbase, n, colj, dg, lay.rhs, lay.rlast, lay.rfirst, prof);
+    bool ok = chol_solve(sm.plan, L, sm.dinv, lay.rhs, prof);
     MV_STAMP(4);
     double bad = 0.0;
     if (ok) for (int j = tid; j < n; j += T) if (!isfinite(lay.rhs[j])) bad = 1.0;
diff --git a/mv_lm_icp_b200/csrc/mvicp.cu b/mv_lm_icp_b200/csrc/mvicp.cu
--- a/mv_lm_icp_b200/csrc/mvicp.cu
+++ b/mv_lm_icp_b200/csrc/mvicp.cu
@@ -110,7 +110,7 @@
   bool nonrigid = false;
   std::vector<float> h_weight; std::vector<unsigned long long> h_count;
   DevBuf d_state, d_x, d_cand, d_Rt, d_K, d_col, d_H, d_g, d_Hc, d_gc, d_scale, d_diag, d_L, d_rhs, d_step,
-      d_eout, d_hb_ptr, d_hb_row, d_hb_col, d_hc_edge, d_hc_sub, d_gb_ptr, d_gc_edge, d_gc_side, d_posegather, d_rlast, d_rfirst, d_rowbase, d_gen;
+      d_eout, d_hb_ptr, d_hb_row, d_hb_col, d_hc_edge, d_hc_sub, d_gb_ptr, d_gc_edge, d_gc_side, d_posegather, d_plan, d_gen;
   int64_t l_size = 0;
   int n_free = 0;
   NormalLayout lay{};
@@ -991,7 +991,7 @@
 }
 
 struct LayoutPlan {
-  std::vector<int32_t> col, hb_ptr{0}, hb_row, hb_col, hc_edge, hc_sub, gb_ptr{0}, gc_edge, gc_side, rlast, rfirst, rowbase;
+  std::vector<int32_t> col, hb_ptr{0}, hb_row, hb_col, hc_edge, hc_sub, gb_ptr{0}, gc_edge, gc_side, plan;
   int64_t l_size = 0;
 };
 static int plan_normal_layout(const mvicp_ctx* c, const std::vector<int32_t>& frames, const std::vector<int32_t>& edges, int n,
@@ -1019,20 +1019,13 @@
       p.hb_ptr.push_back((int32_t)p.hc_edge.size());
     }
   for (int f = 0; f < M; ++f) { for (auto& pr : gl[f]) { p.gc_edge.push_back(pr.first); p.gc_side.push_back(pr.second); } p.gb_ptr.push_back((int32_t)p.gc_edge.size()); }
-  const int n_hblocks = (int)p.hb_row.size();
-  std::vector<int32_t>& rfirst = p.rfirst; std::vector<int32_t>& rlast = p.rlast;
-  rfirst.resize(n); rlast.resize(n);
-  for (int r = 0; r < n; ++r) rfirst[r] = (r / 6) * 6;
-  for (int b = 0; b < n_hblocks; ++b)
-    if (p.hb_col[b] < p.hb_row[b]) for (int i = 0; i < 6; ++i) rfirst[p.hb_row[b] + i] = std::min(rfirst[p.hb_row[b] + i], p.hb_col[b]);
-  for (int j = 0; j < n; ++j) { rlast[j] = j; }
-  for (int r = 0; r < n; ++r) for (int j = rfirst[r]; j <= r; ++j) rlast[j] = std::max(rlast[j], r);
-  for (int j = 1; j < n; ++j) rlast[j] = std::max(rlast[j], rlast[j - 1]);
-  p.rowbase.resize(n + 1); int64_t at = 0;
-  for (int r = 0; r < n; ++r) { p.rowbase[r] = (int32_t)(at - rfirst[r]); at += r - rfirst[r] + 1; }
-  p.rowbase[n] = (int32_t)at; at += n;
-  if (at > INT32_MAX) return fail(MVICP_ERR_INVALID, "normal matrix too large");
-  p.l_size = at;
+  std::vector<std::pair<int, int>> links;
+  for (size_t b = 0; b < p.hb_row.size(); ++b)
+    if (p.hb_row[b] > p.hb_col[b]) links.push_back({p.hb_row[b] / 6, p.hb_col[b] / 6});
+  BlockPlan bp = plan_block_cholesky(n / 6, links);
+  if (bp.l_size > INT32_MAX || bp.words.size() > (size_t)INT32_MAX) return fail(MVICP_ERR_INVALID, "normal matrix too large");
+  p.plan = std::move(bp.words);
+  p.l_size = bp.l_size;
   return MVICP_OK;
 }
 
@@ -1051,11 +1044,9 @@
   RET(up(c->d_hb_ptr, pl.hb_ptr)); RET(up(c->d_hb_row, pl.hb_row)); RET(up(c->d_hb_col, pl.hb_col)); RET(up(c->d_hc_edge, pl.hc_edge));
   RET(up(c->d_hc_sub, pl.hc_sub)); RET(up(c->d_gb_ptr, pl.gb_ptr)); RET(up(c->d_gc_edge, pl.gc_edge)); RET(up(c->d_gc_side, pl.gc_side));
   RET(up(c->d_col, pl.col));
-  RET(up(c->d_rlast, pl.rlast)); RET(up(c->d_rfirst, pl.rfirst));
-  const int64_t at = pl.l_size;
-  c->l_size = at;
-  RET(c->d_L.reserve(sizeof(double) * (size_t)at));
-  RET(up(c->d_rowbase, pl.rowbase));
+  RET(up(c->d_plan, pl.plan));
+  c->l_size = pl.l_size;
+  RET(c->d_L.reserve(sizeof(double) * (size_t)pl.l_size));
   RET(c->d_H.reserve(sizeof(double) * n * n)); RET(c->d_g.reserve(sizeof(double) * n)); RET(c->d_rhs.reserve(sizeof(double) * n));
   RET(c->d_eout.reserve(sizeof(double) * EOUT * E));
   CU(cudaMemsetAsync(c->d_H.p, 0, sizeof(double) * (size_t)n * n, c->stream));
@@ -1065,7 +1056,7 @@
   l.hb_ptr = c->d_hb_ptr.as<int32_t>(); l.hb_row = c->d_hb_row.as<int32_t>(); l.hb_col = c->d_hb_col.as<int32_t>();
   l.hc_edge = c->d_hc_edge.as<int32_t>(); l.hc_sub = c->d_hc_sub.as<int32_t>(); l.n_hblocks = n_hblocks;
   l.gb_ptr = c->d_gb_ptr.as<int32_t>(); l.gc_edge = c->d_gc_edge.as<int32_t>(); l.gc_side = c->d_gc_side.as<int32_t>();
-  l.rlast = c->d_rlast.as<int32_t>(); l.rfirst = c->d_rfirst.as<int32_t>(); l.rowbase = c->d_rowbase.as<int32_t>();
+  l.plan = c->d_plan.as<int32_t>(); l.plan_words = (int32_t)pl.plan.size();
   l.Lg = c->d_L.as<double>(); l.rhs = c->d_rhs.as<double>(); l.host_flag = c->d_flag;
   return MVICP_OK;
 }
@@ -1098,12 +1089,18 @@
 #undef MV_EVALG
 }
 
+static size_t step_smem_bytes(int n, size_t plan_words, int64_t l_size, NormalLayout& lay) {
+  const size_t limit = 220 * 1024, vec = sizeof(double) * (size_t)(n + 1);
+  const size_t pb = sizeof(double) * ((plan_words + 1) / 2), lb = sizeof(double) * (size_t)l_size;
+  lay.plan_in_smem = vec + pb <= limit ? 1 : 0;
+  const size_t used = vec + (lay.plan_in_smem ? pb : 0);
+  lay.l_in_smem = used + lb <= limit ? 1 : 0;
+  return used + (lay.l_in_smem ? lb : 0);
+}
+
 template <typename Kernel, typename Eval, typename Step>
 static int run_steps(mvicp_ctx* c, Kernel kernel, int n, int64_t max_evals, const char* what, NormalLayout& lay, Eval&& eval, Step&& step) {
-  const size_t l_bytes = sizeof(double) * (size_t)c->l_size;
-  const size_t vec_bytes = sizeof(double) * 3 * (size_t)(n + 1);
-  lay.l_in_smem = (l_bytes + vec_bytes) <= 220 * 1024 ? 1 : 0;
-  const size_t dyn = vec_bytes + (lay.l_in_smem ? l_bytes : 0);
+  const size_t dyn = step_smem_bytes(n, (size_t)lay.plan_words, c->l_size, lay);
   CU(cudaFuncSetAttribute(kernel, cudaFuncAttributeMaxDynamicSharedMemorySize, 220 * 1024));
   for (int i = 0; i < 8; ++i) c->h_flag[i] = 0;
   c->eval_ev_used = 0;
@@ -1343,12 +1340,12 @@
   if (!P) { c->cmp_key = key; return MVICP_OK; }
   std::vector<int32_t> blob;
   auto put = [&](const std::vector<int32_t>& v) { const size_t o = blob.size(); blob.insert(blob.end(), v.begin(), v.end()); return o; };
-  struct Off { size_t frame, edge, col, hb_ptr, hb_row, hb_col, hc_edge, hc_sub, gb_ptr, gc_edge, gc_side, rlast, rfirst, rowbase; };
+  struct Off { size_t frame, edge, col, hb_ptr, hb_row, hb_col, hc_edge, hc_sub, gb_ptr, gc_edge, gc_side, plan; };
   std::vector<Off> io(P);
   for (int q = 0; q < P; ++q) {
     const LayoutPlan& pl = plans[q];
     io[q] = Off{put(fr[pc[q]]), put(ed[pc[q]]), put(pl.col), put(pl.hb_ptr), put(pl.hb_row), put(pl.hb_col), put(pl.hc_edge), put(pl.hc_sub),
-                put(pl.gb_ptr), put(pl.gc_edge), put(pl.gc_side), put(pl.rlast), put(pl.rfirst), put(pl.rowbase)};
+                put(pl.gb_ptr), put(pl.gc_edge), put(pl.gc_side), put(pl.plan)};
   }
   std::vector<int32_t> prob_of_edge(E);
   for (int e = 0; e < E; ++e) prob_of_edge[e] = c->cmp_prob[c->cmp_of_frame[c->h_edges[e].src]];
@@ -1374,14 +1371,12 @@
     l.hb_ptr = ib + o.hb_ptr; l.hb_row = ib + o.hb_row; l.hb_col = ib + o.hb_col; l.hc_edge = ib + o.hc_edge; l.hc_sub = ib + o.hc_sub;
     l.n_hblocks = (int32_t)plans[q].hb_row.size();
     l.gb_ptr = ib + o.gb_ptr; l.gc_edge = ib + o.gc_edge; l.gc_side = ib + o.gc_side;
-    l.rlast = ib + o.rlast; l.rfirst = ib + o.rfirst; l.rowbase = ib + o.rowbase;
+    l.plan = ib + o.plan; l.plan_words = (int32_t)plans[q].plan.size();
     double* d = c->d_cmp_f64.as<double>() + fo[q];
     p.H = d; d += (size_t)n * n; p.Hc = d; d += (size_t)n * n;
     p.g = d; d += n; p.gc = d; d += n; p.scale = d; d += n; p.diag = d; d += n; p.step = d; d += n; l.rhs = d; d += n;
     l.Lg = d;
-    const size_t vec = sizeof(double) * 3 * (size_t)(n + 1), lb = sizeof(double) * (size_t)plans[q].l_size;
-    l.l_in_smem = lb + vec <= 220 * 1024 ? 1 : 0;
-    dyn = std::max(dyn, vec + (l.l_in_smem ? lb : 0));
+    dyn = std::max(dyn, step_smem_bytes(n, plans[q].plan.size(), plans[q].l_size, l));
   }
   c->cmp_dyn = dyn;
   CU(cudaMemcpyAsync(c->d_cmp_i32.p, blob.data(), sizeof(int32_t) * blob.size(), cudaMemcpyHostToDevice, c->stream));
@@ -1916,6 +1911,43 @@
   CU(cudaMemcpy(out64, c->d_prof.p, sizeof(long long) * 64, cudaMemcpyDeviceToHost));
   return MVICP_OK;
 }
+int mvicp_debug_block_solve(int32_t device, int32_t nb, const double* A, const double* b, int32_t force_global, double* y,
+                            int32_t* ok, int32_t* levels, int64_t* plan_bytes, int64_t* factor_bytes) {
+  if (nb <= 0 || !A || !b || !y || !ok) return fail(MVICP_ERR_INVALID, "mvicp_debug_block_solve: bad arguments");
+  const int n = 6 * nb;
+  std::vector<std::pair<int, int>> links;
+  for (int I = 1; I < nb; ++I)
+    for (int J = 0; J < I; ++J) {
+      bool nz = false;
+      for (int i = 0; i < 6 && !nz; ++i) for (int j = 0; j < 6 && !nz; ++j) nz = A[(size_t)(6 * I + i) * n + 6 * J + j] != 0.0;
+      if (nz) links.push_back({I, J});
+    }
+  const BlockPlan bp = plan_block_cholesky(nb, links);
+  if (levels) *levels = bp.words[BP_NLEV];
+  if (plan_bytes) *plan_bytes = (int64_t)(sizeof(int32_t) * bp.words.size());
+  if (factor_bytes) *factor_bytes = (int64_t)sizeof(double) * bp.l_size;
+  CU(cudaSetDevice(device));
+  DevBuf d_A, d_b, d_plan, d_L, d_y, d_ok;
+  RET(d_A.reserve(sizeof(double) * (size_t)n * n)); RET(d_b.reserve(sizeof(double) * n)); RET(d_y.reserve(sizeof(double) * n));
+  RET(d_plan.reserve(sizeof(int32_t) * bp.words.size())); RET(d_L.reserve(sizeof(double) * (size_t)bp.l_size));
+  RET(d_ok.reserve(sizeof(int32_t)));
+  CU(cudaMemcpy(d_A.p, A, sizeof(double) * (size_t)n * n, cudaMemcpyHostToDevice));
+  CU(cudaMemcpy(d_b.p, b, sizeof(double) * n, cudaMemcpyHostToDevice));
+  CU(cudaMemcpy(d_plan.p, bp.words.data(), sizeof(int32_t) * bp.words.size(), cudaMemcpyHostToDevice));
+  CU(cudaMemcpy(d_y.p, y, sizeof(double) * n, cudaMemcpyHostToDevice));
+  NormalLayout lay{};
+  lay.plan = d_plan.as<int32_t>(); lay.plan_words = (int32_t)bp.words.size();
+  lay.Lg = d_L.as<double>(); lay.rhs = d_y.as<double>();
+  size_t dyn = step_smem_bytes(n, bp.words.size(), bp.l_size, lay);
+  if (force_global) { lay.plan_in_smem = 0; lay.l_in_smem = 0; dyn = sizeof(double) * (size_t)(n + 1); }
+  CU(cudaFuncSetAttribute(block_solve_kernel, cudaFuncAttributeMaxDynamicSharedMemorySize, 220 * 1024));
+  block_solve_kernel<<<1, STEP_THREADS, dyn>>>(lay, d_A.as<double>(), d_b.as<double>(), n, d_ok.as<int>());
+  CU(cudaGetLastError());
+  CU(cudaStreamSynchronize(0));
+  CU(cudaMemcpy(ok, d_ok.p, sizeof(int32_t), cudaMemcpyDeviceToHost));
+  CU(cudaMemcpy(y, d_y.p, sizeof(double) * n, cudaMemcpyDeviceToHost));
+  return MVICP_OK;
+}
 int mvicp_get_stream(mvicp_ctx* c, void** stream) { if (!c || !stream) return fail(MVICP_ERR_INVALID, "bad arguments"); *stream = (void*)c->stream; return MVICP_OK; }
 int mvicp_sync(mvicp_ctx* c) { if (!c) return fail(MVICP_ERR_INVALID, "null ctx"); CU(cudaSetDevice(c->device)); CU(cudaStreamSynchronize(c->stream)); return MVICP_OK; }
 
```

New measurement: 589.3, median of 6. +6.4%, better.
